# LulinZhang/BRDF-NeRF

Measured on AMD Instinct MI355X. Metric: train rays/sec (+ MFMA% of roofline), spsbrdf-nerf 64 samples/ray, 1/2/4/8 MI355X, higher is better.
Workload: dtype bf16; 1 GPU; BASELINE config 2: Djibouti-shaped synthetic rays, spsbrdf-nerf lambert train step (pass1 64 + guided 64 samples/ray, F=512, 8 Siren layers, PE10, ds_lambda=10), 4096 rays/GPU/step (4096 rays per global step, weak scaling); rays_per_gpu=4096, n_samples=64, guided_samples=64, parallelism=dp1, settle_steps=221

## Files before the change

brdf_nerf_amd/_lib.py:

```python
import ctypes as C
import os

HERE = os.path.dirname(os.path.abspath(__file__))
LIB_PATH = os.environ.get("BRDFNERF_HIP_LIB") or os.path.join(HERE, "libbrdfnerf_hip.so")

BN_MAX_LAYERS = 12
BN_MAX_HEADS = 6
BN_F32, BN_BF16, BN_F16 = 0, 1, 2
DTYPES = {"fp32": BN_F32, "bf16": BN_BF16, "fp16": BN_F16}
BN_ACT_SIN, BN_ACT_RELU = 0, 1
BN_HEAD_PLAIN, BN_HEAD_RPV_K, BN_HEAD_RPV_THETA, BN_HEAD_HAPKE_THETA, BN_HEAD_TILE3, BN_HEAD_BETA = 0, 1, 2, 3, 4, 5
BN_BRDF_AUX = 16

fptr = C.c_void_p


class FieldDesc(C.Structure):
    _fields_ = [("feat", C.c_int32), ("layers", C.c_int32), ("skip", C.c_int32), ("pe_freqs", C.c_int32),
                ("act", C.c_int32), ("dtype", C.c_int32), ("n_heads", C.c_int32),
                ("head_out", C.c_int32 * BN_MAX_HEADS), ("head_kind", C.c_int32 * BN_MAX_HEADS),
                ("normal_lr", C.c_int32), ("normal_an", C.c_int32), ("out_channels", C.c_int32), ("fold_feats", C.c_int32),
                ("dir_dim", C.c_int32), ("dir_freqs", C.c_int32), ("t_dim", C.c_int32)]


_PARAM_FIELDS = [("trunk_w", fptr * BN_MAX_LAYERS), ("trunk_b", fptr * BN_MAX_LAYERS),
                 ("sigma_w", fptr), ("sigma_b", fptr), ("feats_w", fptr), ("feats_b", fptr),
                 ("head_w1", fptr * BN_MAX_HEADS), ("head_b1", fptr * BN_MAX_HEADS),
                 ("head_w2", fptr * BN_MAX_HEADS), ("head_b2", fptr * BN_MAX_HEADS),
                 ("normal_w", fptr), ("normal_b", fptr), ("head0_wdir", fptr), ("head0_wdir_ld", C.c_int64),
                 ("head1_wt", fptr), ("head1_wt_ld", C.c_int64)]


class FieldParams(C.Structure):
    _fields_ = list(_PARAM_FIELDS)


class FieldGrads(C.Structure):
    _fields_ = list(_PARAM_FIELDS) + [("d_t_embed", fptr)]


class Points(C.Structure):
    _fields_ = [("xyz", fptr), ("rays", fptr), ("z", fptr), ("ray_stride", C.c_int32), ("n_samples", C.c_int32),
                ("n_points", C.c_int64), ("dirs", fptr), ("t_embed", fptr), ("point_offset", C.c_int64), ("total_points", C.c_int64),
                ("z2", fptr), ("n_samples2", C.c_int32), ("seg1_points", C.c_int64)]


class ShadeDesc(C.Structure):
    _fields_ = [(k, C.c_int32) for k in ("kind", "C", "ch_normal", "ch_p0", "ch_p1", "ch_p2", "rhoc_is_albedo", "shell",
                                         "cos_irradiance", "usealldepth")] + \
               [(k, C.c_float) for k in ("hpk_scl", "f0", "rgb_padding", "lambda_rgb", "lambda_ds", "lambda_hs")] + \
               [("irr", fptr), ("irr_stride", C.c_int64)]


BN_SHADE_LAMBERT, BN_SHADE_RPV, BN_SHADE_HAPKE, BN_SHADE_MICROFACET = 0, 1, 2, 3


class NormalReg(C.Structure):
    _fields_ = [("rays_d", fptr), ("rd_stride", C.c_int64), ("ch_an", C.c_int32), ("ch_lr", C.c_int32),
                ("lambda_an", C.c_float), ("lambda_lr", C.c_float), ("lambda_spv", C.c_float), ("spv_ch_an", C.c_int32),
                ("spv_ch_lr", C.c_int32), ("spv_ray", fptr), ("spv_tot", fptr)]


class Noise(C.Structure):
    _fields_ = [("rng", fptr), ("noise_std", C.c_float), ("rng_stream", C.c_uint32), ("ray_offset", C.c_int64)]


class FoldDesc(C.Structure):
    _fields_ = [("n_heads", C.c_int32), ("F", C.c_int32), ("rows", C.c_int32), ("wf", fptr), ("bf", fptr),
                ("w1", fptr * BN_MAX_HEADS), ("w1_ld", C.c_int64 * BN_MAX_HEADS), ("b1", fptr * BN_MAX_HEADS),
                ("w_fold", fptr * BN_MAX_HEADS), ("b_fold", fptr * BN_MAX_HEADS), ("m", fptr * BN_MAX_HEADS), ("s", fptr * BN_MAX_HEADS),
                ("d_w1", fptr * BN_MAX_HEADS), ("d_w1_ld", C.c_int64 * BN_MAX_HEADS), ("d_b1", fptr * BN_MAX_HEADS),
                ("d_wf", fptr), ("d_bf", fptr)]


BN_ABI_VERSION = 7
BN_STATE_BYTES, BN_STATE_LOSS_OFF, BN_STATE_LOSS_SLOTS, BN_STATE_POW_OFF, BN_STATE_PART_OFF = 1024, 64, 64, 320, 512
BN_STATE_NOISE_OFF = 40
BN_RNG_COARSE, BN_RNG_GUIDED, BN_RNG_GUIDED_TARGET, BN_RNG_NOISE_COARSE, BN_RNG_NOISE_MERGED, BN_RNG_SUN = 1, 2, 3, 4, 5, 6
BN_BWD_CHAIN, BN_BWD_WGRAD_TRUNK, BN_BWD_WGRAD_HEADS, BN_BWD_SKINNY, BN_BWD_ALL = 1, 2, 4, 8, 15


class LibraryMissing(RuntimeError):
    pass


_lib = None

_SIGS = {
    "bn_abi_version": (C.c_int, []),
    "bn_source_hash": (C.c_char_p, []),
    "bn_last_error": (C.c_char_p, []),
    "bn_build_flags": (C.c_char_p, []),
    "bn_set_deterministic": (C.c_int, [C.c_int]),
    "bn_get_deterministic": (C.c_int, []),
    "bn_field_packed_bytes": (C.c_size_t, [C.POINTER(FieldDesc)]),
    "bn_pack_field": (C.c_int, [C.POINTER(FieldDesc), C.POINTER(FieldParams), fptr, fptr]),
    "bn_field_stash_bytes": (C.c_size_t, [C.POINTER(FieldDesc), C.c_int64]),
    "bn_field_sigma": (C.c_int, [C.POINTER(FieldDesc), C.POINTER(FieldParams), fptr, C.POINTER(Points), fptr, fptr]),
    "bn_field_forward": (C.c_int, [C.POINTER(FieldDesc), C.POINTER(FieldParams), fptr, C.POINTER(Points), fptr, fptr,
                                   fptr]),
    "bn_field_backward": (C.c_int, [C.POINTER(FieldDesc), C.POINTER(FieldParams), fptr, C.POINTER(Points), fptr, fptr,
                                    fptr, C.POINTER(FieldGrads), fptr]),
    "bn_field_backward_parts": (C.c_int, [C.POINTER(FieldDesc), C.POINTER(FieldParams), fptr, C.POINTER(Points), fptr, fptr,
                                          fptr, C.POINTER(FieldGrads), C.c_int32, fptr]),
    "bn_field_normals": (C.c_int, [C.POINTER(FieldDesc), C.POINTER(FieldParams), fptr, C.POINTER(Points), fptr, fptr, fptr,
                                   C.c_int32, fptr]),
    "bn_composite_forward": (C.c_int, [fptr, fptr, C.c_int64, fptr, C.c_float, fptr, C.c_int64, C.c_int32, C.c_int64,
                                       C.c_int32, fptr, fptr, fptr, fptr, fptr, fptr]),
    "bn_composite_backward": (C.c_int, [fptr, fptr, C.c_int64, fptr, C.c_float, fptr, C.c_int64, C.c_int32, C.c_int64,
                                        C.c_int32, fptr, fptr, fptr, fptr, C.c_int64, fptr, C.c_int64, fptr]),
    "bn_lambert_loss": (C.c_int, [fptr, C.c_int32, fptr, fptr, C.c_int32, fptr, fptr, fptr, fptr, fptr, fptr, C.c_float, C.c_float,
                                  C.c_float, C.c_int32, C.c_int64, fptr, fptr, fptr, fptr, fptr, fptr]),
    "bn_stratified_z": (C.c_int, [fptr, fptr, C.c_int64, fptr, C.c_int64, C.c_int32, fptr, fptr]),
    "bn_guided_samples": (C.c_int, [fptr, fptr, fptr, fptr, C.c_int64, C.c_int32, C.c_int32, C.c_float, C.c_float,
                                    C.c_float, fptr, fptr, fptr, fptr, fptr, fptr, fptr, fptr, fptr]),
    "bn_guided_samples_nf": (C.c_int, [fptr, fptr, fptr, fptr, C.c_int64, C.c_int32, C.c_int32, fptr, C.c_float, fptr, fptr,
                                       fptr, fptr, fptr, fptr, fptr, fptr, fptr]),
    "bn_brdf_rpv_forward": (C.c_int, [fptr] * 7 + [C.c_int64, fptr, fptr, fptr]),
    "bn_brdf_rpv_backward": (C.c_int, [fptr] * 8 + [C.c_int64] + [fptr] * 6),
    "bn_brdf_hapke_forward": (C.c_int, [fptr] * 7 + [C.c_float, C.c_int32, C.c_int64, fptr, fptr, fptr]),
    "bn_brdf_hapke_backward": (C.c_int, [fptr] * 7 + [C.c_float, C.c_int32, fptr, C.c_int64] + [fptr] * 6),
    "bn_brdf_microfacet_forward": (C.c_int, [fptr] * 5 + [C.c_float, C.c_int64, fptr, fptr, fptr]),
    "bn_brdf_microfacet_backward": (C.c_int, [fptr] * 5 + [C.c_float, fptr, C.c_int64] + [fptr] * 4),
    "bn_adam_step": (C.c_int, [fptr, fptr, fptr, fptr, C.c_int64, C.c_float, C.c_float, C.c_float, C.c_float,
                               C.c_float, C.c_int32, C.c_float, fptr]),
    "bn_count_nonfinite": (C.c_int, [fptr, C.c_int64, fptr, fptr]),
    "bn_stratified_z_rng": (C.c_int, [fptr, fptr, C.c_int64, fptr, C.c_uint32, C.c_int64, C.c_int64, C.c_int32, fptr, fptr]),
    "bn_rng_uniform": (C.c_int, [fptr, C.c_uint32, C.c_int64, fptr, fptr]),
    "bn_rng_normal": (C.c_int, [fptr, C.c_uint32, C.c_int64, fptr, fptr]),
    "bn_normal_spv_reduce": (C.c_int, [fptr, C.c_int64, C.c_int32, C.c_float, fptr, fptr, fptr, fptr]),
    "bn_composite_guided": (C.c_int, [fptr, fptr, C.c_int64, C.c_int64, C.c_int32, C.c_int32, fptr, C.c_float, fptr, C.c_int64,
                                      fptr, C.c_int64, fptr, C.c_int64, fptr, fptr, fptr, C.c_uint32, C.c_uint32, C.c_int64, fptr, fptr,
                                      fptr, fptr, fptr, fptr, fptr]),
    "bn_merged_composite_forward": (C.c_int, [fptr, fptr, fptr, fptr, C.c_int32, C.c_int32, C.c_int32, C.c_int64, fptr, fptr, fptr,
                                              fptr, fptr, fptr, fptr, fptr, fptr, fptr, fptr]),
    "bn_merged_composite_backward": (C.c_int, [fptr, fptr, fptr, fptr, C.c_int32, C.c_int32, C.c_int32, C.c_int64, fptr, fptr, fptr,
                                               fptr, C.c_float, fptr, fptr, fptr, fptr, fptr, fptr, fptr]),
    "bn_ray_shade_loss": (C.c_int, [fptr, fptr, fptr, fptr, fptr, fptr, C.c_int64, fptr, C.c_int64, fptr, fptr, C.c_int64, fptr,
                                    C.c_int64, fptr, C.c_int64, fptr, C.c_int64, C.c_int64, fptr, fptr, fptr, C.c_int32, fptr, fptr,
                                    fptr, fptr, fptr, fptr]),
    "bn_ray_shade_dirs": (C.c_int, [fptr, fptr, fptr, fptr, C.c_int64, fptr, fptr, C.c_int64, C.c_int32, fptr, fptr, fptr]),
    "bn_lambert_tail": (C.c_int, [fptr, fptr, fptr, fptr, C.c_int32, C.c_int32, C.c_int32, C.c_int64, fptr, fptr, C.c_int64, fptr,
                                  C.c_int64, fptr, C.c_int64, fptr, C.c_int64, C.c_float, C.c_float, C.c_float, C.c_int32, fptr, fptr,
                                  C.c_int32, fptr, fptr, fptr, fptr, fptr, fptr, fptr, fptr]),
    "bn_sample_brdf_forward": (C.c_int, [fptr, fptr, fptr, C.c_int64, C.c_int64, C.c_int32, C.c_int64, C.c_int64, C.c_int32, C.c_int32,
                                         fptr, C.c_int32, fptr]),
    "bn_sample_brdf_backward": (C.c_int, [fptr, fptr, fptr, C.c_int64, C.c_int64, C.c_int32, C.c_int64, C.c_int64, C.c_int32, C.c_int32,
                                          fptr, C.c_int32, fptr, fptr]),
    "bn_fold_heads": (C.c_int, [fptr, fptr]),
    "bn_unfold_heads": (C.c_int, [fptr, fptr]),
    "bn_adam_multi": (C.c_int, [fptr, fptr, fptr, fptr, C.c_int32, fptr, fptr, fptr, C.c_float, C.c_float, C.c_float, C.c_float,
                                C.c_float, C.c_int32, fptr, fptr]),
    "bn_device_faults": (C.c_int, [C.POINTER(C.c_uint), fptr]),
    "bn_prof_enable": (C.c_int, [C.c_int]),
    "bn_prof_collect": (C.c_int, [C.POINTER(C.c_double), C.POINTER(C.c_int), C.c_int]),
}

PROF_NAMES = ["pack", "field_fwd_sigma", "field_fwd_full", "field_bwd_chain", "wgrad", "skinny_wgrad", "composite_fwd",
              "composite_bwd", "guided_samples", "stratified_z", "adam", "brdf", "field_adjoint", "field_adjoint_bwd", "wgrad_reduce"]


def prof_enable(on):
    lib().bn_prof_enable(int(bool(on)))


def prof_collect():
    n = len(PROF_NAMES)
    ms, cnt = (C.c_double * n)(), (C.c_int * n)()
    lib().bn_prof_collect(ms, cnt, n)
    return {PROF_NAMES[i]: (ms[i], cnt[i]) for i in range(n) if cnt[i]}


def exported_symbols():
    return sorted(_SIGS)


def load(path, baseline=False):
    if not os.path.exists(path):
        raise LibraryMissing(f"{path} not found: build the HIP extension first "
                             f"(python -m brdf_nerf_amd.build). There is no CPU fallback.")
    L = C.CDLL(path)
    for name, (res, args) in _SIGS.items():
        if baseline and not hasattr(L, name):
            continue
        fn = getattr(L, name)
        fn.restype, fn.argtypes = res, args
    if not baseline and L.bn_abi_version() != BN_ABI_VERSION:
        raise LibraryMissing(f"{path}: ABI version mismatch; rebuild")
    if not baseline and os.environ.get("BRDFNERF_ALLOW_STALE_LIB", "0") in ("", "0"):
        from .build import CSRC, source_hash
        if os.path.isdir(CSRC):
            have, want = L.bn_source_hash().decode(), source_hash()
            if have != want:
                raise LibraryMissing(f"{path} was built from other sources (library {have}, tree {want}): run "
                                     f"python -m brdf_nerf_amd.build (BRDFNERF_ALLOW_STALE_LIB=1 to load it anyway)")
    return L


def lib():
    global _lib
    if _lib is None:
        _lib = load(LIB_PATH)
        if os.environ.get("BRDFNERF_DETERMINISTIC", "0") not in ("", "0"):
            _lib.bn_set_deterministic(1)
    return _lib


def set_deterministic(on=True):
    return bool(lib().bn_set_deterministic(1 if on else 0))


def deterministic():
    L = lib()
    if not hasattr(L, "bn_get_deterministic"):
        prev = L.bn_set_deterministic(0)
        if prev:
            L.bn_set_deterministic(1)
        return bool(prev)
    return bool(L.bn_get_deterministic())


def use(handle):
    global _lib
    prev, _lib = _lib, handle
    return prev


def check(status, what=""):
    if status != 0:
        raise RuntimeError(f"{what} failed ({status}): {lib().bn_last_error().decode()}")
```

brdf_nerf_amd/csrc/field.h:

```cpp
#pragma once
#include "common.h"

#define BN_MAX_PASS 3
#define BN_DPH (3 * BN_MAX_HEADS)
#define BN_SINGLE_HEAD_NTW(NT) ((NT) > 1 ? (NT) / 2 : 1)

struct FieldGeom {
  int F, L, skip, pe_freqs, act;
  int P;
  int KP;
  int NT;
  int BM, waves;
  int dsz;
  int H2;
  int n_heads, n_pass;
  int pass_heads[BN_MAX_PASS];
  int pass_N[BN_MAX_PASS];
  int pass_NTW[BN_MAX_PASS];
  int head_col[BN_MAX_HEADS];
  int C;
  int ch_normal_an, ch_normal_lr;
  int fold;
  int DD, KD, dir_freqs, TD, KT0;
};

static inline void bn_tile_config(int dtype, int *BM, int *waves) {
  *BM = bn_half(dtype) ? 128 : 64;
  *waves = 8;
}

static inline int bn_make_geom(const bn_field_desc *d, FieldGeom *g) {
  BN_REQUIRE(d->feat >= 64 && d->feat <= 512 && d->feat % 64 == 0 && (d->feat == 512 || d->feat <= 256),
             "field: feat=%d unsupported (64,128,192,256,512)", d->feat);
  BN_REQUIRE(d->dtype == BN_F32 || d->dtype == BN_BF16 || d->dtype == BN_F16, "field: dtype=%d unknown", d->dtype);
  BN_REQUIRE(d->layers >= 2 && d->layers <= BN_MAX_LAYERS, "field: layers=%d unsupported", d->layers);
  BN_REQUIRE(d->skip < d->layers && d->skip != 0, "field: skip=%d invalid", d->skip);
  BN_REQUIRE(d->n_heads >= 1 && d->n_heads <= BN_MAX_HEADS, "field: n_heads=%d", d->n_heads);
  BN_REQUIRE(d->pe_freqs >= 0 && d->pe_freqs <= 10, "field: pe_freqs=%d", d->pe_freqs);
  g->F = d->feat; g->L = d->layers; g->skip = d->skip; g->pe_freqs = d->pe_freqs; g->act = d->act;
  g->P = d->pe_freqs > 0 ? 6 * d->pe_freqs : 3;
  g->KP = (g->P + 63) / 64 * 64;
  bn_tile_config(d->dtype, &g->BM, &g->waves);
  g->dsz = (int)bn_dsize(d->dtype, d->normal_an);
  {
    const int per = (d->feat + 32 * g->waves - 1) / (32 * g->waves);
    g->NT = per <= 1 ? 1 : (per <= 2 ? 2 : 4);
  }
  g->H2 = d->feat / 2;
  g->fold = d->fold_feats != 0;
  g->DD = d->dir_dim; g->dir_freqs = d->dir_freqs; g->TD = d->t_dim;
  g->KT0 = (d->dir_dim + 7) / 8 * 8;
  g->KD = (g->KT0 + d->t_dim + 15) / 16 * 16;
  BN_REQUIRE(d->dir_dim == 0 || (d->dir_dim == (d->dir_freqs > 0 ? 6 * d->dir_freqs : 3) && d->dir_dim <= 32 && g->fold),
             "field: dir_dim=%d dir_freqs=%d fold=%d unsupported (input_viewdir needs fold_feats and at most 5 octaves)", d->dir_dim,
             d->dir_freqs, g->fold);
  {
    const bool beta = d->n_heads >= 2 && d->head_kind[1] == BN_HEAD_BETA;
    BN_REQUIRE(beta == (d->t_dim > 0) && d->t_dim >= 0 && d->t_dim <= 16 && (!beta || (g->fold && d->head_out[1] == 1)),
               "field: t_dim=%d needs exactly a 1-wide head 1 of kind BN_HEAD_BETA (and fold_feats)", d->t_dim);
    for (int i = 0; i < d->n_heads; ++i)
      BN_REQUIRE(i == 1 || d->head_kind[i] != BN_HEAD_BETA, "field: BN_HEAD_BETA is head 1 only (head %d)", i);
    BN_REQUIRE(g->KD <= 32, "field: dir_dim=%d + t_dim=%d do not fit the 32-column extra-input tile", d->dir_dim, d->t_dim);
  }
  g->n_heads = d->n_heads;
  g->n_pass = (d->n_heads + 1) / 2;
  int c = d->t_dim > 0 ? 5 : 4;
  g->ch_normal_an = g->ch_normal_lr = -1;
  if (d->normal_an) { g->ch_normal_an = c; c += 3; }
  if (d->normal_lr) { g->ch_normal_lr = c; c += 3; }
  g->head_col[0] = 0;
  for (int i = 1; i < d->n_heads; ++i) {
    BN_REQUIRE(d->head_out[i] == 1 || d->head_out[i] == 3, "field: head_out[%d]=%d", i, d->head_out[i]);
    if (d->head_kind[i] == BN_HEAD_BETA) { g->head_col[i] = 4; continue; }
    g->head_col[i] = c;
    c += (d->head_kind[i] == BN_HEAD_PLAIN || d->head_kind[i] == BN_HEAD_HAPKE_THETA) ? d->head_out[i] : 3;
  }
  BN_REQUIRE(d->head_out[0] == 3, "field: head 0 must be rgb (3 outputs)");
  g->C = c;
  BN_REQUIRE(d->out_channels == c, "field: out_channels=%d but layout needs %d", d->out_channels, c);
  for (int p = 0; p < g->n_pass; ++p) {
    g->pass_heads[p] = (d->n_heads - 2 * p) >= 2 ? 2 : 1;
    g->pass_N[p] = g->pass_heads[p] * g->H2;
    g->pass_NTW[p] = g->pass_heads[p] == 2 ? g->NT : BN_SINGLE_HEAD_NTW(g->NT);
  }
  return 0;
}

struct PackedLayout {
  size_t fwd_trunk[BN_MAX_LAYERS][2];
  size_t fwd_feats, fwd_head[BN_MAX_PASS];
  size_t fwd_sigma, fwd_nlr;
  size_t fwd_dir;
  size_t bwd_trunk[BN_MAX_LAYERS];
  size_t bwd_feats, bwd_head[BN_MAX_PASS];
  size_t bwd_pe[2];
  size_t total;
};

static inline size_t bn_pad(size_t v, size_t a) { return (v + a - 1) / a * a; }

static inline void bn_make_packed_layout(const FieldGeom &g, PackedLayout *pl) {
  size_t off = 0;
  auto take = [&](size_t rows, size_t k) { size_t o = off; off += bn_pad(rows, 32) * bn_pad(k, 16); return o; };
  for (int l = 0; l < g.L; ++l) {
    pl->fwd_trunk[l][0] = pl->fwd_trunk[l][1] = 0;
    if (l == 0) pl->fwd_trunk[l][0] = take(g.F, g.KP);
    else if (l == g.skip) { pl->fwd_trunk[l][0] = take(g.F, g.KP); pl->fwd_trunk[l][1] = take(g.F, g.F); }
    else pl->fwd_trunk[l][0] = take(g.F, g.F);
  }
  pl->fwd_sigma = take(32, g.F);
  pl->fwd_feats = g.fold ? 0 : take(g.F, g.F);
  for (int p = 0; p < g.n_pass; ++p) pl->fwd_head[p] = take(g.pass_N[p], g.F);
  pl->fwd_nlr = g.ch_normal_lr >= 0 ? take(32, g.F) : 0;
  pl->fwd_dir = g.KD > 0 ? take(g.pass_N[0], g.KD) : 0;
  for (int l = 0; l < g.L; ++l) pl->bwd_trunk[l] = l >= 1 ? take(g.F, g.F) : 0;
  pl->bwd_feats = g.fold ? 0 : take(g.F, g.F);
  for (int p = 0; p < g.n_pass; ++p) pl->bwd_head[p] = take(g.F, g.pass_N[p]);
  pl->bwd_pe[0] = take(g.KP, g.F);
  pl->bwd_pe[1] = g.skip > 0 ? take(g.KP, g.F) : 0;
  pl->total = off;
}

struct StashLayout {
  size_t gscale;
  size_t sraw;
  size_t nraw;
  size_t dpre_trunk;
  size_t dpre_head;
  size_t pe;
  size_t dirpe;
  size_t Y[BN_MAX_LAYERS];
  size_t D[BN_MAX_LAYERS];
  size_t feats;
  size_t G[BN_MAX_PASS];
  size_t DG[BN_MAX_PASS];
  size_t dZ[BN_MAX_LAYERS];
  size_t dfeats;
  size_t dG[BN_MAX_PASS];
  size_t gradx;
  size_t sbar;
  size_t sprime;
  size_t gbar_pe;
  size_t adj_delta[BN_MAX_LAYERS];
  size_t adj_a[BN_MAX_LAYERS];
  size_t adj_abar[BN_MAX_LAYERS + 1];
  size_t adj_zbar[BN_MAX_LAYERS];
  size_t wgpart, wgpart_bytes;
  size_t total;
  int64_t Mpad;
};

static inline int64_t bn_wgrad_splits(bool half, int64_t tiles, int64_t Mpad, int64_t *m_per_block) {
  const int64_t stage = half ? 64 : 32;
  const int64_t min_mpb = half ? 512 : 256;
  int64_t n_split = (half ? (Mpad <= 327680 ? BN_W2_BLOCKS : 2 * BN_W2_BLOCKS) : 2048) / (tiles > 0 ? tiles : 1);
  if (n_split < 1) n_split = 1;
  int64_t mpb = ceil_div64(ceil_div64(Mpad, n_split), stage) * stage;
  if (mpb < min_mpb) mpb = min_mpb;
  if (m_per_block) *m_per_block = mpb;
  return ceil_div64(Mpad, mpb);
}
static inline size_t bn_wgpart_bytes(const FieldGeom &g, int64_t Mpad, size_t esz) {
  const bool half = esz != 4;
  const int64_t tl = half ? 256 : 128, ft = (g.F + tl - 1) / tl;
  const int64_t tiles_bound = (2 * g.L + 12) * ft * ft;
  const int64_t grid_bound = half ? 2 * BN_W2_BLOCKS : 2048;
  int64_t slabs = tiles_bound > grid_bound ? tiles_bound : grid_bound;
  const int64_t by_points = tiles_bound * bn_wgrad_splits(half, 1, Mpad, nullptr);
  if (by_points < slabs) slabs = by_points;
  const size_t wg = (size_t)slabs * (size_t)(tl * tl + tl) * 4;
  int64_t sk_splits = ceil_div64(Mpad, g.BM);
  if (sk_splits > 256) sk_splits = 256;
  const size_t sk = (size_t)10 * (size_t)sk_splits * (4 * 512 + 4) * 4;
  return wg > sk ? wg : sk;
}

static inline void bn_make_stash_layout(const FieldGeom &g, int64_t n_points, int BM, size_t esz, StashLayout *s) {
  const size_t dsz = (size_t)g.dsz;
  int64_t Mpad = ceil_div64(n_points, BM) * BM;
  s->Mpad = Mpad;
  size_t off = 0;
  auto take = [&](size_t bytes) { size_t o = off; off += bn_pad(bytes, 256); return o; };
  s->gscale = take(256);
  s->sraw = take((size_t)Mpad * 4);
  s->nraw = take((size_t)Mpad * 16);
  s->dpre_trunk = take((size_t)Mpad * 16);
  s->dpre_head = take((size_t)Mpad * BN_DPH * 4);
  s->pe = take((size_t)Mpad * g.KP * esz);
  s->dirpe = g.KD > 0 ? take((size_t)Mpad * g.KD * esz) : 0;
  for (int l = 0; l < g.L; ++l) s->Y[l] = take((size_t)Mpad * g.F * esz);
  for (int l = 0; l < g.L; ++l) s->D[l] = take((size_t)Mpad * g.F * dsz);
  s->feats = take((size_t)Mpad * g.F * esz);
  for (int p = 0; p < BN_MAX_PASS; ++p) {
    s->G[p] = s->DG[p] = s->dG[p] = 0;
    if (p < g.n_pass) {
      s->G[p] = take((size_t)Mpad * g.F * esz);
      s->DG[p] = take((size_t)Mpad * g.F * dsz);
    }
  }
  for (int l = 0; l < g.L; ++l) s->dZ[l] = take((size_t)Mpad * g.F * esz);
  s->dfeats = take((size_t)Mpad * g.F * esz);
  for (int p = 0; p < g.n_pass; ++p) s->dG[p] = take((size_t)Mpad * g.pass_N[p] * esz);
  s->gradx = s->sbar = s->sprime = s->gbar_pe = 0;
  for (int l = 0; l < BN_MAX_LAYERS; ++l) s->adj_delta[l] = s->adj_a[l] = s->adj_abar[l] = s->adj_zbar[l] = 0;
  s->adj_abar[BN_MAX_LAYERS] = 0;
  if (g.ch_normal_an >= 0) {
    s->gradx = take((size_t)Mpad * 16);
    s->sbar = take((size_t)Mpad * 4);
    s->sprime = take((size_t)Mpad * 4);
    s->gbar_pe = take((size_t)Mpad * g.KP * esz);
    for (int l = 0; l < g.L; ++l) {
      s->adj_delta[l] = take((size_t)Mpad * g.F * esz);
      s->adj_a[l] = take((size_t)Mpad * g.F * esz);
      s->adj_abar[l + 1] = take((size_t)Mpad * g.F * esz);
      s->adj_zbar[l] = take((size_t)Mpad * g.F * esz);
    }
  }
  s->wgpart_bytes = bn_wgpart_bytes(g, Mpad, esz);
  s->wgpart = take(s->wgpart_bytes);
  s->total = off;
}

static inline void bn_stash_layout_at(const FieldGeom &g, const bn_points *pts, int BM, size_t esz, StashLayout *s) {
  const int64_t total = pts->total_points > 0 ? pts->total_points : pts->n_points;
  bn_make_stash_layout(g, total, BM, esz, s);
  const size_t off = (size_t)pts->point_offset;
  if (off == 0) return;
  const size_t dsz = (size_t)g.dsz, F = (size_t)g.F;
  s->sraw += off * 4; s->nraw += off * 16; s->dpre_trunk += off * 16; s->dpre_head += off * BN_DPH * 4;
  s->pe += off * g.KP * esz;
  if (g.KD > 0) s->dirpe += off * g.KD * esz;
  for (int l = 0; l < g.L; ++l) { s->Y[l] += off * F * esz; s->D[l] += off * F * dsz; s->dZ[l] += off * F * esz; }
  s->feats += off * F * esz; s->dfeats += off * F * esz;
  for (int p = 0; p < g.n_pass; ++p) { s->G[p] += off * F * esz; s->DG[p] += off * F * dsz; s->dG[p] += off * g.pass_N[p] * esz; }
  if (g.ch_normal_an >= 0) {
    s->gradx += off * 16; s->sbar += off * 4; s->sprime += off * 4; s->gbar_pe += off * g.KP * esz;
    for (int l = 0; l < g.L; ++l) {
      s->adj_delta[l] += off * F * esz; s->adj_a[l] += off * F * esz; s->adj_abar[l + 1] += off * F * esz; s->adj_zbar[l] += off * F * esz;
    }
  }
  s->Mpad = ceil_div64(pts->n_points, BM) * BM;
}
```

brdf_nerf_amd/csrc/field_bwd.hip:

```cpp
#include "field_kernels.h"
#include "field_wgrad.h"

int bn_field_adjoint_backward(const bn_field_desc *desc, const bn_field_params *params, const void *packed, const bn_points *pts,
                              const float *d_out, void *stash, void *stream);

__device__ unsigned int g_bwd_fault;
unsigned int bn_bwd_fault_read(hipStream_t) {
  unsigned int v = 0u;
  if (hipMemcpyFromSymbol(&v, HIP_SYMBOL(g_bwd_fault), sizeof(unsigned int), 0, hipMemcpyDeviceToHost) != hipSuccess) return 0x80000000u;
  return v;
}
const unsigned int *bn_bwd_fault_ptr() {
  void *p = nullptr;
  return hipGetSymbolAddress(&p, HIP_SYMBOL(g_bwd_fault)) == hipSuccess ? (const unsigned int *)p : nullptr;
}

BN_PH_DEFINE_READER(bn_debug_phase_read_bwd)
BN_CLK_DEFINE(bn_debug_clock_read_bwd)

struct BwdArgs {
  FieldGeom g;
  bn_field_desc d;
  bn_field_params p;
  PackedLayout pl;
  StashLayout sl;
  const void *packed;
  int64_t M;
  const float *out, *d_out;
  char *stash;
  int an;
  const float *amax;
};

__device__ __forceinline__ void head_y_dy(int kind, int nout, const float *o, const float *dgo, int c, float &y, float &dy) {
  if (kind == BN_HEAD_PLAIN || kind == BN_HEAD_BETA) { y = o[c]; dy = dgo[c]; }
  else if (kind == BN_HEAD_HAPKE_THETA) { y = o[0] * (1.f / 0.52359877559829887f); dy = dgo[0] * 0.52359877559829887f; }
  else {
    const float ov = nout == 1 ? o[0] : o[c];
    const float dv = nout == 1 ? dgo[0] + dgo[1] + dgo[2] : dgo[c];
    if (kind == BN_HEAD_RPV_K) { y = (ov - 1.f) * 0.5f + 0.5f; dy = 2.f * dv; }
    else if (kind == BN_HEAD_RPV_THETA) { y = ov * 0.5f + 0.5f; dy = 2.f * dv; }
    else { y = ov; dy = dv; }
  }
}

__device__ __forceinline__ void bwd_dpre(const BwdArgs &A, int64_t gm, float (&dph)[BN_DPH], float (&dpt)[4]) {
  const FieldGeom &g = A.g;
#pragma unroll
  for (int i = 0; i < BN_DPH; ++i) dph[i] = 0.f;
#pragma unroll
  for (int i = 0; i < 4; ++i) dpt[i] = 0.f;
  if (gm >= A.M) return;
  const float *o = A.out + gm * g.C, *dgo = A.d_out + gm * g.C;
  for (int hd = 0; hd < g.n_heads; ++hd) {
    const int nout = A.d.head_out[hd], kind = A.d.head_kind[hd];
    for (int c = 0; c < nout; ++c) {
      float y, dy;
      head_y_dy(kind, nout, o + g.head_col[hd], dgo + g.head_col[hd], c, y, dy);
      dph[hd * 3 + c] = kind == BN_HEAD_BETA ? dy * -expm1f(-y) : dy * y * (1.f - y);
    }
  }
  const float sraw = ((const float *)(A.stash + A.sl.sraw))[gm];
  dpt[0] = dgo[3] * sigmoid_f(sraw);
  if (A.an) dpt[0] += ((const float *)(A.stash + A.sl.sbar))[gm];
  if (g.ch_normal_lr >= 0) {
    const float *v = (const float *)(A.stash + A.sl.nraw) + gm * 4;
    const float *dn = dgo + g.ch_normal_lr;
    const float n2 = v[0] * v[0] + v[1] * v[1] + v[2] * v[2];
    const float eps = 1.1920928955078125e-07f;
    const float inv = 1.f / sqrtf(fmaxf(n2, eps));
    const float vd = v[0] * dn[0] + v[1] * dn[1] + v[2] * dn[2];
    const float k = n2 > eps ? vd * inv * inv * inv : 0.f;
#pragma unroll
    for (int i = 0; i < 3; ++i) dpt[1 + i] = -(dn[i] * inv - v[i] * k);
  }
}

__global__ void clear_words_kernel(unsigned int *p, int n) {
  for (int i = blockIdx.x * blockDim.x + threadIdx.x; i < n; i += gridDim.x * blockDim.x) p[i] = 0u;
}

template <int WHICH> __global__ __launch_bounds__(256) void grad_amax_kernel(const BwdArgs A, float *amax) {
  const FieldGeom &g = A.g;
  float mx = 0.f;
  for (int64_t gm = (int64_t)blockIdx.x * 256 + threadIdx.x; gm < A.M; gm += (int64_t)gridDim.x * 256) {
    if (WHICH == 0) {
      float dph[BN_DPH], dpt[4];
      bwd_dpre(A, gm, dph, dpt);
#pragma unroll
      for (int i = 0; i < BN_DPH; ++i) { const float a = fabsf(dph[i]); mx = (a < 3.0e38f && a > mx) ? a : mx; }
#pragma unroll
      for (int i = 0; i < 4; ++i) { const float a = fabsf(dpt[i]); mx = (a < 3.0e38f && a > mx) ? a : mx; }
    } else {
      const float *gx = (const float *)(A.stash + A.sl.gradx) + gm * 4;
      const float *dn = A.d_out + gm * g.C + g.ch_normal_an;
      const float n2 = gx[0] * gx[0] + gx[1] * gx[1] + gx[2] * gx[2];
      const float eps = 1.1920928955078125e-07f;
      const float inv = 1.f / sqrtf(fmaxf(n2, eps));
      const float gd = gx[0] * dn[0] + gx[1] * dn[1] + gx[2] * dn[2];
      const float k = n2 > eps ? gd * inv * inv * inv : 0.f;
      const float fmx = g.pe_freqs > 0 ? (float)(1 << (g.pe_freqs - 1)) : 1.f;
      const float spm = ((const float *)(A.stash + A.sl.sprime))[gm];
#pragma unroll
      for (int c = 0; c < 3; ++c) { const float a = fabsf(dn[c] * inv - gx[c] * k) * spm * fmx; mx = (a < 3.0e38f && a > mx) ? a : mx; }
    }
  }
#pragma unroll
  for (int o = 32; o >= 1; o >>= 1) mx = fmaxf(mx, __shfl_xor(mx, o));
  if ((threadIdx.x & 63) == 0 && mx > 0.f) atomicMax((unsigned int *)amax + WHICH, __float_as_uint(mx));
}

template <typename T>
__global__ __launch_bounds__(256) void head_xin_grad_kernel(const T *__restrict__ dG, int ldg, int col0, int H2, const float *__restrict__ Wt,
                                                            int64_t ldw, int TD, int64_t M, const float *amax, float *__restrict__ d_t) {
  __shared__ float W[256 * 16];
  for (int i = threadIdx.x; i < H2 * 16; i += 256) W[i] = (i & 15) < TD ? Wt[(int64_t)(i >> 4) * ldw + (i & 15)] : 0.f;
  __syncthreads();
  const float osc = 1.f / chain_scale(amax);
  const int lane = threadIdx.x & 63, wave = threadIdx.x >> 6;
  for (int64_t gm = (int64_t)blockIdx.x * 4 + wave; gm < M; gm += (int64_t)gridDim.x * 4) {
    float acc[16];
#pragma unroll
    for (int c = 0; c < 16; ++c) acc[c] = 0.f;
    const T *row = dG + gm * ldg + col0;
    for (int j = lane; j < H2; j += 64) {
      const float d = (float)row[j];
#pragma unroll
      for (int c = 0; c < 16; ++c) acc[c] += d * W[j * 16 + c];
    }
#pragma unroll
    for (int c = 0; c < 16; ++c) {
#pragma unroll
      for (int o = 32; o >= 1; o >>= 1) acc[c] += __shfl_xor(acc[c], o);
    }
    if (lane < TD) {
      float v = 0.f;
#pragma unroll
      for (int c = 0; c < 16; ++c) v = lane == c ? acc[c] : v;
      d_t[gm * TD + lane] = v * osc;
    }
  }
}

template <typename T, int MT, int NTW, bool D16>
__device__ __forceinline__ void bwd_head_dG(const BwdArgs &A, int p, T *ACT, const float *DPH, int64_t , int64_t tile) {
  typedef typename DKind<T, D16>::type DK;
  typedef typename Elem<T>::vec4 vec4;
  constexpr int BM = MT * 32;
  const FieldGeom &g = A.g;
  const int F = g.F, LDA = F + Elem<T>::kPad;
  const int tid = threadIdx.x, lane = tid & 63, wave = tid >> 6, r = lane & 31, h = lane >> 5;
  const int N = g.pass_N[p];
  const int pc0 = wave * 32 * NTW;
  if (pc0 >= N) return;
// ... 167 lines not shown
          const int n0 = ncol0 + nt * 32 + 16 * gp + 4 * h;
          float dv[8], v[8];
          dpiece_get<DK>(dpre[nt][mt], gp, g.act, dscale, dv);
#pragma unroll
          for (int e = 0; e < 8; ++e) v[e] = acc[nt][mt][8 * gp + e];
          if constexpr (top) {
            const float ds = DPT[m * 4], a0 = DPT[m * 4 + 1], a1 = DPT[m * 4 + 2], a2 = DPT[m * 4 + 3];
#pragma unroll
            for (int half = 0; half < 2; ++half) {
              const int n = n0 + 8 * half;
              const f32x4 ws = *(const f32x4 *)(A.p.sigma_w + n);
#pragma unroll
              for (int e = 0; e < 4; ++e) v[4 * half + e] += ws[e] * ds;
              if (nlr) {
                const f32x4 wn0 = *(const f32x4 *)(A.p.normal_w + n), wn1 = *(const f32x4 *)(A.p.normal_w + F + n),
                            wn2 = *(const f32x4 *)(A.p.normal_w + 2 * F + n);
#pragma unroll
                for (int e = 0; e < 4; ++e) v[4 * half + e] += wn0[e] * a0 + wn1[e] * a1 + wn2[e] * a2;
              }
            }
          }
#pragma unroll
          for (int e = 0; e < 8; ++e) v[e] *= dv[e];
          if (A.an) {
            float zb[8];
            if constexpr (ZPRE) {
              const auto zq = __builtin_bit_cast(bf16x8, zraw[nt][mt][gp]);
#pragma unroll
              for (int e = 0; e < 8; ++e) zb[e] = (float)zq[e];
            } else {
              ld8((const WT *)(A.stash + A.sl.adj_zbar[lo]) + (size_t)tile * BM * F + native_off8<MT, NT>(wave, nt, mt, gp, lane), zb);
            }
#pragma unroll
            for (int e = 0; e < 8; ++e) v[e] += zb[e] * zr;
          }
          if constexpr (NATZ) {
            const typename Elem<T>::frag q = cvt8(T(), v);
            *(vec4 *)(ACT + (size_t)m * LDA + n0) = __builtin_shufflevector(q, q, 0, 1, 2, 3);
            *(vec4 *)(ACT + (size_t)m * LDA + n0 + 8) = __builtin_shufflevector(q, q, 4, 5, 6, 7);
            stash_store_buf(Zr, voff, ((((wave_u * NT + nt) * MT + mt) * 2 + gp) * 1024), q);
          } else {
            *(vec4 *)(ACT + (size_t)m * LDA + n0) = to_vec4(T(), v[0], v[1], v[2], v[3]);
            *(vec4 *)(ACT + (size_t)m * LDA + n0 + 8) = to_vec4(T(), v[4], v[5], v[6], v[7]);
          }
        }
      }
  };
  {
    if (!g.fold) {
      zero_acc<MT, NT>(acc);
      T *fdst = (T *)(A.stash + A.sl.dfeats) + (size_t)m0 * F;
      if (!ride) tile_to_global<T>(ACT, LDA, fdst, F, BM, F);
      if (wave_on) {
        load_D(g.L - 1, 0, NPRE);
        const size_t off = A.pl.bwd_feats + (size_t)(ncol0 / 32) * KSF * 512;
        if (ride) {
          TileCopyExact<T> zcopy(ACT, LDA, fdst, F, F, tid, WAVES * 64);
          gemm_seg<T, MT, NT, DP>(acc, packed + off, KSF, ACT, LDA, lane, zcopy);
        } else {
          gemm_seg<T, MT, NT, DP>(acc, packed + off, KSF, ACT, LDA, lane);
        }
        load_D(g.L - 1, NPRE, NT);
      }
    } else if (wave_on) {
      load_D(g.L - 1, 0, NT);
    }
    BN_PH(9)
    __syncthreads();
    BN_PH(10)
    if (wave_on) epilogue(g.L - 1, std::true_type());
    BN_PH(11)
    __syncthreads();
    BN_PH(12)
  }
  for (int l = g.L - 1; l >= 1; --l) {
    const int it = g.L - 1 - l;
    const int lo = l - 1;
    zero_acc<MT, NT>(acc);
    T *zdst = (T *)(A.stash + A.sl.dZ[l]) + (size_t)m0 * F;
    if (!NATZ && !ride) tile_to_global<T>(ACT, LDA, zdst, F, BM, F);
    if (wave_on) {
      if (!PING || BN_BWD_D_AT == 0) load_D(lo, 0, NPRE);
      const size_t off = A.pl.bwd_trunk[l] + (size_t)(ncol0 / 32) * KSF * 512;
      if constexpr (PING) {
        pp_wait(WR + 0, 4 * it, &g_bwd_fault);
        if (grp == 1) pp_wait(RD + 0, 4 * (it + 1), &g_bwd_fault);
        BN_PH(12)
        __builtin_amdgcn_s_setprio(1);
        if constexpr (sizeof(T) == 2) {
          gemm_fixed<T, MT, NT, (DP & (BN_GEMM_AFFINE - 1)), 32, 16>(acc, packed + off, KSF, 0, ACT, LDA, lane, [&]() {
            pp_signal(RD + 0 + grp, lane);
            pp_wait(WR + 1, 4 * it, &g_bwd_fault);
            if (BN_BWD_D_AT == 1) load_D(lo, 0, NPRE);
          });
        }
        __builtin_amdgcn_s_setprio(0);
        pp_signal(RD + 2 + grp, lane);
        if (BN_BWD_D_AT == 2) load_D(lo, 0, NPRE);
      } else if (!NATZ && ride) {
        TileCopyExact<T> zcopy(ACT, LDA, zdst, F, F, tid, WAVES * 64);
        gemm_seg<T, MT, NT, DP>(acc, packed + off, KSF, ACT, LDA, lane, zcopy);
      } else {
        gemm_seg<T, MT, NT, DP>(acc, packed + off, KSF, ACT, LDA, lane);
      }
      load_D(lo, NPRE, NT);
    }
    BN_PH(9)
    if constexpr (PING) {
      pp_wait(RD + 2 * grp + 0, 4 * (it + 1), &g_bwd_fault);
      pp_wait(RD + 2 * grp + 1, 4 * (it + 1), &g_bwd_fault);
    } else {
      __syncthreads();
    }
    BN_PH(10)
    if (wave_on) epilogue(lo, std::false_type());
    BN_PH(11)
    if constexpr (PING) pp_signal(WR + grp, lane);
    else __syncthreads();
    BN_PH(12)
  }
  if (PING) __syncthreads();
  if (!NATZ) tile_to_global<T>(ACT, LDA, (T *)(A.stash + A.sl.dZ[0]) + (size_t)m0 * F, F, BM, F);
  BN_PH(13)
#ifndef BN_PHASE_TIMING_WGRAD
  BN_PH_FLUSH
#endif
#ifndef BN_CLOCK_STAMP_WGRAD
  BN_CLK_END
#endif
}

template <typename T, int MT, int NT, int WAVES, bool D16> static int launch_bwd_k(const BwdArgs &a, int64_t tiles, hipStream_t st) {
  constexpr int BM = MT * 32;
  const size_t lds = (size_t)BM * (a.g.F + Elem<T>::kPad) * sizeof(T) + (size_t)BM * (BN_DPH + 4) * sizeof(float) + 64;
  if (int e = bn_configure_lds((const void *)field_bwd_kernel<T, MT, NT, WAVES, D16>, lds, "field_bwd")) return e;
  BnProfScope prof_(BN_K_BWD_CHAIN, st);
  field_bwd_kernel<T, MT, NT, WAVES, D16><<<dim3((unsigned)tiles), WAVES * 64, lds, st>>>(a);
  BN_LAUNCH_CHECK("field_bwd");
  return 0;
}
template <typename T, int MT, int NT, int WAVES> static int launch_bwd(const BwdArgs &a, int64_t tiles, hipStream_t st) {
  if constexpr (std::is_same<T, f16>::value) {
    if (a.g.dsz == 2) return launch_bwd_k<T, MT, NT, WAVES, true>(a, tiles, st);
  }
  return launch_bwd_k<T, MT, NT, WAVES, false>(a, tiles, st);
}

extern "C" int bn_field_backward(const bn_field_desc *desc, const bn_field_params *params, const void *packed,
                                 const bn_points *pts, const float *out, const float *d_out, void *stash,
                                 const bn_field_grads *G, void *stream) {
  return bn_field_backward_parts(desc, params, packed, pts, out, d_out, stash, G, BN_BWD_ALL, stream);
}

extern "C" int bn_field_backward_parts(const bn_field_desc *desc, const bn_field_params *params, const void *packed,
                                       const bn_points *pts, const float *out, const float *d_out, void *stash,
                                       const bn_field_grads *G, int32_t parts, void *stream) {
  BwdArgs a;
  if (int e = bn_make_geom(desc, &a.g)) return e;
  if (const int f = bn_field_fault_seen()) {
    bn_set_error("field_backward: an earlier %s launch lost an LDS hand-over (pp_wait timed out): its results are invalid",
                 (f & 1) ? "forward" : "backward");
    return BN_ELAUNCH;
  }
  a.an = desc->normal_an ? 1 : 0;
  BN_REQUIRE(pts && pts->n_points > 0 && packed && out && d_out && stash && G, "field_backward: null argument");
  BN_REQUIRE(parts > 0 && (parts & ~BN_BWD_ALL) == 0, "field_backward: parts=%d", parts);
  BN_REQUIRE(pts->point_offset == 0 && (pts->total_points == 0 || pts->total_points == pts->n_points),
             "field_backward: the backward runs over a whole point set (point_offset = 0)");
  BN_REQUIRE(pts->seg1_points == 0 || (pts->rays && pts->z && pts->z2 && pts->n_samples2 > 0 && pts->seg1_points < pts->n_points &&
                                       pts->seg1_points % pts->n_samples == 0 && (pts->n_points - pts->seg1_points) % pts->n_samples2 == 0),
             "field_backward: bad two-block point set");
  BN_REQUIRE(pts->seg1_points == 0 || !(desc->t_dim > 0 && G->d_t_embed), "field_backward: d_t_embed is not served for a two-block point set");
  const FieldGeom &g = a.g;
  a.d = *desc; a.p = *params; a.packed = packed; a.M = pts->n_points; a.out = out; a.d_out = d_out; a.stash = (char *)stash;
  bn_make_packed_layout(g, &a.pl);
  const bool bf = bn_half(desc->dtype);
  const bool f16m = desc->dtype == BN_F16;
  const int BM = g.BM;
  const size_t esz = bn_esize(desc->dtype);
  bn_make_stash_layout(g, pts->n_points, BM, esz, &a.sl);
  const int64_t tiles = ceil_div64(pts->n_points, BM);
  hipStream_t st = (hipStream_t)stream;
  int rc;
  float *amax = f16m ? (float *)((char *)stash + a.sl.gscale) : nullptr;
  a.amax = amax;
  const unsigned amax_grid = (unsigned)(ceil_div64(pts->n_points, 256) < 1024 ? ceil_div64(pts->n_points, 256) : 1024);
  if (parts & BN_BWD_CHAIN) {
  if (f16m) {
    clear_words_kernel<<<1, 64, 0, st>>>((unsigned int *)amax, 4);
    BN_LAUNCH_CHECK("clear amax");
    if (a.an) {
      grad_amax_kernel<1><<<amax_grid, 256, 0, st>>>(a, amax);
      BN_LAUNCH_CHECK("grad_amax<1>");
    }
  }
  if (a.an) {
    rc = bn_field_adjoint_backward(desc, params, packed, pts, d_out, stash, stream);
    if (rc) return rc;
  }
  if (f16m) {
    grad_amax_kernel<0><<<amax_grid, 256, 0, st>>>(a, amax);
    BN_LAUNCH_CHECK("grad_amax<0>");
  }
  rc = [&]() -> int { BN_DISPATCH_TILE(desc->dtype, g, launch_bwd, (a, tiles, st)); }();
  if (rc) return rc;
  }

  const StashLayout &sl = a.sl;
  char *S = (char *)stash;
  const int F = g.F, P0 = g.P;
  WgradArgs w;
  w.n_jobs = 0; w.Mpad = sl.Mpad; w.tile0[0] = 0; w.amax = amax; w.part = nullptr; w.n_split = 1;
  int scale_sel = 1;
  int b_native = 0;
  int a_native = 0;
  int part = BN_BWD_WGRAD_TRUNK;
  auto add = [&](const void *A_, int lda, int a0, const void *B_, int ldb, int b0, float *C, int ldc, float *bias, int N, int K) {
    if (!C || !(parts & part)) return;
    WgradJob &j = w.job[w.n_jobs];
    j.scale_sel = scale_sel;
    j.b_native = (b_native ? WG_B_NATIVE : 0) | (a_native ? WG_A_NATIVE : 0); j.b_bm = BM; j.b_F = F; j.b_bm_shift = BM == 128 ? 7 : 6;
    j.A = A_; j.B = B_; j.C = C; j.bias = bias; j.lda = lda; j.ldb = ldb; j.ldc = ldc; j.a_col0 = a0; j.b_col0 = b0; j.N = N; j.K = K;
    w.tile0[w.n_jobs + 1] = w.tile0[w.n_jobs] + ((N + 127) / 128) * ((K + 127) / 128);
    ++w.n_jobs;
  };
  const int naty = bf ? 1 : 0;
  a_native = naty;
  for (int l = 0; l < g.L; ++l) {
    const void *dZ = S + sl.dZ[l];
    b_native = 0;
    if (l == 0) add(dZ, F, 0, S + sl.pe, g.KP, 0, G->trunk_w[l], P0, G->trunk_b[l], F, P0);
    else if (l == g.skip) {
      add(dZ, F, 0, S + sl.pe, g.KP, 0, G->trunk_w[l], F + P0, G->trunk_b[l], F, P0);
      b_native = naty;
      add(dZ, F, 0, S + sl.Y[l - 1], F, 0, G->trunk_w[l] ? G->trunk_w[l] + P0 : nullptr, F + P0, nullptr, F, F);
    } else {
      b_native = naty;
      add(dZ, F, 0, S + sl.Y[l - 1], F, 0, G->trunk_w[l], F, G->trunk_b[l], F, F);
    }
  }
  a_native = 0;
  b_native = naty;
  part = BN_BWD_WGRAD_HEADS;
  if (!g.fold) add(S + sl.dfeats, F, 0, S + sl.Y[g.L - 1], F, 0, G->feats_w, F, G->feats_b, F, F);
  part = BN_BWD_WGRAD_TRUNK;
  b_native = 0;
  if (a.an) {
    scale_sel = 2;
    for (int l = 0; l < g.L; ++l) {
      const void *dl = S + sl.adj_delta[l];
      if (l == 0) add(dl, F, 0, S + sl.gbar_pe, g.KP, 0, G->trunk_w[l], P0, nullptr, F, P0);
      else if (l == g.skip) {
        add(dl, F, 0, S + sl.gbar_pe, g.KP, 0, G->trunk_w[l], F + P0, nullptr, F, P0);
        add(dl, F, 0, S + sl.adj_abar[l], F, 0, G->trunk_w[l] ? G->trunk_w[l] + P0 : nullptr, F + P0, nullptr, F, F);
      } else add(dl, F, 0, S + sl.adj_abar[l], F, 0, G->trunk_w[l], F, nullptr, F, F);
    }
  }
  scale_sel = 1;
  part = BN_BWD_WGRAD_HEADS;
  for (int hd = 0; hd < g.n_heads; ++hd) {
    const int p = hd / 2, hl = hd % 2;
    b_native = g.fold ? naty : 0;
    add(S + sl.dG[p], g.pass_N[p], hl * g.H2, S + (g.fold ? sl.Y[g.L - 1] : sl.feats), F, 0, G->head_w1[hd], F, G->head_b1[hd], g.H2, F);
  }
  if (g.DD > 0 && G->head0_wdir) {
    b_native = 0; scale_sel = 1;
    add(S + sl.dG[0], g.pass_N[0], 0, S + sl.dirpe, g.KD, 0, G->head0_wdir, (int)G->head0_wdir_ld, nullptr, g.H2, g.DD);
  }
  if (g.TD > 0 && G->head1_wt) {
    b_native = 0; scale_sel = 1;
    add(S + sl.dG[0], g.pass_N[0], g.H2, S + sl.dirpe, g.KD, g.KT0, G->head1_wt, (int)G->head1_wt_ld, nullptr, g.H2, g.TD);
  }
  BN_REQUIRE(w.n_jobs <= BN_MAX_WGRAD_JOBS, "field_backward: too many wgrad jobs");
  float *wgpart = (float *)(S + sl.wgpart);
  if (w.n_jobs > 0)
    if (int e = bn_launch_wgrad(w, bf, f16m, sl.Mpad, wgpart, sl.wgpart_bytes, st)) return e;
  if (!(parts & BN_BWD_SKINNY)) return 0;
  SkinnyArgs s;
  s.n_jobs = 0; s.Mpad = sl.Mpad; s.amax = amax; s.part = nullptr;
  for (int i = 0; i < BN_MAX_SKINNY_JOBS; ++i) { s.job[i].scale_sel = 0; s.job[i].unit_dpre = 0; }
  {
    SkinnyJob &j = s.job[s.n_jobs];
    j.X = S + sl.Y[g.L - 1]; j.ldx = F; j.x_col0 = 0; j.K = F; j.dpre = (const float *)(S + sl.dpre_trunk); j.ldp = 4; j.p_col0 = 0;
    j.nc = g.ch_normal_lr >= 0 ? 4 : 1; j.native = 0;
    if (naty) { j.native = 1; j.bm = BM; j.ntw = g.NT; j.tstride = BM * F; }
    for (int c = 0; c < 4; ++c) { j.out[c] = nullptr; j.bias[c] = nullptr; }
    j.out[0] = G->sigma_w; j.bias[0] = G->sigma_b;
    if (g.ch_normal_lr >= 0) {
      BN_REQUIRE(G->normal_w && G->normal_b, "field_backward: normal grads missing");
      for (int c = 0; c < 3; ++c) { j.out[1 + c] = G->normal_w + (size_t)c * F; j.bias[1 + c] = G->normal_b + c; }
    }
    if (j.out[0]) ++s.n_jobs;
  }
  if (a.an && G->sigma_w) {
    SkinnyJob &j = s.job[s.n_jobs++];
    j.unit_dpre = 1;
    j.scale_sel = 2;
    j.X = S + sl.adj_abar[g.L]; j.ldx = F; j.x_col0 = 0; j.K = F; j.dpre = (const float *)(S + sl.sprime); j.ldp = 1; j.p_col0 = 0; j.nc = 1; j.native = 0;
    for (int c = 0; c < 4; ++c) { j.out[c] = nullptr; j.bias[c] = nullptr; }
    j.out[0] = G->sigma_w;
  }
  for (int hd = 0; hd < g.n_heads; ++hd) {
    if (!G->head_w2[hd]) continue;
    const int p = hd / 2, hl = hd % 2;
    SkinnyJob &j = s.job[s.n_jobs++];
    j.X = S + sl.G[p]; j.ldx = 0; j.x_col0 = hl * g.H2; j.K = g.H2;
    j.native = 1; j.bm = BM; j.ntw = g.pass_NTW[p]; j.tstride = BM * F;
    j.dpre = (const float *)(S + sl.dpre_head); j.ldp = BN_DPH; j.p_col0 = hd * 3; j.nc = desc->head_out[hd];
    for (int c = 0; c < 4; ++c) { j.out[c] = nullptr; j.bias[c] = nullptr; }
    for (int c = 0; c < j.nc; ++c) { j.out[c] = G->head_w2[hd] + (size_t)c * g.H2; j.bias[c] = G->head_b2[hd] ? G->head_b2[hd] + c : nullptr; }
  }
  if (s.n_jobs > 0) {
    int skinny_splits = SKINNY_SPLITS;
    {
      int64_t most = sl.Mpad / (2 * (int64_t)BM) > 1 ? sl.Mpad / (2 * (int64_t)BM) : 1;
      if (sl.Mpad <= 131072 && most > 128) most = 128;
      if (skinny_splits > most) skinny_splits = (int)most;
    }
    int64_t smpb = ceil_div64(ceil_div64(sl.Mpad, skinny_splits), BM) * BM;
    s.m_per_block = (int)smpb;
    if (int e = bn_launch_skinny(s, bf, f16m, sl.Mpad, smpb, wgpart, sl.wgpart_bytes, st)) return e;
  }
  if (g.TD > 0 && G->d_t_embed) {
    BN_REQUIRE(params->head1_wt && params->head1_wt_ld >= g.TD && g.H2 <= 256, "field_backward: head1_wt missing (beta)");
    const int64_t M = pts->n_points;
    const unsigned blocks = (unsigned)(ceil_div64(M, 4) < 4096 ? ceil_div64(M, 4) : 4096);
    const int ldg = g.pass_N[0];
    if (f16m) head_xin_grad_kernel<f16><<<dim3(blocks), 256, 0, st>>>((const f16 *)(S + sl.dG[0]), ldg, g.H2, g.H2, params->head1_wt, params->head1_wt_ld, g.TD, M, amax, G->d_t_embed);
    else if (bf) head_xin_grad_kernel<bf16><<<dim3(blocks), 256, 0, st>>>((const bf16 *)(S + sl.dG[0]), ldg, g.H2, g.H2, params->head1_wt, params->head1_wt_ld, g.TD, M, amax, G->d_t_embed);
    else head_xin_grad_kernel<float><<<dim3(blocks), 256, 0, st>>>((const float *)(S + sl.dG[0]), ldg, g.H2, g.H2, params->head1_wt, params->head1_wt_ld, g.TD, M, amax, G->d_t_embed);
    BN_LAUNCH_CHECK("head_xin_grad");
  }
  return 0;
}
```

brdf_nerf_amd/csrc/field_wgrad.h:

```cpp
#pragma once
#include <hip/hip_runtime.h>
#include <stdint.h>

struct WgradJob {
  const void *A;
  const void *B;
  float *C;
  float *bias;
  int lda, ldb, ldc;
  int a_col0, b_col0;
  int N, K;
  int scale_sel;
  int b_native;
  int b_bm, b_F;
  int b_bm_shift;
};
#define WG_B_NATIVE 1
#define WG_A_NATIVE 2
#define BN_MAX_WGRAD_JOBS 44
struct WgradArgs {
  WgradJob job[BN_MAX_WGRAD_JOBS];
  int tile0[BN_MAX_WGRAD_JOBS + 1];
  int n_jobs;
  int64_t Mpad;
  int m_per_block;
  const float *amax;
  float *part;
  int n_split;
  int chain_next[BN_MAX_WGRAD_JOBS];
  unsigned char head[BN_MAX_WGRAD_JOBS];
};
#define WG_SLAB256 (256 * 256 + 256)
#define WG_SLAB128 (128 * 128 + 128)
#define SK_SLAB (4 * 512 + 4)

struct SkinnyJob {
  const void *X;
  const float *dpre;
  int ldx, x_col0, K, ldp, p_col0, nc;
  int native;
  int bm, ntw, tstride;
  float *out[4];
  float *bias[4];
  int scale_sel;
  int unit_dpre;
};
#define BN_MAX_SKINNY_JOBS 10
struct SkinnyArgs {
  SkinnyJob job[BN_MAX_SKINNY_JOBS];
  int n_jobs;
  int64_t Mpad;
  int m_per_block;
  const float *amax;
  float *part;
};

int bn_launch_wgrad(WgradArgs &wv, bool bf, bool f16m, int64_t Mpad, float *part, size_t part_bytes, hipStream_t st);
int bn_launch_skinny(SkinnyArgs &sv, bool bf, bool f16m, int64_t Mpad, int64_t m_per_block, float *part, size_t part_bytes, hipStream_t st);
unsigned int bn_bwd_fault_read(hipStream_t st);
```

brdf_nerf_amd/csrc/field_wgrad.hip:

```cpp
#include "field_kernels.h"
#include "field_wgrad.h"


__device__ __forceinline__ float wg_unscale(const float *amax, int sel) {
  if (amax == nullptr || sel == 0) return 1.f;
  return 1.f / (sel == 1 ? chain_scale(amax) : grad_scale_from(amax + 1, BN_GS_TARGET_ADJ));
}

#define WG_BK 32
template <typename T> struct WgTile;
template <> struct WgTile<float> { static constexpr int LD = 128 + 4; };

template <typename T> __device__ __forceinline__ typename Elem<T>::frag wg_frag(const T *tile, int mm, int col0, int lane);
template <> __device__ __forceinline__ f32x8 wg_frag<float>(const float *tile, int mm, int col0, int lane) {
  constexpr int LD = WgTile<float>::LD;
  const int h = lane >> 5, r = lane & 31;
  f32x8 f;
#pragma unroll
  for (int j = 0; j < 8; ++j) f[j] = tile[(size_t)(mm + 2 * j + h) * LD + col0 + r];
  return f;
}

template <typename T> __global__ __launch_bounds__(256) void wgrad_kernel(const WgradArgs A) {
  constexpr int LD = WgTile<T>::LD;
  constexpr int EPC = 16 / sizeof(T);
  constexpr int CPR = 128 / EPC;
  constexpr int NCH = WG_BK * CPR / 256;
  __shared__ __attribute__((aligned(16))) T sA[WG_BK * LD];
  __shared__ __attribute__((aligned(16))) T sB[WG_BK * LD];
  int jb = 0;
  while (jb + 1 < A.n_jobs && (int)blockIdx.x >= A.tile0[jb + 1]) ++jb;
  const WgradJob &J = A.job[jb];
  const int t = blockIdx.x - A.tile0[jb];
  const int tiles_k = (J.K + 127) / 128;
  const int n0 = (t / tiles_k) * 128, k0 = (t % tiles_k) * 128;
  const int tid = threadIdx.x, lane = tid & 63, wave = tid >> 6, wr = wave >> 1, wc = wave & 1;
  const int64_t mb = (int64_t)blockIdx.y * A.m_per_block;
  const int64_t me = mb + A.m_per_block < A.Mpad ? mb + A.m_per_block : A.Mpad;
  const T *gA = (const T *)J.A + J.a_col0 + n0;
  const T *gB = (const T *)J.B + J.b_col0 + k0;
  uint4 ra[NCH], rb[NCH];
  auto gload = [&](int64_t m) {
#pragma unroll
    for (int c = 0; c < NCH; ++c) {
      const int ch = tid + c * 256, row = ch / CPR, cc = (ch % CPR) * EPC;
      ra[c] = (n0 + cc < J.N) ? *(const uint4 *)(gA + (m + row) * J.lda + cc) : uint4{0, 0, 0, 0};
      rb[c] = (k0 + cc < J.K) ? *(const uint4 *)(gB + (m + row) * J.ldb + cc) : uint4{0, 0, 0, 0};
    }
  };
  auto sstore = [&]() {
#pragma unroll
    for (int c = 0; c < NCH; ++c) {
      const int ch = tid + c * 256, row = ch / CPR, cc = (ch % CPR) * EPC;
      *(uint4 *)(sA + row * LD + cc) = ra[c];
      *(uint4 *)(sB + row * LD + cc) = rb[c];
    }
  };
  f32x16 acc[2][2];
#pragma unroll
  for (int a = 0; a < 2; ++a)
#pragma unroll
    for (int b = 0; b < 2; ++b)
#pragma unroll
      for (int i = 0; i < 16; ++i) acc[a][b][i] = 0.f;
  float bsum = 0.f;
  const bool do_bias = J.bias != nullptr && k0 == 0 && tid < 128;
  gload(mb);
  for (int64_t m = mb; m < me; m += WG_BK) {
    __syncthreads();
    sstore();
    __syncthreads();
    if (m + WG_BK < me) gload(m + WG_BK);
#pragma unroll
    for (int mm = 0; mm < WG_BK; mm += 16) {
      typename Elem<T>::frag fa[2], fb[2];
#pragma unroll
      for (int a = 0; a < 2; ++a) fa[a] = wg_frag<T>(sA, mm, wr * 64 + a * 32, lane);
#pragma unroll
      for (int b = 0; b < 2; ++b) fb[b] = wg_frag<T>(sB, mm, wc * 64 + b * 32, lane);
#pragma unroll
      for (int a = 0; a < 2; ++a)
#pragma unroll
        for (int b = 0; b < 2; ++b) mma32(acc[a][b], fa[a], fb[b]);
    }
    if (do_bias) {
#pragma unroll 8
      for (int row = 0; row < WG_BK; ++row) bsum += (float)sA[row * LD + tid];
    }
  }
  float *P = A.part + ((size_t)blockIdx.x * gridDim.y + blockIdx.y) * WG_SLAB128;
#pragma unroll
  for (int a = 0; a < 2; ++a)
#pragma unroll
    for (int b = 0; b < 2; ++b)
#pragma unroll
      for (int q = 0; q < 4; ++q)
        *(f32x4 *)(P + (size_t)(((((wave * 2 + a) * 2 + b) * 4 + q) * 64 + lane) * 4)) =
            f32x4{acc[a][b][4 * q], acc[a][b][4 * q + 1], acc[a][b][4 * q + 2], acc[a][b][4 * q + 3]};
  if (do_bias) P[128 * 128 + tid] = bsum;
}

__device__ __attribute__((aligned(16))) unsigned short w2_zeros[8];
#define W2_LD (256 + 32)
#define W2_BK 64
#define W2_STAGE (W2_BK * W2_LD)
__device__ __forceinline__ int w2_swz(int row) { return ((row >> 1) & 3) << 1; }
template <typename T> __device__ __forceinline__ typename Elem<T>::frag w2_frag(const T *tile, int mm, int col0, int lane) {
  const int h = lane >> 5, grp = (lane >> 4) & 1, i = lane & 15, q = i >> 2, p = i & 3;
  const int s_lo = (4 * grp + p) ^ w2_swz(8 * h + q);
  const int d_hi = 4 * W2_LD + ((((s_lo ^ 4) - s_lo)) << 2);
  const T *a = tile + (size_t)(mm + 8 * h + q) * W2_LD + (((col0 >> 2) + s_lo) << 2);
  typedef __attribute__((address_space(3))) s16x4 lds_v4;
  const s16x4 lo = __builtin_amdgcn_ds_read_tr16_b64_v4i16((lds_v4 *)a);
  const s16x4 hi = __builtin_amdgcn_ds_read_tr16_b64_v4i16((lds_v4 *)(a + d_hi));
  union { s16x4 s[2]; typename Elem<T>::frag b; } u;
  u.s[0] = lo; u.s[1] = hi;
  return u.b;
}

__device__ __forceinline__ float frag_sum8(float s, const bf16x8 &f) {
  typedef __attribute__((ext_vector_type(2))) __bf16 bf16x2;
  const bf16x2 one = {(__bf16)1.f, (__bf16)1.f};
  s = __builtin_amdgcn_fdot2_f32_bf16(__builtin_shufflevector(f, f, 0, 1), one, s, false);
  s = __builtin_amdgcn_fdot2_f32_bf16(__builtin_shufflevector(f, f, 2, 3), one, s, false);
  s = __builtin_amdgcn_fdot2_f32_bf16(__builtin_shufflevector(f, f, 4, 5), one, s, false);
  s = __builtin_amdgcn_fdot2_f32_bf16(__builtin_shufflevector(f, f, 6, 7), one, s, false);
  return s;
}
__device__ __forceinline__ float frag_sum8(float s, const f16x8 &f) {
  typedef __attribute__((ext_vector_type(2))) _Float16 f16x2;
  const f16x2 one = {(_Float16)1.f, (_Float16)1.f};
  s = __builtin_amdgcn_fdot2(__builtin_shufflevector(f, f, 0, 1), one, s, false);
  s = __builtin_amdgcn_fdot2(__builtin_shufflevector(f, f, 2, 3), one, s, false);
  s = __builtin_amdgcn_fdot2(__builtin_shufflevector(f, f, 4, 5), one, s, false);
  s = __builtin_amdgcn_fdot2(__builtin_shufflevector(f, f, 6, 7), one, s, false);
  return s;
}
__device__ __forceinline__ float frag_sum8(float s, const f32x8 &f) {
#pragma unroll
  for (int j = 0; j < 8; ++j) s += f[j];
  return s;
}

#if defined(BN_PHASE_TIMING) && defined(BN_PHASE_TIMING_WGRAD)
BN_PH_DEFINE_READER(bn_debug_phase_read_wgrad)
#define WG_PH_DECL BN_PH_DECL
#define WG_PH(i) BN_PH(i)
#define WG_PH_FLUSH BN_PH_FLUSH
#else
#define WG_PH_DECL
#define WG_PH(i)
#define WG_PH_FLUSH
#endif
#ifndef W2_WAVES
// ... 48 lines not shown
      *(u32x4 *)(rowp + ((sl0 ^ nswz) << 2)) = u32x4{s02[0], s13[0], s02[1], s13[1]};
    } else {
      *(u32x4 *)(sA + buf * W2_STAGE + (row0 + RPP * c) * W2_LD + scol) = ra[c];
    }
    if (BNAT) {
      T *rowp = sB + buf * W2_STAGE + (32 * (c & 1) + nr) * W2_LD;
      const int sl0 = lslot0 + 4 * ((c >> 1) & 1);
      const auto s02 = __builtin_amdgcn_permlane32_swap(rb[c][0], rb[c][2], false, false);
      const auto s13 = __builtin_amdgcn_permlane32_swap(rb[c][1], rb[c][3], false, false);
      *(u32x4 *)(rowp + ((sl0 ^ nswz) << 2)) = u32x4{s02[0], s13[0], s02[1], s13[1]};
    } else {
      *(u32x4 *)(sB + buf * W2_STAGE + (row0 + RPP * c) * W2_LD + scol) = rb[c];
    }
  };
  auto sstore = [&](int buf) {
#pragma unroll
    for (int c = 0; c < NC; ++c) sstore1(buf, c);
  };
  f32x16 acc[W2_RA][4];
#pragma unroll
  for (int a = 0; a < W2_RA; ++a)
#pragma unroll
    for (int b = 0; b < 4; ++b)
#pragma unroll
      for (int i = 0; i < 16; ++i) acc[a][b][i] = 0.f;
  constexpr int BA = W2_RA / 2;
  const bool do_bias = J.bias != nullptr && k0 == 0;
  float bsum[BA];
#pragma unroll
  for (int a = 0; a < BA; ++a) bsum[a] = 0.f;
  WG_PH_DECL
  auto compute = [&](int buf, int64_t m_next2) {
    const T *cA = sA + buf * W2_STAGE, *cB = sB + buf * W2_STAGE;
    frag_t fa[2][W2_RA], fb[2][NBV > 0 ? NBV : 1];
    auto frags = [&](int set, int mm) {
#pragma unroll
      for (int a = 0; a < W2_RA; ++a) fa[set][a] = w2_frag<T>(cA, mm, wr * (W2_RA * 32) + a * 32, lane);
#pragma unroll
      for (int b = 0; b < NBV; ++b) fb[set][b] = w2_frag<T>(cB, mm, wc * 128 + b * 32, lane);
    };
    frags(0, 0);
#pragma unroll
    for (int i = 0; i < W2_BK / 16; ++i) {
      const int cur = i & 1;
      if (i + 1 < W2_BK / 16) frags(cur ^ 1, (i + 1) * 16);
      __builtin_amdgcn_sched_barrier(0);
#pragma unroll
      for (int a = 0; a < W2_RA; ++a)
#pragma unroll
        for (int b = 0; b < NBV; ++b) mma32(acc[a][b], fa[cur][a], fb[cur][b]);
      {
#pragma unroll
        for (int a = 0; a < BA; ++a) {
          const u32x4 f0 = __builtin_bit_cast(u32x4, fa[cur][a]), f1 = __builtin_bit_cast(u32x4, fa[cur][BA + a]);
          bsum[a] = frag_sum8(bsum[a], __builtin_bit_cast(frag_t, wc ? f1 : f0));
        }
      }
      {
        constexpr int CPS = NC / (W2_BK / 16) > 0 ? NC / (W2_BK / 16) : 1;
#pragma unroll
        for (int q = 0; q < CPS; ++q) {
          const int c = i * CPS + q;
          if (c < NC) { sstore1(buf ^ 1, c); gload1(m_next2, c); }
        }
      }
      __builtin_amdgcn_sched_barrier(0);
    }
  };
  gload(mb);
  sstore(0);
#pragma unroll
  for (int c = 0; c < NC; ++c) {
    __builtin_amdgcn_sched_barrier(0);
    gload1(mb + W2_BK, c);
  }
  __builtin_amdgcn_sched_barrier(0);
  WG_PH(14)
  int buf = 0;
  for (int64_t m = mb; m < me; m += W2_BK) {
    __syncthreads();
    WG_PH(3)
    compute(buf, m + 2 * W2_BK);
    WG_PH(0)
    buf ^= 1;
  }
  const int r = lane & 31, h = lane >> 5;
#pragma unroll
  for (int a = 0; a < W2_RA; ++a)
#pragma unroll
    for (int b = 0; b < 4; ++b)
#pragma unroll
      for (int q = 0; q < 4; ++q)
        *(f32x4 *)(P + (size_t)(((((wave * W2_RA + a) * 4 + b) * 4 + q) * 64 + lane) * 4)) =
            f32x4{acc[a][b][4 * q], acc[a][b][4 * q + 1], acc[a][b][4 * q + 2], acc[a][b][4 * q + 3]};
  if (do_bias) {
#pragma unroll
    for (int a = 0; a < BA; ++a) {
      const float v = bsum[a] + __shfl_xor(bsum[a], 32);
      if (h == 0) P[256 * 256 + wr * (W2_RA * 32) + (wc * BA + a) * 32 + r] = v;
    }
  }
  WG_PH(4)
  WG_PH_FLUSH
}

template <typename T>
__global__ __launch_bounds__(W2_WAVES * 64, W2_WAVES == 8 ? 2 : 1) void wgrad256_kernel(const WgradArgs A, int n_split, int n_blocks) {
  extern __shared__ __attribute__((aligned(16))) char smem_w[];
  T *sA = (T *)smem_w;
  T *sB = sA + 2 * W2_STAGE;
  const int per = n_blocks / 8;
  const int lid = (int)((blockIdx.x % 8) * per + blockIdx.x / 8);
  const int total_tiles = A.tile0[A.n_jobs];
  if (lid >= total_tiles * n_split) return;
  const int split = lid / total_tiles, tt = lid % total_tiles;
  int jb = 0;
  while (jb + 1 < A.n_jobs && tt >= A.tile0[jb + 1]) ++jb;
  const WgradJob &J = A.job[jb];
  const int t = tt - A.tile0[jb];
  const int tiles_k = (J.K + 255) / 256;
  const int n0 = (t / tiles_k) * 256, k0 = (t % tiles_k) * 256;
  const int64_t mb = (int64_t)split * A.m_per_block;
  const int64_t me = mb + A.m_per_block < A.Mpad ? mb + A.m_per_block : A.Mpad;
  if (mb >= me) return;
  const int wc = (threadIdx.x >> 6) & 1;
  const int cols = J.K - k0 - wc * 128;
  float *P = A.part + ((size_t)tt * n_split + split) * WG_SLAB256;
#ifdef BN_CLOCK_STAMP_WGRAD
  BN_CLK_BEGIN
#endif
  if (J.b_native & WG_A_NATIVE) {
    if (J.b_native & WG_B_NATIVE) {
      if (cols >= 65) w2_body<T, 4, true, true>(J, n0, k0, mb, me, sA, sB, P);
      else if (cols >= 33) w2_body<T, 2, true, true>(J, n0, k0, mb, me, sA, sB, P);
      else w2_body<T, 0, true, true>(J, n0, k0, mb, me, sA, sB, P);
    } else if (cols >= 65) w2_body<T, 4, false, true>(J, n0, k0, mb, me, sA, sB, P);
    else if (cols >= 33) w2_body<T, 2, false, true>(J, n0, k0, mb, me, sA, sB, P);
    else if (cols >= 1) w2_body<T, 1, false, true>(J, n0, k0, mb, me, sA, sB, P);
    else w2_body<T, 0, false, true>(J, n0, k0, mb, me, sA, sB, P);
  } else if (J.b_native & WG_B_NATIVE) {
    if (cols >= 65) w2_body<T, 4, true, false>(J, n0, k0, mb, me, sA, sB, P);
    else if (cols >= 33) w2_body<T, 2, true, false>(J, n0, k0, mb, me, sA, sB, P);
    else w2_body<T, 0, true, false>(J, n0, k0, mb, me, sA, sB, P);
  } else if (cols >= 65) w2_body<T, 4, false, false>(J, n0, k0, mb, me, sA, sB, P);
  else if (cols >= 33) w2_body<T, 2, false, false>(J, n0, k0, mb, me, sA, sB, P);
  else if (cols >= 1) w2_body<T, 1, false, false>(J, n0, k0, mb, me, sA, sB, P);
  else w2_body<T, 0, false, false>(J, n0, k0, mb, me, sA, sB, P);
#ifdef BN_CLOCK_STAMP_WGRAD
  BN_CLK_END
#endif
}


template <typename T> __global__ __launch_bounds__(256) void skinny_wgrad_kernel(const SkinnyArgs A) {
  const SkinnyJob &J = A.job[blockIdx.y];
  const float osc = wg_unscale(A.amax, J.scale_sel);
  const int64_t mb = (int64_t)blockIdx.x * A.m_per_block;
  const int64_t me = mb + A.m_per_block < A.Mpad ? mb + A.m_per_block : A.Mpad;
  const int tid = threadIdx.x;
  __shared__ float red[4 * 512 + 4];
  for (int i = tid; i < 4 * 512 + 4; i += 256) red[i] = 0.f;
  __syncthreads();
  if (J.native) {
    const int lane = tid & 63, wv = tid >> 6, r = lane & 31, h = lane >> 5;
    const int mt_n = J.bm / 32, ncb = J.K / 32;
    const T *X = (const T *)J.X;
    float bs[4] = {0, 0, 0, 0}, bs0[4] = {0, 0, 0, 0};
    for (int cb = wv; cb < ncb; cb += 4) {
      const int cbp = J.x_col0 / 32 + cb, wave_n = cbp / J.ntw, nt = cbp % J.ntw;
      float s[2][4][8];
#pragma unroll
      for (int gp = 0; gp < 2; ++gp)
#pragma unroll
        for (int c = 0; c < 4; ++c)
#pragma unroll
          for (int e = 0; e < 8; ++e) s[gp][c][e] = 0.f;
#pragma unroll 2
      for (int64_t m0 = mb; m0 < me; m0 += 32) {
        const int64_t tile = m0 / J.bm;
        const int mt = (int)(m0 % J.bm) / 32;
        const float *dp = J.dpre + (m0 + r) * J.ldp + J.p_col0;
        float d[4];
#pragma unroll
        for (int c = 0; c < 4; ++c) d[c] = dp[c];
#pragma unroll
        for (int c = 0; c < 4; ++c) bs[c] += d[c];
#pragma unroll
        for (int gp = 0; gp < 2; ++gp) {
          float x[8];
          ld8(X + (size_t)tile * J.tstride + ((((size_t)(wave_n * J.ntw + nt) * mt_n + mt) * 2 + gp) * 64 + lane) * 8, x);
#pragma unroll
          for (int c = 0; c < 4; ++c)
#pragma unroll
            for (int e = 0; e < 8; ++e) s[gp][c][e] += d[c] * x[e];
        }
      }
#pragma unroll
      for (int c = 0; c < 4; ++c)
        if (c < J.nc) {
#pragma unroll
          for (int gp = 0; gp < 2; ++gp)
#pragma unroll
            for (int e = 0; e < 8; ++e) {
              float *dst = &red[c * 512 + cb * 32 + 16 * gp + 4 * h + (e & 3) + 8 * (e >> 2)];
              float v = s[gp][c][e];
#pragma unroll
              for (int o = 16; o >= 1; o >>= 1) v += __shfl_xor(v, o);
              if (r == 0) *dst = v;
            }
        }
      if (cb == 0) {
#pragma unroll
        for (int c = 0; c < 4; ++c) bs0[c] = bs[c];
      }
#pragma unroll
      for (int c = 0; c < 4; ++c) bs[c] = 0.f;
    }
    if (wv == 0 && h == 0) {
#pragma unroll
      for (int c = 0; c < 4; ++c)
        if (c < J.nc) {
          float v = bs0[c];
#pragma unroll
          for (int o = 16; o >= 1; o >>= 1) v += __shfl_xor(v, o);
          if (r == 0) red[4 * 512 + c] = v;
        }
    }
  } else {
  const T *X = (const T *)J.X + J.x_col0;
  const int ncg = J.K / 8, nrg = 256 / ncg;
  const int cg = tid % ncg, rg = tid / ncg;
  float s[4][8], bs[4] = {0, 0, 0, 0};
#pragma unroll
  for (int c = 0; c < 4; ++c)
#pragma unroll
    for (int e = 0; e < 8; ++e) s[c][e] = 0.f;
  if (rg < nrg) {
#pragma unroll 2
    for (int64_t m = mb + rg; m < me; m += nrg) {
      float x[8];
      ld8(X + m * J.ldx + cg * 8, x);
      const float *dp = J.dpre + m * J.ldp + J.p_col0;
#pragma unroll
      for (int c = 0; c < 4; ++c) {
        const float d = J.unit_dpre ? 1.f : dp[c];
#pragma unroll
        for (int e = 0; e < 8; ++e) s[c][e] += d * x[e];
        bs[c] += d;
      }
    }
  }
  for (int turn = 0; turn < nrg; ++turn) {
    if (rg == turn) {
#pragma unroll
      for (int c = 0; c < 4; ++c)
        if (c < J.nc) {
#pragma unroll
          for (int e = 0; e < 8; ++e) red[c * 512 + cg * 8 + e] += s[c][e];
          if (cg == 0) red[4 * 512 + c] += bs[c];
        }
    }
    __syncthreads();
  }
  }
  __syncthreads();
  float *SP = A.part + ((size_t)blockIdx.y * gridDim.x + blockIdx.x) * SK_SLAB;
  for (int i = tid; i < J.nc * J.K; i += 256) {
    const int c = i / J.K, k = i % J.K;
    SP[c * 512 + k] = red[c * 512 + k];
  }
  if (tid < 4) SP[4 * 512 + tid] = tid < J.nc ? red[4 * 512 + tid] : 0.f;
}

template <int TILE> __global__ __launch_bounds__(256) void wgrad_reduce_kernel(const WgradArgs A) {
  constexpr int NB = TILE / 64;
  constexpr int SLAB = TILE * TILE + TILE;
  constexpr int SUBS = TILE * TILE / 4 / 256;
  const int tt = blockIdx.x / SUBS, sub = blockIdx.x % SUBS, tid = threadIdx.x;
  int jb = 0;
  while (jb + 1 < A.n_jobs && tt >= A.tile0[jb + 1]) ++jb;
  if (!A.head[jb]) return;
  const WgradJob &J = A.job[jb];
  const int t = tt - A.tile0[jb];
  const int tiles_k = (J.K + TILE - 1) / TILE;
  const int n0 = (t / tiles_k) * TILE, k0 = (t % tiles_k) * TILE;
  const int ns = A.n_split;
  {
    const int idx4 = sub * 256 + tid;
    const int lane = idx4 & 63, q = (idx4 >> 6) & 3, b = (idx4 >> 8) % NB, a = ((idx4 >> 8) / NB) & 1, wave = (idx4 >> 8) / (NB * 2);
    f32x4 v = {0.f, 0.f, 0.f, 0.f};
    for (int jj = jb; jj >= 0; jj = A.chain_next[jj]) {
      const float osc = wg_unscale(A.amax, A.job[jj].scale_sel);
      const float *P = A.part + (size_t)(A.tile0[jj] + t) * ns * SLAB + (size_t)idx4 * 4;
      f32x4 sum = {0.f, 0.f, 0.f, 0.f};
      int sp = 0;
      for (; sp + 8 <= ns; sp += 8) {
        f32x4 x[8];
#pragma unroll
        for (int u = 0; u < 8; ++u) x[u] = *(const f32x4 *)(P + (size_t)(sp + u) * SLAB);
#pragma unroll
        for (int u = 0; u < 8; ++u) sum += x[u];
      }
      for (; sp < ns; ++sp) sum += *(const f32x4 *)(P + (size_t)sp * SLAB);
      v += sum * osc;
    }
    const int r = lane & 31, h = lane >> 5, wr = wave >> 1, wc = wave & 1;
    const int k = k0 + wc * (TILE / 2) + b * 32 + r, nb = n0 + wr * 64 + a * 32 + 8 * q + 4 * h;
#pragma unroll
    for (int e = 0; e < 4; ++e)
      if (nb + e < J.N && k < J.K) J.C[(size_t)(nb + e) * J.ldc + k] += v[e];
  }
  if (sub == 0 && k0 == 0 && tid < TILE && n0 + tid < J.N) {
    float v = 0.f;
    float *dst = nullptr;
    for (int jj = jb; jj >= 0; jj = A.chain_next[jj]) {
      if (!A.job[jj].bias) continue;
      dst = A.job[jj].bias;
      const float osc = wg_unscale(A.amax, A.job[jj].scale_sel);
      const float *P = A.part + (size_t)(A.tile0[jj] + t) * ns * SLAB + TILE * TILE + tid;
      float sum = 0.f;
      for (int sp = 0; sp < ns; ++sp) sum += P[(size_t)sp * SLAB];
      v += sum * osc;
    }
    if (dst) dst[n0 + tid] += v;
  }
}

__global__ __launch_bounds__(256) void skinny_reduce_kernel(const SkinnyArgs A, int n_split) {
  __shared__ float part[8][32], bpart[256];
  const int jb = blockIdx.x, c = blockIdx.y, k0 = blockIdx.z * 32, tid = threadIdx.x, kk = tid & 31, g = tid >> 5;
  const SkinnyJob &J = A.job[jb];
  if (c >= J.nc || !J.out[c] || k0 >= J.K) return;
  for (int j2 = 0; j2 < jb; ++j2)
    for (int c2 = 0; c2 < A.job[j2].nc; ++c2)
      if (A.job[j2].out[c2] == J.out[c]) return;
  float v = 0.f, vb = 0.f;
  for (int j2 = jb; j2 < A.n_jobs; ++j2)
    for (int c2 = 0; c2 < A.job[j2].nc; ++c2) {
      if (A.job[j2].out[c2] != J.out[c]) continue;
      const float osc = wg_unscale(A.amax, A.job[j2].scale_sel);
      const float *P = A.part + (size_t)j2 * n_split * SK_SLAB;
      const bool col = k0 + kk < A.job[j2].K;
      float sum = 0.f;
      int sp = g;
      for (; sp + 56 < n_split; sp += 64) {
        float x[8];
#pragma unroll
        for (int u = 0; u < 8; ++u) x[u] = col ? P[(size_t)(sp + 8 * u) * SK_SLAB + c2 * 512 + k0 + kk] : 0.f;
#pragma unroll
        for (int u = 0; u < 8; ++u) sum += x[u];
      }
      for (; sp < n_split; sp += 8) sum += col ? P[(size_t)sp * SK_SLAB + c2 * 512 + k0 + kk] : 0.f;
      __syncthreads();
      part[g][kk] = sum;
      __syncthreads();
      if (g == 0) {
        float t = 0.f;
#pragma unroll
        for (int q = 0; q < 8; ++q) t += part[q][kk];
        v += t * osc;
      }
      if (k0 == 0 && A.job[j2].bias[c2] && J.bias[c]) {
        __syncthreads();
        bpart[tid] = tid < n_split ? P[(size_t)tid * SK_SLAB + 4 * 512 + c2] : 0.f;
        __syncthreads();
        if (tid == 0) {
          float t = 0.f;
          for (int q = 0; q < n_split; ++q) t += bpart[q];
          vb += t;
        }
      }
    }
  if (g == 0 && k0 + kk < J.K) J.out[c][k0 + kk] += v;
  if (k0 == 0 && tid == 0 && J.bias[c]) *J.bias[c] += vb;
}

static void wg_chain(WgradArgs &wv) {
  for (int j = 0; j < wv.n_jobs; ++j) { wv.chain_next[j] = -1; wv.head[j] = 1; }
  for (int j = 0; j < wv.n_jobs; ++j) {
    if (!wv.head[j]) continue;
    int last = j;
    for (int q = j + 1; q < wv.n_jobs; ++q) {
      const WgradJob &a = wv.job[j], &b = wv.job[q];
      if (b.C == a.C && b.N == a.N && b.K == a.K && b.ldc == a.ldc) { wv.chain_next[last] = q; wv.head[q] = 0; last = q; }
    }
  }
}

int bn_launch_wgrad(WgradArgs &wv, bool bf, bool f16m, int64_t Mpad, float *part, size_t part_bytes, hipStream_t st) {
  if (wv.n_jobs == 0) { wv.tile0[0] = 0; return 0; }
  BN_REQUIRE(part, "wgrad: no slab workspace");
  wv.part = part;
  wv.tile0[0] = 0;
  wg_chain(wv);
  if (bf) {
    for (int j = 0; j < wv.n_jobs; ++j)
      wv.tile0[j + 1] = wv.tile0[j] + ((wv.job[j].N + 255) / 256) * ((wv.job[j].K + 255) / 256);
    const int tiles = wv.tile0[wv.n_jobs];
    static_assert(W2_BK == 64, "bn_wgrad_splits (field.h) rounds the points per workgroup to W2_BK");
    int64_t mpb2 = 0;
    const int64_t n_split = bn_wgrad_splits(true, tiles, Mpad, &mpb2);
    wv.m_per_block = (int)mpb2;
    wv.n_split = (int)n_split;
    BN_REQUIRE((size_t)tiles * n_split * WG_SLAB256 * sizeof(float) <= part_bytes, "wgrad: %d tiles x %d splits do not fit the slab workspace (%zu bytes)",
               tiles, (int)n_split, part_bytes);
    const int n_blocks = (int)ceil_div64((int64_t)tiles * n_split, 8) * 8;
    const size_t lds = (size_t)4 * W2_STAGE * 2;
    const void *kfn = f16m ? (const void *)wgrad256_kernel<f16> : (const void *)wgrad256_kernel<bf16>;
    if (int e = bn_configure_lds(kfn, lds, "wgrad256")) return e;
    {
      BnProfScope prof_(BN_K_WGRAD, st);
      const dim3 grd((unsigned)n_blocks), blk(W2_WAVES * 64);
      if (f16m) wgrad256_kernel<f16><<<grd, blk, lds, st>>>(wv, (int)n_split, n_blocks);
      else wgrad256_kernel<bf16><<<grd, blk, lds, st>>>(wv, (int)n_split, n_blocks);
      BN_LAUNCH_CHECK("wgrad256");
    }
    BnProfScope prof_(BN_K_WGRAD_REDUCE, st);
    wgrad_reduce_kernel<256><<<dim3((unsigned)tiles * 64), 256, 0, st>>>(wv);
    BN_LAUNCH_CHECK("wgrad_reduce");
    return 0;
  }
  for (int j = 0; j < wv.n_jobs; ++j)
    wv.tile0[j + 1] = wv.tile0[j] + ((wv.job[j].N + 127) / 128) * ((wv.job[j].K + 127) / 128);
  const int tiles = wv.tile0[wv.n_jobs];
  static_assert(WG_BK == 32, "bn_wgrad_splits (field.h) rounds the points per workgroup to WG_BK");
  int64_t mpb = 0;
  wv.n_split = (int)bn_wgrad_splits(false, tiles, Mpad, &mpb);
  wv.m_per_block = (int)mpb;
  BN_REQUIRE((size_t)tiles * wv.n_split * WG_SLAB128 * sizeof(float) <= part_bytes, "wgrad: %d tiles x %d splits do not fit the slab workspace (%zu bytes)",
             tiles, wv.n_split, part_bytes);
  dim3 grid((unsigned)tiles, (unsigned)wv.n_split);
  {
    BnProfScope prof_(BN_K_WGRAD, st);
    wgrad_kernel<float><<<grid, 256, 0, st>>>(wv);
    BN_LAUNCH_CHECK("wgrad");
  }
  BnProfScope prof_(BN_K_WGRAD_REDUCE, st);
  wgrad_reduce_kernel<128><<<dim3((unsigned)tiles * 16), 256, 0, st>>>(wv);
  BN_LAUNCH_CHECK("wgrad_reduce");
  return 0;
}

int bn_launch_skinny(SkinnyArgs &sv, bool bf, bool f16m, int64_t Mpad, int64_t m_per_block, float *part, size_t part_bytes, hipStream_t st) {
  if (sv.n_jobs == 0) return 0;
  sv.part = part;
  sv.m_per_block = (int)m_per_block;
  const int n_split = (int)ceil_div64(Mpad, m_per_block);
  BN_REQUIRE(n_split <= 256, "skinny_wgrad: %d splits (at most 256)", n_split);
  BN_REQUIRE(part && (size_t)sv.n_jobs * n_split * SK_SLAB * sizeof(float) <= part_bytes, "skinny_wgrad: %d jobs x %d splits do not fit the slab workspace",
             sv.n_jobs, n_split);
  dim3 grid((unsigned)n_split, (unsigned)sv.n_jobs);
  {
    BnProfScope prof_(BN_K_SKINNY, st);
    if (f16m) skinny_wgrad_kernel<f16><<<grid, 256, 0, st>>>(sv);
    else if (bf) skinny_wgrad_kernel<bf16><<<grid, 256, 0, st>>>(sv);
    else skinny_wgrad_kernel<float><<<grid, 256, 0, st>>>(sv);
    BN_LAUNCH_CHECK("skinny_wgrad");
  }
  BnProfScope prof_(BN_K_WGRAD_REDUCE, st);
  skinny_reduce_kernel<<<dim3((unsigned)sv.n_jobs, 4, 16), 256, 0, st>>>(sv, n_split);
  BN_LAUNCH_CHECK("skinny_reduce");
  return 0;
}
```

brdf_nerf_amd/csrc/head_fold.hip:

```cpp
#include "common.h"

struct FoldArgs {
  bn_fold_desc d;
  int tiles_per_head;
  int tiles_dw1, tiles_dwf;
};

__device__ __forceinline__ f32x4 k4_load(const float *p, int64_t sk, bool vec) {
  if (vec) return *(const f32x4 *)p;
  return f32x4{p[0], p[sk], p[2 * sk], p[3 * sk]};
}
__device__ __forceinline__ void tile_mac(f32x16 &acc, const float *A, int64_t sam, int64_t sak, const float *B, int64_t sbk, int64_t sbn,
                                         int k0, int k1, int lane) {
  const int r = lane & 31, h = lane >> 5;
  const bool a4 = sak == 1 && (sam & 3) == 0 && ((uintptr_t)A & 15) == 0;
  const bool b4 = sbk == 1 && (sbn & 3) == 0 && ((uintptr_t)B & 15) == 0;
  const float *a = A + r * sam + 4 * h * sak, *b = B + r * sbn + 4 * h * sbk;
  int k = k0;
  for (; k + 32 <= k1; k += 32) {
    f32x4 av[4], bv[4];
#pragma unroll
    for (int u = 0; u < 4; ++u) {
      av[u] = k4_load(a + (int64_t)(k + 8 * u) * sak, sak, a4);
      bv[u] = k4_load(b + (int64_t)(k + 8 * u) * sbk, sbk, b4);
    }
#pragma unroll
    for (int u = 0; u < 4; ++u)
#pragma unroll
      for (int q = 0; q < 4; ++q) acc = __builtin_amdgcn_mfma_f32_32x32x2f32(av[u][q], bv[u][q], acc, 0, 0, 0);
  }
  for (; k + 8 <= k1; k += 8) {
    const f32x4 av = k4_load(a + (int64_t)k * sak, sak, a4), bv = k4_load(b + (int64_t)k * sbk, sbk, b4);
#pragma unroll
    for (int q = 0; q < 4; ++q) acc = __builtin_amdgcn_mfma_f32_32x32x2f32(av[q], bv[q], acc, 0, 0, 0);
  }
}
__device__ __forceinline__ void tile_reduce(f32x16 &acc, float *red, int wave, int lane) {
  if (wave > 0) {
#pragma unroll
    for (int i = 0; i < 16; ++i) red[((wave - 1) * 16 + i) * 64 + lane] = acc[i];
  }
  __syncthreads();
  if (wave == 0) {
#pragma unroll
    for (int w = 0; w < 3; ++w)
#pragma unroll
      for (int i = 0; i < 16; ++i) acc[i] += red[(w * 16 + i) * 64 + lane];
  }
}

__global__ __launch_bounds__(256) void fold_kernel(const FoldArgs A) {
  __shared__ float red[3 * 16 * 64];
  const bn_fold_desc &d = A.d;
  const int tid = threadIdx.x, lane = tid & 63, wave = tid >> 6, r = lane & 31, h = lane >> 5;
  const int F = d.F, rows = d.rows;
  const int head = blockIdx.x / A.tiles_per_head, t = blockIdx.x % A.tiles_per_head;
  const float *w1 = d.w1[head];
  const int64_t ld1 = d.w1_ld[head];
  const int nt = F / 32, m0 = (t / nt) * 32, n0 = (t % nt) * 32;
  f32x16 acc;
#pragma unroll
  for (int i = 0; i < 16; ++i) acc[i] = 0.f;
  const int kq = F / 4;
  tile_mac(acc, w1 + (int64_t)m0 * ld1, ld1, 1, d.wf + n0, F, 1, wave * kq, (wave + 1) * kq, lane);
  tile_reduce(acc, red, wave, lane);
  if (wave == 0) {
#pragma unroll
    for (int i = 0; i < 16; ++i) d.w_fold[head][(int64_t)(m0 + (i & 3) + 8 * (i >> 2) + 4 * h) * F + n0 + r] = acc[i];
  }
  if (d.m[head]) {
    const int rr = tid >> 3, cc = (tid & 7) * 4;
    *(f32x4 *)(d.m[head] + (int64_t)(m0 + rr) * F + n0 + cc) = f32x4{0.f, 0.f, 0.f, 0.f};
  }
  if (n0 == 0) {
    float sum[8];
#pragma unroll
    for (int i = 0; i < 8; ++i) sum[i] = 0.f;
    const float *wr = w1 + (int64_t)(m0 + 8 * wave) * ld1;
    for (int k = lane; k < F; k += 64) {
      const float bk = d.bf[k];
#pragma unroll
      for (int i = 0; i < 8; ++i) sum[i] = fmaf(wr[(int64_t)i * ld1 + k], bk, sum[i]);
    }
#pragma unroll
    for (int i = 0; i < 8; ++i) {
#pragma unroll
      for (int o = 32; o > 0; o >>= 1) sum[i] += __shfl_xor(sum[i], o);
    }
    if (lane < 8) {
      float v = 0.f;
#pragma unroll
      for (int i = 0; i < 8; ++i) v = lane == i ? sum[i] : v;
      const int n = m0 + 8 * wave + lane;
      d.b_fold[head][n] = v + d.b1[head][n];
      if (d.s[head]) d.s[head][n] = 0.f;
    }
  }
}

__global__ __launch_bounds__(256) void unfold_kernel(const FoldArgs A) {
  __shared__ float red[3 * 16 * 64];
  const bn_fold_desc &d = A.d;
  const int tid = threadIdx.x, lane = tid & 63, wave = tid >> 6, r = lane & 31, h = lane >> 5;
  const int F = d.F, rows = d.rows, nt = F / 32;
  int b = blockIdx.x;
  f32x16 acc;
#pragma unroll
  for (int i = 0; i < 16; ++i) acc[i] = 0.f;
  if (b < A.tiles_dw1) {
    const int head = b / A.tiles_per_head, t = b % A.tiles_per_head;
    if (!d.m[head] || !d.d_w1[head]) return;
    const int m0 = (t / nt) * 32, n0 = (t % nt) * 32, kq = F / 4;
    tile_mac(acc, d.m[head] + (int64_t)m0 * F, F, 1, d.wf + (int64_t)n0 * F, 1, F, wave * kq, (wave + 1) * kq, lane);
    tile_reduce(acc, red, wave, lane);
    if (wave == 0) {
      const float bfn = d.bf[n0 + r];
#pragma unroll
      for (int i = 0; i < 16; ++i) {
        const int m = m0 + (i & 3) + 8 * (i >> 2) + 4 * h;
        float *p = d.d_w1[head] + (int64_t)m * d.d_w1_ld[head] + n0 + r;
        *p += acc[i] + d.s[head][m] * bfn;
      }
    }
    if (n0 == 0 && tid < 32 && d.d_b1[head]) d.d_b1[head][m0 + tid] += d.s[head][m0 + tid];
    return;
  }
  b -= A.tiles_dw1;
  if (b < A.tiles_dwf) {
    if (!d.d_wf) return;
    const int m0 = (b / nt) * 32, n0 = (b % nt) * 32, kq = rows / 4;
    for (int head = 0; head < d.n_heads; ++head)
      if (d.m[head])
        tile_mac(acc, d.w1[head] + m0, 1, d.w1_ld[head], d.m[head] + n0, F, 1, wave * kq, (wave + 1) * kq, lane);
    tile_reduce(acc, red, wave, lane);
    if (wave == 0) {
#pragma unroll
      for (int i = 0; i < 16; ++i) d.d_wf[(int64_t)(m0 + (i & 3) + 8 * (i >> 2) + 4 * h) * F + n0 + r] += acc[i];
    }
    if (n0 == 0 && d.d_bf) {
      const int kk = tid & 31, grp = tid >> 5;
      float sum = 0.f;
      for (int head = 0; head < d.n_heads; ++head)
        if (d.s[head])
          for (int n = grp; n < rows; n += 8) sum = fmaf(d.w1[head][(int64_t)n * d.w1_ld[head] + m0 + kk], d.s[head][n], sum);
      __syncthreads();
      red[grp * 32 + kk] = sum;
      __syncthreads();
      if (tid < 32) {
        float v = 0.f;
#pragma unroll
        for (int q = 0; q < 8; ++q) v += red[q * 32 + tid];
        d.d_bf[m0 + tid] += v;
      }
    }
    return;
  }
}

static int fold_check(const bn_fold_desc *d, const char *what) {
  BN_REQUIRE(d && d->n_heads >= 1 && d->n_heads <= BN_MAX_HEADS && d->F >= 64 && d->F % 64 == 0 && d->rows >= 32 && d->rows % 32 == 0 &&
                 d->wf && d->bf,
             "%s: bad descriptor (F=%d rows=%d heads=%d)", what, d ? d->F : 0, d ? d->rows : 0, d ? d->n_heads : 0);
  for (int i = 0; i < d->n_heads; ++i) BN_REQUIRE(d->w1[i] && d->w1_ld[i] >= d->F, "%s: head %d first-layer weight missing", what, i);
  return 0;
}

extern "C" int bn_fold_heads(const bn_fold_desc *d, void *stream) {
  if (int e = fold_check(d, "fold_heads")) return e;
  for (int i = 0; i < d->n_heads; ++i) BN_REQUIRE(d->b1[i] && d->w_fold[i] && d->b_fold[i], "fold_heads: head %d buffers missing", i);
  FoldArgs a;
  a.d = *d; a.tiles_per_head = (d->rows / 32) * (d->F / 32); a.tiles_dw1 = a.tiles_dwf = 0;
  BnProfScope prof_(BN_K_PACK, (hipStream_t)stream);
  fold_kernel<<<dim3((unsigned)(d->n_heads * a.tiles_per_head)), 256, 0, (hipStream_t)stream>>>(a);
  BN_LAUNCH_CHECK("fold_heads");
  return 0;
}

extern "C" int bn_unfold_heads(const bn_fold_desc *d, void *stream) {
  if (int e = fold_check(d, "unfold_heads")) return e;
  FoldArgs a;
  a.d = *d; a.tiles_per_head = (d->rows / 32) * (d->F / 32);
  a.tiles_dw1 = d->n_heads * a.tiles_per_head; a.tiles_dwf = (d->F / 32) * (d->F / 32);
  BnProfScope prof_(BN_K_PACK, (hipStream_t)stream);
  unfold_kernel<<<dim3((unsigned)(a.tiles_dw1 + a.tiles_dwf)), 256, 0, (hipStream_t)stream>>>(a);
  BN_LAUNCH_CHECK("unfold_heads");
  return 0;
}
```

brdf_nerf_amd/csrc/prof.h:

```cpp
#pragma once
#include <hip/hip_runtime.h>
enum { BN_K_PACK = 0, BN_K_FWD_SIGMA, BN_K_FWD_FULL, BN_K_BWD_CHAIN, BN_K_WGRAD, BN_K_SKINNY, BN_K_COMPOSITE_FWD,
       BN_K_COMPOSITE_BWD, BN_K_GUIDED, BN_K_STRATIFIED, BN_K_ADAM, BN_K_BRDF, BN_K_ADJOINT, BN_K_ADJBWD, BN_K_WGRAD_REDUCE, BN_K_COUNT };
extern bool g_bn_prof_on;
void bn_prof_start(int id, hipStream_t st);
void bn_prof_stop(hipStream_t st);
struct BnProfScope {
  hipStream_t st; bool on;
  BnProfScope(int id, hipStream_t s) : st(s), on(g_bn_prof_on) { if (on) bn_prof_start(id, st); }
  ~BnProfScope() { if (on) bn_prof_stop(st); }
};
```

brdf_nerf_amd/functions.py:

```python
import ctypes as C
import os

import torch

from . import _lib as L


def _stream():
    return C.c_void_p(torch.cuda.current_stream().cuda_stream)


def _p(t):
    if t is None:
        return None
    assert t.is_cuda and t.is_contiguous(), "C ABI needs contiguous device tensors"
    return C.c_void_p(t.data_ptr())


def _f32(t):
    return t.contiguous() if t.dtype == torch.float32 else t.float().contiguous()


class FieldSpec:

# ... 191 lines not shown
        names, grad_enabled, dirs = names_grad
        named = dict(zip(names, params))
        if t_embed is not None:
            t_embed = t_embed.detach().float().contiguous()
        pts = make_points(xyz, rays, z, dirs, t_embed)
        ref = xyz if xyz is not None else z
        out = torch.empty(pts.n_points, spec.out_channels, dtype=torch.float32, device=ref.device)
        ctx.t_grad = bool(grad_enabled and t_embed is not None and ctx.needs_input_grad[5])
        need_grad = grad_enabled and (any(p.requires_grad for p in params) or ctx.t_grad)
        stash = None
        if need_grad or spec.normal_an:
            nbytes = L.lib().bn_field_stash_bytes(C.byref(spec.desc), pts.n_points)
            stash = torch.empty(nbytes, dtype=torch.uint8, device=ref.device)
        ps = spec.params_struct(named)
        L.check(L.lib().bn_field_forward(C.byref(spec.desc), C.byref(ps), _p(packed), C.byref(pts), _p(out), _p(stash),
                                         _stream()), "bn_field_forward")
        if spec.normal_an:
            L.check(L.lib().bn_field_normals(C.byref(spec.desc), C.byref(ps), _p(packed), C.byref(pts), _p(stash), _p(out), None,
                                             1 if need_grad else 0, _stream()), "bn_field_normals")
            if not need_grad:
                stash = None
        ctx.spec, ctx.packed, ctx.names, ctx.stash = spec, packed, names, stash
        ctx.pts_t = (xyz, rays, z, dirs, t_embed)
        ctx.save_for_backward(out, *params)
        return out

    @staticmethod
    def backward(ctx, d_out):
        out, *params = ctx.saved_tensors
        spec, names = ctx.spec, ctx.names
        if ctx.stash is None:
            raise RuntimeError("FieldFunction.backward without a stash (forward ran under no_grad)")
        named = dict(zip(names, params))
        sizes = [p.numel() for p in params]
        offs, tot = [], 0
        for n in sizes:
            offs.append(tot)
            tot += (n + 3) // 4 * 4
        flat = torch.zeros(tot, dtype=torch.float32, device=out.device)
        grads = [flat[o:o + n].view(p.shape) for o, n, p in zip(offs, sizes, params)]
        named_grads = dict(zip(names, grads))
        gs = spec.params_struct(named_grads, grads=True)
        ps = spec.params_struct(named)
        xyz, rays, z, dirs, t_embed = ctx.pts_t
        pts = make_points(xyz, rays, z, dirs, t_embed)
        d_t = None
        if ctx.t_grad:
            d_t = torch.empty(pts.n_points, spec.t_dim, dtype=torch.float32, device=out.device)
            gs.d_t_embed = d_t.data_ptr()
            if rays is not None:
                d_t = d_t.view(rays.shape[0], -1, spec.t_dim)
        d_out = _f32(d_out)
        L.check(L.lib().bn_field_backward(C.byref(spec.desc), C.byref(ps), _p(ctx.packed), C.byref(pts), _p(out),
                                          _p(d_out), _p(ctx.stash), C.byref(gs), _stream()), "bn_field_backward")
        if spec.fold_feats:
            spec.unfold_grads(named, named_grads)
        ctx.stash = None
        if d_t is not None and d_t.dim() == 3:
            d_t = d_t.sum(1)
        return (None, None, None, None, None, d_t, None) + tuple(g if p.requires_grad else None
                                                                 for g, p in zip(grads, params))


class CompositeFunction(torch.autograd.Function):

    @staticmethod
    def forward(ctx, z, out, noise, noise_std):
        R, S = z.shape
        Cc = out.shape[-1] if out.dim() == 3 else 1
        dev = z.device
        alphas = torch.empty(R, S, dtype=torch.float32, device=dev)
        trans = torch.empty_like(alphas)
        weights = torch.empty_like(alphas)
        depth = torch.empty(R, dtype=torch.float32, device=dev)
        sigma_only = out.dim() == 2
        acc = None if sigma_only else torch.empty(R, Cc, dtype=torch.float32, device=dev)
        base = out.data_ptr()
        sig_ptr = C.c_void_p(base if sigma_only else base + 3 * 4)
        L.check(L.lib().bn_composite_forward(_p(z), sig_ptr, 1 if sigma_only else Cc, _p(noise), float(noise_std),
                                             None if sigma_only else _p(out), Cc, 0 if sigma_only else Cc, R, S,
                                             _p(alphas), _p(trans), _p(weights), _p(depth), _p(acc), _stream()),
                "bn_composite_forward")
        ctx.save_for_backward(z, out, noise)
        ctx.noise_std, ctx.sigma_only = float(noise_std), sigma_only
        ctx.mark_non_differentiable(alphas, trans)
        if sigma_only:
            return alphas, trans, weights, depth
        return alphas, trans, weights, depth, acc

    @staticmethod
    def backward(ctx, d_alphas, d_trans, d_weights, d_depth, d_acc=None):
        z, out, noise = ctx.saved_tensors
        R, S = z.shape
        sigma_only = ctx.sigma_only
        Cc = 1 if sigma_only else out.shape[-1]
        d_out = torch.zeros_like(out)
        base = out.data_ptr()
        dbase = d_out.data_ptr()
        sig_ptr = C.c_void_p(base if sigma_only else base + 12)
        dsig_ptr = C.c_void_p(dbase if sigma_only else dbase + 12)
        dw = None if d_weights is None else _f32(d_weights)
        dd = None if d_depth is None else _f32(d_depth)
        da = None if (d_acc is None or sigma_only) else _f32(d_acc)
        L.check(L.lib().bn_composite_backward(_p(z), sig_ptr, 1 if sigma_only else Cc, _p(noise), ctx.noise_std,
                                              None if sigma_only else _p(out), Cc, 0 if sigma_only else Cc, R, S,
                                              _p(dw), _p(dd), _p(da), dsig_ptr, 1 if sigma_only else Cc,
                                              None if sigma_only else _p(d_out), Cc, _stream()),
                "bn_composite_backward")
        return None, d_out, None, None


def composite(z, out, noise=None, noise_std=0.0):
    return CompositeFunction.apply(z.contiguous(), out.contiguous(), noise, noise_std)


def composite_forward_raw(z, out, noise=None, noise_std=0.0, bufs=None):
    R, S = z.shape
    Cc = out.shape[-1]
    dev = z.device
    b = bufs if bufs is not None else {}
    mk = lambda k, shape: b.get(k) if k in b else torch.empty(shape, dtype=torch.float32, device=dev)
    alphas, trans, weights = mk("alphas", (R, S)), mk("trans", (R, S)), mk("weights", (R, S))
    depth, acc = mk("depth", (R,)), mk("acc", (R, Cc))
    L.check(L.lib().bn_composite_forward(_p(z), C.c_void_p(out.data_ptr() + 12), Cc, _p(noise), float(noise_std), _p(out), Cc,
                                         Cc, R, S, _p(alphas), _p(trans), _p(weights), _p(depth), _p(acc), _stream()),
            "bn_composite_forward")
    return alphas, trans, weights, depth, acc


def composite_backward_raw(z, out, d_weights, d_depth, d_acc, noise=None, noise_std=0.0, d_out=None):
    R, S = z.shape
    Cc = out.shape[-1]
    if d_out is None:
        d_out = torch.empty_like(out)
    L.check(L.lib().bn_composite_backward(_p(z), C.c_void_p(out.data_ptr() + 12), Cc, _p(noise), float(noise_std), _p(out), Cc,
                                          Cc, R, S, _p(d_weights), _p(d_depth), _p(d_acc),
                                          C.c_void_p(d_out.data_ptr() + 12), Cc, _p(d_out), Cc, _stream()),
            "bn_composite_backward")
    return d_out


def field_forward_raw(spec, named_params, packed, out, stash, xyz=None, rays=None, z=None, point_offset=0, total_points=0):
    pts = make_points(xyz, rays, z, point_offset=point_offset, total_points=total_points)
    ps = spec.params_struct(named_params)
    L.check(L.lib().bn_field_forward(C.byref(spec.desc), C.byref(ps), _p(packed), C.byref(pts), _p(out), _p(stash), _stream()),
            "bn_field_forward")
    if spec.normal_an:
        L.check(L.lib().bn_field_normals(C.byref(spec.desc), C.byref(ps), _p(packed), C.byref(pts), _p(stash), _p(out), None, 1,
                                         _stream()), "bn_field_normals")
    return out


def field_backward_raw(spec, named_params, named_grads, packed, out, d_out, stash, xyz=None, rays=None, z=None, unfold=True,
                       zero_folded=True, parts=L.BN_BWD_ALL, z2=None):
    pts = make_points(xyz, rays, z, z2=z2)
    ps, gs = spec.params_struct(named_params), spec.params_struct(named_grads, grads=True)
    L.check(L.lib().bn_field_backward_parts(C.byref(spec.desc), C.byref(ps), _p(packed), C.byref(pts), _p(out), _p(d_out), _p(stash),
                                            C.byref(gs), int(parts), _stream()), "bn_field_backward")
    if spec.fold_feats and unfold:
        spec.unfold_grads(named_params, named_grads, zero=zero_folded)


def field_stash_bytes(spec, n_points):
    return L.lib().bn_field_stash_bytes(C.byref(spec.desc), int(n_points))


def lambert_loss(acc, weights, z, depth, rgbs, rgb_padding, lambda_rgb, valid_depth=None, target_depth=None,
                 target_weight=None, target_std=None, lambda_ds=0.0, usealldepth=False):
    R, S = weights.shape
    Cc = acc.shape[1]
    dev = acc.device
    ray_loss = torch.empty(R, dtype=torch.float32, device=dev)
    rgb = torch.empty(R, 3, dtype=torch.float32, device=dev)
    d_acc = torch.empty(R, Cc, dtype=torch.float32, device=dev)
    d_depth = torch.empty(R, dtype=torch.float32, device=dev)
    d_weights = torch.empty(R, S, dtype=torch.float32, device=dev)
    use = target_depth is not None and lambda_ds > 0
    f = lambda t: _f32(t).contiguous() if (use and t is not None) else None
    acc, weights, z, depth, rgbs = _f32(acc), _f32(weights), _f32(z), _f32(depth), _f32(rgbs)
    vd, td, tw, ts = f(valid_depth), f(target_depth), f(target_weight), f(target_std)
    L.check(L.lib().bn_lambert_loss(_p(acc), Cc, _p(weights), _p(z), S, _p(depth), _p(rgbs), _p(vd), _p(td), _p(tw), _p(ts),
                                    float(rgb_padding), float(lambda_rgb), float(lambda_ds), int(bool(usealldepth)), R,
                                    _p(ray_loss), _p(rgb), _p(d_acc), _p(d_depth), _p(d_weights), _stream()), "bn_lambert_loss")
    return ray_loss.sum(), rgb, d_acc, d_depth, d_weights


def stratified_z(near, far, u):
    R, S = u.shape
    near, far, u = _f32(near).reshape(R), _f32(far).reshape(R), _f32(u)
    z = torch.empty(R, S, dtype=torch.float32, device=u.device)
    L.check(L.lib().bn_stratified_z(_p(near), _p(far), 1, _p(u), R, S, _p(z), _stream()), "bn_stratified_z")
    return z


def guided_samples(z, weights, depth, u, near0, far0, d_range, use_target=None, target_depth=None, target_std=None,
                   u_target=None, target_row=None, merge=True):
    R, S = z.shape
    G = u.shape[1]
    dev = z.device
    z2 = torch.empty(R, G, dtype=torch.float32, device=dev)
    z_all = torch.empty(R, S + G, dtype=torch.float32, device=dev) if merge else None
    idx = torch.empty(R, S + G, dtype=torch.int64, device=dev) if merge else None
    if torch.is_tensor(near0):
        assert far0 is None and near0.is_cuda and near0.dtype == torch.float32 and near0.numel() == 2 and near0.is_contiguous()
        L.check(L.lib().bn_guided_samples_nf(_p(z), _p(weights), _p(depth), _p(u), R, S, G, C.c_void_p(near0.data_ptr()),
                                             float(d_range), _p(use_target), _p(target_depth), _p(target_std), _p(u_target),
                                             _p(target_row), _p(z2), _p(z_all), _p(idx), _stream()), "bn_guided_samples_nf")
        return z2, z_all, idx
    L.check(L.lib().bn_guided_samples(_p(z), _p(weights), _p(depth), _p(u), R, S, G, float(near0), float(far0),
                                      float(d_range), _p(use_target), _p(target_depth), _p(target_std), _p(u_target),
                                      _p(target_row), _p(z2), _p(z_all), _p(idx), _stream()), "bn_guided_samples")
    return z2, z_all, idx


def new_step_state(device, seed, lr):
    st = torch.zeros(L.BN_STATE_BYTES // 8, dtype=torch.int64, device=device)
    st[0] = int(seed) & 0x7FFFFFFFFFFFFFFF
    st.view(torch.float32)[4] = float(lr)
    st.view(torch.float64)[L.BN_STATE_POW_OFF // 8:L.BN_STATE_POW_OFF // 8 + 8] = 1.0
    return st


def set_adam_steps(state, steps, betas=(0.9, 0.999)):
    steps = list(steps) + [0] * (4 - len(steps))
    state.view(torch.int32)[6:10] = torch.tensor(steps, dtype=torch.int32)
    pw = [float(betas[0]) ** s for s in steps] + [float(betas[1]) ** s for s in steps]
    state.view(torch.float64)[L.BN_STATE_POW_OFF // 8:L.BN_STATE_POW_OFF // 8 + 8] = torch.tensor(pw, dtype=torch.float64)


def state_views(state):
    f, i = state.view(torch.float32), state.view(torch.int32)
    return state[1], f[4], i[6:10], f[L.BN_STATE_LOSS_OFF // 4:L.BN_STATE_LOSS_OFF // 4 + L.BN_STATE_LOSS_SLOTS]


def set_state_noise(state, noise_std):
    state.view(torch.float32)[L.BN_STATE_NOISE_OFF // 4].fill_(float(noise_std))


def state_loss_partials(state):
    return state.view(torch.float32)[L.BN_STATE_PART_OFF // 4:L.BN_STATE_PART_OFF // 4 + L.BN_STATE_LOSS_SLOTS]


def stratified_z_rng(rays, S, state, z=None, ray_offset=0, near_far=None, stream_id=None):
    src, col = (rays, 6) if near_far is None else (near_far, 0)
    R = src.shape[0]
    assert src.is_contiguous() and src.dtype == torch.float32 and src.shape[1] >= col + 2
    if z is None:
        z = torch.empty(R, S, dtype=torch.float32, device=src.device)
    base = src.data_ptr() + 4 * col
    L.check(L.lib().bn_stratified_z_rng(C.c_void_p(base), C.c_void_p(base + 4), src.shape[1], _p(state),
                                        L.BN_RNG_COARSE if stream_id is None else int(stream_id),
                                        int(ray_offset), R, S, _p(z), _stream()), "bn_stratified_z_rng")
    return z


def rng_uniform(state, stream_id, n):
    u = torch.empty(n, dtype=torch.float32, device=state.device)
    L.check(L.lib().bn_rng_uniform(_p(state), int(stream_id), n, _p(u), _stream()), "bn_rng_uniform")
    return u


def rng_normal(state, stream_id, n):
    x = torch.empty(n, dtype=torch.float32, device=state.device)
    L.check(L.lib().bn_rng_normal(_p(state), int(stream_id), n, _p(x), _stream()), "bn_rng_normal")
    return x


def noise_arg(state, noise_std, stream_id, ray_offset=0, from_state=False):
    if not noise_std:
        return None
    n = L.Noise()
    n.rng, n.noise_std, n.rng_stream, n.ray_offset = state.data_ptr(), -1.0 if from_state else float(noise_std), int(stream_id), int(ray_offset)
    n._keep = state
    return n


def _nz(noise):
    return None if noise is None else C.byref(noise)


def _strided(t):
    if t is None:
        return None, 1
    assert t.dtype == torch.float32 and t.dim() == 1 and t.is_cuda
    return C.c_void_p(t.data_ptr()), t.stride(0) if t.shape[0] > 1 else 1


def _depth_targets(use, valid_depth, target_depth, target_weight, target_std):
    return tuple(a for t in (valid_depth, target_depth, target_weight, target_std) for a in _strided(t if use else None))


def composite_guided(z, out1, G, near_far, d_range, use_target=None, target_depth=None, target_std=None, u=None, u_target=None,
                     state=None, bufs=None, want_pass1=False, ray_offset=0, sigma=None, noise=None):
    R, S = z.shape
    Cc = out1.shape[-1] if sigma is None else 1
    sig_ptr = C.c_void_p(out1.data_ptr() + 12) if sigma is None else _p(sigma)
    dev = z.device
    b = bufs if bufs is not None else {}
    mk = lambda k, shape, dt=torch.float32: b[k] if k in b else torch.empty(shape, dtype=dt, device=dev)
    z2, z_all, idx = mk("z2", (R, G)), mk("z_all", (R, S + G)), mk("idx", (R, S + G), torch.int64)
    w1 = mk("w1", (R, S)) if want_pass1 else None
    d1 = mk("d1", (R,)) if want_pass1 else None
    ut_p, ut_s = _strided(use_target)
    td_p, td_s = _strided(target_depth)
    ts_p, ts_s = _strided(target_std)
    L.check(L.lib().bn_composite_guided(_p(z), sig_ptr, Cc, R, S, G, C.c_void_p(near_far.data_ptr()),
                                        float(d_range), ut_p, ut_s, td_p, td_s, ts_p, ts_s, _p(u), _p(u_target), _p(state),
                                        L.BN_RNG_GUIDED, L.BN_RNG_GUIDED_TARGET, int(ray_offset), _p(z2), _p(z_all), _p(idx), _p(w1), _p(d1),
                                        _nz(noise), _stream()), "bn_composite_guided")
# ... 249 lines not shown
```

brdf_nerf_amd/trainer.py:

```python
import functools
import warnings
from collections import OrderedDict, namedtuple

import torch

from . import functions as Fn
from . import _lib as L
from . import losses
from .distributed import allreduce_sum_
from .rendering import shade, shade_desc, identity_desc, get_z_vals, inference, sun_far

_Block = namedtuple("_Block", "out stash z z2 s1 s2 row0")


class _Rows:

    def __init__(self, blocks, z_all, idx, src, d_all):
        self.blocks, self.z_all, self.idx, self.src, self.d_all = blocks, z_all, idx, src, d_all
        self.R, self.S1 = src[0].shape[:2]
        self.S2 = 0 if src[1] is None else src[1].shape[1]
        self.n = self.R * (self.S1 + self.S2)
        self.d_src = self.split(d_all)

    def split(self, a):
        n1 = self.R * self.S1
        return a[:n1].view(self.R, self.S1, -1), (a[n1:].view(self.R, self.S2, -1) if self.S2 else None)

    @staticmethod
    def of(a, block):
        return a[block.row0:block.row0 + block.out.shape[0]]


def _reg_lambdas(spec, reg):
    spv = float(reg.get("nr_spv", 0)) if (spec.normal_an and spec.normal_lr and abs(reg.get("nr_spv", 0)) > 1e-5) else 0.0
    return float(reg.get("hs", 0)), float(reg.get("nr_an", 0)), float(reg.get("nr_lr", 0)), spv


class FusedTrainer:
    def __init__(self, model, args, lr=5e-4, betas=(0.9, 0.999), eps=1e-8, weight_decay=0.0, lambda_rgb=1.0, ds_lambda=0.0,
                 usealldepth=False, process_group=None, strict_rng=True, reuse_coarse=True, nr_reg_an_lambda=0.0,
                 nr_reg_lr_lambda=0.0, hs_lambda=0.0, nr_spv_lambda=0.0, data_parallel=True):
        self.model, self.args = model, args
        self.reg = dict(nr_an=nr_reg_an_lambda, nr_lr=nr_reg_lr_lambda, hs=hs_lambda, nr_spv=nr_spv_lambda)
        self.fused_glue = True
        self.sanitize_grads = True
        self.lr, self.betas, self.eps, self.wd = lr, betas, eps, weight_decay
        self.lambda_rgb, self.ds_lambda, self.usealldepth = lambda_rgb, ds_lambda, usealldepth
        self.pg, self.strict_rng, self.reuse_coarse = process_group, strict_rng, reuse_coarse
        self.world = 1
        if data_parallel and (process_group is not None or (torch.distributed.is_available() and torch.distributed.is_initialized())):
            self.world = torch.distributed.get_world_size(process_group)
        self.nr_lr = model.normal in ("analystic_learned", "learned")
        self.nr_an = model.normal in ("analystic_learned", "analystic")
        self._flatten()
        self._bufs = OrderedDict()
        self._touched = None
        self.max_buf_variants = 3
        self.lean = True
        self.merge_passes = True
        self.overlap_allreduce = True
        self.ray_offset = 0
        self.keep_grads = False
        self.seed_hook = None
        self.repeatable_loss = True
        self.use_graph = True
        self.graph_after = 3
        self.max_graphs = 16
        self._graphs, self._sig_seen, self._nf_dev, self._no_graph = OrderedDict(), OrderedDict(), {}, set()
        self._graph_cap_warned = False
        self.state = Fn.new_step_state(self.flat_param.device, torch.initial_seed(), lr)
        self._rng_step, self._state_lr, self._grads_clean, self._state_noise = 0, float(lr), True, 0.0
        self._state_adam = [0, 0, 0, 0]
        self._nonfinite = torch.zeros(2, dtype=torch.int64, device=self.flat_param.device)

    def seed_draws(self, seed):
        self.state[0] = int(seed) & 0x7FFFFFFFFFFFFFFF

    def _flatten(self):
        model = self.model
        named = dict(model.named_parameters())
        base = set(model.spec(False, False, self.nr_lr, beta=False).used_param_names())
        theta = {n for n in named if n.startswith("theta_from_xyz.")}
        groups = [("base", [n for n in named if n in base]),
                  ("brdf", [n for n in named if n not in base and n not in theta]),
                  ("theta", [n for n in named if n in theta])]
        offs, tot = {}, 0
        self.groups = []
        for gname, names in groups:
            lo = tot
            for n in names:
                offs[n] = tot
                tot += (named[n].numel() + 3) // 4 * 4
            if tot > lo:
                self.groups.append((gname, lo, tot))
        self.n_base = self.groups[0][2]
        trunk = [n for n in named if n.startswith("fc_net.")]
        ends = [offs[n] + (named[n].numel() + 3) // 4 * 4 for n in trunk]
        self.n_trunk = max(ends) if trunk and max(ends) <= min([offs[n] for n in named if n not in trunk] + [tot]) else 0
        self.adam_steps = {gname: 0 for gname, _, _ in self.groups}
        dev = next(model.parameters()).device
        self.flat_param = torch.zeros(tot, dtype=torch.float32, device=dev)
        self.flat_grad = torch.zeros_like(self.flat_param)
        self.exp_avg = torch.zeros_like(self.flat_param)
        self.exp_avg_sq = torch.zeros_like(self.flat_param)
        self.grad_views = {}
        with torch.no_grad():
            for _, names in groups:
                for n in names:
                    p, o = named[n], offs[n]
                    view = self.flat_param[o:o + p.numel()].view(p.shape)
                    view.copy_(p.data)
                    p.data = view
                    self.grad_views[n] = self.flat_grad[o:o + p.numel()].view(p.shape)

    @property
    def steps_a(self):
        return self.adam_steps["base"]

    @property
    def steps_b(self):
        return self.adam_steps.get("brdf", self.adam_steps.get("theta", 0))

    def dropped_grad_elems(self):
        return tuple(int(v) for v in self._nonfinite.tolist())

    @property
    def dropped_samples(self):
        return sum(self.dropped_grad_elems())

    def _buf(self, key, shape, dtype=torch.float32):
        k = (key, tuple(shape), dtype)
        b = self._bufs.get(k)
        if b is None:
            b = torch.empty(shape, dtype=dtype, device=self.flat_param.device)
            same = [q for q in self._bufs if q[0] == key]
            for q in same[:max(0, len(same) + 1 - self.max_buf_variants)]:
                del self._bufs[q]
            self._bufs[k] = b
        else:
            self._bufs.move_to_end(k)
        if self._touched is not None:
            self._touched.append(b)
        return b

    def step(self, rays, rgbs, valid_depth=None, depths=None, depth_std=None, apply_brdf=False, apply_theta=False,
             cos_irra_on=False, depth_loss_on=True, near_far=None, regularisers=True, gsam_only=False):
        model, args = self.model, self.args
        S, G = args.n_samples, args.guided_samples
        R = rays.shape[0]
        dev = rays.device
        spec = model.spec(apply_brdf, apply_theta, self.nr_lr, self.nr_an, beta=False)
        reg0 = self.reg if regularisers else {}
        sun_on = getattr(model, "sun_v", "none") == "analystic" and apply_brdf
        sun_lean = sun_on and gsam_only and args.noise_std == 0 and args.data == "sat"
        if (self.lean and not self.strict_rng and self.reuse_coarse
                and (not sun_on or sun_lean)
                and rays.dtype == torch.float32 and rays.is_contiguous() and rays.shape[1] >= 8 and S + G <= 512):
            return self._step_lean(spec, rays, rgbs, valid_depth, depths, depth_std, apply_brdf, apply_theta, cos_irra_on,
                                   depth_loss_on, near_far, regularisers, gsam_only)
        self._grads_clean = False
        named = model.named()
        packed = model.repack(spec)
        near, far = rays[:, 6:7], rays[:, 7:8]
        rays_d = rays[:, 3:6]
        sun_d = rays[:, 8:11] if args.data == "sat" else torch.ones_like(rays[:, 0:3])
        need_noise = self.strict_rng or args.noise_std != 0
        C = spec.out_channels
        S2 = G if gsam_only else S + G
        reuse = self.reuse_coarse and not gsam_only
        with torch.no_grad():
            z = Fn.stratified_z(near, far, torch.rand(R, S, device=dev))
            noise1 = torch.randn(R, S, device=dev) if need_noise else None
            noise1 = noise1 if args.noise_std != 0 else None
            if reuse:
                out1 = self._buf("out1", (R * S, C))
                stash1 = self._buf("stash1", (Fn.field_stash_bytes(spec, R * S),), torch.uint8)
                Fn.field_forward_raw(spec, named, packed, out1, stash1, rays=rays, z=z)
                _, _, w1, d1, _ = Fn.composite_forward_raw(z, out1.view(R, S, C), noise1, args.noise_std)
            else:
                sig = Fn.field_sigma(spec, named, packed, rays=rays, z=z).view(R, S)
                _, _, w1, d1 = Fn.composite(z, sig, noise1, args.noise_std)
            sun_res = None
            if sun_on:
                if not gsam_only:
                    raise NotImplementedError("--sun_v analystic needs gsam_only=True (SURVEY quirk 2: the reference raises a "
                                              "shape error with the merged S+G sample set)")
                far_sun = sun_far(d1, rays_d, sun_d)
                z_sun = get_z_vals(G, dev, far_sun * 0.01, far_sun)
                sun_rays = torch.cat([rays[:, 0:3] + rays_d * d1.unsqueeze(-1), sun_d], -1).contiguous()
                rs, _ = inference(model, args, None, z_sun, rays_d=sun_d, mode="train", sigma_only=True, _rays=sun_rays,
                                  _packed=packed)
                sun_res = {"sun": rs["transparency"].unsqueeze(-1), "weights_sc": rs["weights"]}
            u = torch.rand(R, G, device=dev)
            use_t = tdep = tstd = u_t = trow = None
            if valid_depth is not None:
                valid = (valid_depth > 0) if self.strict_rng else None
                u_t = torch.rand(R, G, device=dev)
                tdep = depths[:, 0].float().contiguous()
                tstd = depth_std.float().reshape(-1).contiguous()
                if self.strict_rng:
                    use_t = valid.float().contiguous()
                    trow = (torch.cumsum(valid.int(), 0) - 1).clamp_min(0).int().contiguous()
                else:
                    use_t = valid_depth if (valid_depth.dtype == torch.float32 and valid_depth.is_contiguous()) \
                        else (valid_depth > 0).float().contiguous()
            near0, far0 = near_far if near_far is not None else (rays[0, 6:8], None)
            z2, z_all, idx = Fn.guided_samples(z, w1, d1, u, near0, far0, args.std_range, use_t, tdep, tstd, u_t, trow,
                                               merge=not gsam_only)
            if gsam_only:
                z_all = z2
            noise2 = torch.randn(R, S2, device=dev) if need_noise else None
            noise2 = noise2 if args.noise_std != 0 else None
# ... 164 lines not shown
                None if depths is None else depths.data_ptr(), None if depth_std is None else depth_std.data_ptr(),
                nf.data_ptr(), use_ds, tuple(active), float(self.ds_lambda), float(self.lambda_rgb), bool(self.usealldepth),
                L.deterministic(), int(self.ray_offset), bool(self.keep_grads), bool(self.merge_passes), bool(apply_brdf),
                bool(cos_irra_on), float(reg.get("hs", 0)), bool(self.sanitize_grads), float(reg.get("nr_an", 0)),
                float(reg.get("nr_lr", 0)), bool(gsam_only), self._noise_f32() != 0.0, float(reg.get("nr_spv", 0)),
                bool(self.repeatable_loss),
                str(getattr(model, "sun_v", "none")), bool(model.MultiBRDF), str(args.data),
                int(args.n_samples), int(args.guided_samples), float(args.std_range), float(model.rgb_padding),
                int(getattr(args, "funcH", 1)), float(getattr(args, "hpk_scl", 1.0)), float(getattr(args, "fresnel_f0", 0.04)),
                int(getattr(args, "shell_hapke", 0)), tuple(float(b) for b in self.betas), float(self.eps), float(self.wd))

    def _replay_or_capture(self, sig, body, keep):
        ent = self._graphs.get(sig)
        if ent is not None:
            self._graphs.move_to_end(sig)
            ent[0].replay()
            return ent[1]
        n = self._sig_seen.pop(sig, 0) + 1
        self._sig_seen[sig] = n
        while len(self._sig_seen) > 256:
            self._sig_seen.popitem(last=False)
        if n <= self.graph_after or sig in self._no_graph:
            return body()
        if len(self._graphs) >= self.max_graphs:
            self._graphs.popitem(last=False)
            if not self._graph_cap_warned:
                warnings.warn(f"brdf_nerf_amd: more than {self.max_graphs} distinct training-step signatures were captured; the "
                              f"least recently used graph is dropped (inputs whose addresses change every step defeat the replay: "
                              f"keep batches in fixed buffers, e.g. RayTable.next_batch(out=...))")
                self._graph_cap_warned = True
        g = torch.cuda.CUDAGraph()
        torch.cuda.synchronize()
        self._touched = []
        try:
            with torch.cuda.graph(g):
                out = body()
        except Exception as e:
            warnings.warn(f"brdf_nerf_amd: HIP graph capture of the training step failed ({type(e).__name__}: {e}); "
                          f"this step signature runs eagerly")
            self._no_graph.add(sig)
            self._touched = None
            torch.cuda.synchronize()
            return body()
        self._graphs[sig] = (g, out, tuple(keep + self._touched))
        self._touched = None
        g.replay()
        return out

    def _lean_body(self, spec, rays, rgbs, valid_depth, depths, depth_std, apply_brdf, cos_irra_on, use_ds, nf, reg, active,
                   gsam_only=False):
        model, args = self.model, self.args
        S, G = args.n_samples, args.guided_samples
        R, C = rays.shape[0], spec.out_channels
        st = self.state
        named = model.named()
        sun_on = gsam_only and getattr(model, "sun_v", "none") == "analystic" and apply_brdf
        with torch.no_grad():
            packed = model.repack(spec)
            z = Fn.stratified_z_rng(rays, S, st, self._buf("z", (R, S)), ray_offset=self.ray_offset)
            tile = 64 if spec.dtype == L.BN_F32 else 128
            merged = self.merge_passes and (R * S) % tile == 0 and not gsam_only
            n_all = R * (S + G)
            has_t = valid_depth is not None
            guide = (valid_depth, depths[:, 0], depth_std) if has_t else (None, None, None)
            nz1 = Fn.noise_arg(st, self._noise_f32(), L.BN_RNG_NOISE_COARSE, self.ray_offset, from_state=True)
            nz2 = Fn.noise_arg(st, self._noise_f32(), L.BN_RNG_NOISE_MERGED, self.ray_offset, from_state=True)
            bufs = {"z2": self._buf("z2", (R, G)), "z_all": self._buf("z_all", (R, S + G)),
                    "idx": self._buf("idx", (R, S + G), torch.int64)}
            if gsam_only:
                sig1 = Fn.field_sigma(spec, named, packed, rays=rays, z=z, out=self._buf("sig1", (R * S,)))
                if sun_on:
                    bufs = dict(bufs, w1=self._buf("w1", (R, S)), d1=self._buf("d1", (R,)))
                cg = Fn.composite_guided(z, None, G, nf, args.std_range, *guide, state=st, bufs=bufs,
                                         ray_offset=self.ray_offset, sigma=sig1.view(R, S), noise=nz1, want_pass1=sun_on)
                z2 = cg[0]
                if sun_on:
                    d1 = cg[4]
                    rays_d, sun_d = rays[:, 3:6], rays[:, 8:11]
                    far_sun = sun_far(d1, rays_d, sun_d)
                    z_sun = Fn.stratified_z_rng(None, G, st, self._buf("z_sun", (R, G)), ray_offset=self.ray_offset,
                                                near_far=torch.cat([far_sun * 0.01, far_sun], -1).contiguous(), stream_id=L.BN_RNG_SUN)
                    sun_rays = torch.cat([rays[:, 0:3] + rays_d * d1.unsqueeze(-1), sun_d], -1).contiguous()
                    sig_sun = Fn.field_sigma(spec, named, packed, rays=sun_rays, z=z_sun)
                    sun_T = Fn.composite(z_sun, sig_sun.view(R, G), None, 0.0)[1]
                if self.seed_hook is not None:
                    self.seed_hook("z2", z2)
                out2 = self._buf("out2", (R * G, C))
                stash2 = self._buf("stash2", (Fn.field_stash_bytes(spec, R * G),), torch.uint8)
                Fn.field_forward_raw(spec, named, packed, out2, stash2, rays=rays, z=z2)
                rows = _Rows([_Block(out2, stash2, z2, None, G, 0, 0)], z2, None, (out2.view(R, G, C), None), self._buf("d_all", (R * G, C)))
            else:
                if merged:
                    out_all = self._buf("out_all", (n_all, C))
                    stash_all = self._buf("stash_all", (Fn.field_stash_bytes(spec, n_all),), torch.uint8)
                    out1 = out_all[:R * S]
                    Fn.field_forward_raw(spec, named, packed, out_all, stash_all, rays=rays, z=z, point_offset=0, total_points=n_all)
                else:
                    out1 = self._buf("out1", (R * S, C))
                    stash1 = self._buf("stash1", (Fn.field_stash_bytes(spec, R * S),), torch.uint8)
                    Fn.field_forward_raw(spec, named, packed, out1, stash1, rays=rays, z=z)
                z2, z_all, idx = Fn.composite_guided(z, out1.view(R, S, C), G, nf, args.std_range, *guide, state=st, bufs=bufs,
                                                     ray_offset=self.ray_offset, noise=nz1)
                if self.seed_hook is not None:
                    self.seed_hook("z2", z2)
                if merged:
                    Fn.field_forward_raw(spec, named, packed, out_all, stash_all, rays=rays, z=z2, point_offset=R * S, total_points=n_all)
                    if self.seed_hook is not None:
                        self.seed_hook("out_all", out_all)
                    out2 = out_all[R * S:]
                    blocks = [_Block(out_all, stash_all, z, z2, S, G, 0)]
                else:
                    out2 = self._buf("out2", (R * G, C))
                    stash2 = self._buf("stash2", (Fn.field_stash_bytes(spec, R * G),), torch.uint8)
                    Fn.field_forward_raw(spec, named, packed, out2, stash2, rays=rays, z=z2)
                    blocks = [_Block(out1, stash1, z, None, S, 0, 0), _Block(out2, stash2, z2, None, G, 0, R * S)]
                rows = _Rows(blocks, z_all, idx, (out1.view(R, S, C), out2.view(R, G, C)), self._buf("d_all", (n_all, C)))
            hs, nr_an, nr_lr, spv = regs = _reg_lambdas(spec, reg)
            lambda_ds = self.ds_lambda if use_ds else 0.0
            targets = (valid_depth, depths[:, 0], depths[:, 1], depth_std) if use_ds else (None, None, None, None)
            tail = functools.partial(self._ray_tail, spec, rows, rays, rgbs, targets, lambda_ds, nz2)
            kdesc = shade_desc(model, args, spec, apply_brdf, cos_irra_on)
            multi = bool(model.MultiBRDF) and apply_brdf
            sun_rows = sun_on and (multi or kdesc.kind == L.BN_SHADE_LAMBERT)
            if (multi and kdesc.kind != L.BN_SHADE_LAMBERT) or sun_rows:
                bdesc = shade_desc(model, args, spec, apply_brdf, cos_irra_on, irr=sun_T.reshape(-1)) if sun_rows else kdesc
                sun_col = 8 if args.data == "sat" else -1
                with_reg = hs > 0 or spv != 0.0 or nr_an > 0 or nr_lr > 0
                Bd = self._buf("B_full" if with_reg else "B_4", (rows.n, C if with_reg else 4))
                d_B = self._buf("d_Bfull" if with_reg else "d_B", Bd.shape)
                for b in rows.blocks:
                    Fn.sample_brdf(bdesc, b.out, rays, R * b.s1, b.s1, b.s2, rows.of(Bd, b), sun_col=sun_col)
                if with_reg:
                    loss, rgb = tail(rows.split(Bd), rows.split(d_B), regs=regs,
                                     desc=identity_desc(C, self.lambda_rgb, lambda_ds, hs, self.usealldepth))
                else:
                    loss, rgb = tail(rows.split(Bd), rows.split(d_B), pad=0.0)
                for b in rows.blocks:
                    Fn.sample_brdf(bdesc, b.out, rays, R * b.s1, b.s1, b.s2, rows.of(rows.d_all, b), backward_of=rows.of(d_B, b), sun_col=sun_col)
                if self.sanitize_grads:
                    Fn.count_nonfinite(rows.d_all, self._nonfinite)
                    torch.nan_to_num_(rows.d_all, nan=0.0, posinf=0.0, neginf=0.0)
            elif len(spec.heads) == 1 and not spec.normal_an and not spec.normal_lr and hs <= 0:
                loss, rgb = tail(rows.src, rows.d_src, pad=model.rgb_padding)
            else:
                desc = shade_desc(model, args, spec, apply_brdf, cos_irra_on, self.lambda_rgb, lambda_ds, hs, self.usealldepth,
                                  irr=sun_T[:, -1] if sun_on else None)
                loss, rgb = tail(rows.src, rows.d_src, desc=desc, regs=regs, sun_d=rays[:, 8:11] if args.data == "sat" else None)
        if self.seed_hook is not None:
            self.seed_hook("d_all", rows.d_all)
        with torch.no_grad():
            def backward(parts, last):
                for b in rows.blocks:
                    Fn.field_backward_raw(spec, named, self.grad_views, packed, b.out, rows.of(rows.d_all, b), b.stash, rays=rays, z=b.z,
                                          z2=b.z2, unfold=last and b is rows.blocks[-1], zero_folded=False, parts=parts)
            if self.world > 1 and self.overlap_allreduce and 0 < self.n_trunk < self.flat_grad.numel():
                import torch.distributed as dist
                backward(L.BN_BWD_CHAIN | L.BN_BWD_WGRAD_TRUNK, False)
                wa = dist.all_reduce(self.flat_grad[:self.n_trunk], op=dist.ReduceOp.SUM, group=self.pg, async_op=True)
                backward(L.BN_BWD_WGRAD_HEADS | L.BN_BWD_SKINNY, True)
                wb = dist.all_reduce(self.flat_grad[self.n_trunk:], op=dist.ReduceOp.SUM, group=self.pg, async_op=True)
                wa.wait()
                wb.wait()
            else:
                backward(L.BN_BWD_ALL, True)
                if self.world > 1:
                    allreduce_sum_(self.flat_grad, self.pg)
            keep = self.keep_grads
            Fn.adam_multi(self.flat_param, self.flat_grad, self.exp_avg, self.exp_avg_sq, [(lo, hi) for _, lo, hi in self.groups],
                          active, st, self.betas, self.eps, self.wd, 1.0 / self.world, zero_grad=not keep)
        return loss, rgb

    def _ray_tail(self, spec, rows, rays, rgbs, targets, lambda_ds, noise, src, grads, pad=None, desc=None, regs=None, sun_d=None):
        R, C = rays.shape[0], spec.out_channels
        z_all, idx = rows.z_all, rows.idx
        ray_loss = self._buf("ray_loss", (R,)) if self.repeatable_loss else None
        loss_acc = None if self.repeatable_loss else Fn.state_loss_partials(self.state)
        nonfinite = self._nonfinite if self.sanitize_grads else None
        if desc is None:
            rgb = self._buf("rgb", (R, 3))
            Fn.lambert_tail(z_all, idx, *src, rgbs, pad, self.lambda_rgb, *grads, *targets, lambda_ds, self.usealldepth,
                            ray_loss=ray_loss, loss_acc=loss_acc, rgb=rgb, nonfinite=nonfinite, noise=noise)
        else:
            hs, nr_an, nr_lr, spv = regs
            nreg = Fn.normal_reg(rays[:, 3:6], spec.ch_normal_an if spec.normal_an else -1, spec.ch_normal_lr if spec.normal_lr else -1,
                                 nr_an, nr_lr, lambda_spv=spv,
                                 spv_ray=self._buf("spv_ray", (R, 2)) if spv else None, spv_tot=self._buf("spv_tot", (4,)) if spv else None)
            o = Fn.merged_composite_forward(z_all, idx, *src,
                                            {k: self._buf("m_" + k, sh) for k, sh in (("depth", (R,)), ("acc", (R, C)),
                                                                                      ("wsum", (R,)), ("var", (R,)), ("reg", (R,)))},
                                            want=("depth", "acc", "wsum", "var"), nreg=nreg, noise=noise)
            sb = {k: self._buf("s_" + k, sh) for k, sh in (("rgb", (R, 3)), ("d_acc", (R, C)), ("d_wsum", (R,)), ("d_depth", (R,)))}
            g = Fn.ray_shade_loss(desc, o["acc"], o["wsum"], o["depth"], o["var"], rays[:, 3:6], sun_d, rgbs, sb, *targets,
                                  ray_loss=ray_loss, loss_acc=loss_acc, nonfinite=nonfinite, extra_loss=o.get("reg"))
            rgb = g["rgb"]
            if spv:
                Fn.normal_spv_reduce(nreg, R, z_all.shape[1], ray_loss=ray_loss, loss_acc=loss_acc)
            Fn.merged_composite_backward(z_all, idx, *src, None, g["d_depth"], g["d_acc"], *grads, d_wsum=g["d_wsum"],
                                         nonfinite=nonfinite, hs_scale=hs / R if hs > 0 else 0.0, depth=o["depth"], nreg=nreg, noise=noise)
        return (ray_loss.sum() if self.repeatable_loss else None), rgb

    def _adam(self, apply_brdf, apply_theta=False):
        scale = 1.0 / self.world
        for (gname, lo, hi), on in zip(self.groups, self._active_groups(apply_brdf, apply_theta)):
            if not on:
                continue
            self.adam_steps[gname] += 1
            Fn.adam_step(self.flat_param[lo:hi], self.flat_grad[lo:hi], self.exp_avg[lo:hi], self.exp_avg_sq[lo:hi],
                         self.adam_steps[gname], self.lr, self.betas, self.eps, self.wd, scale)
```

include/brdfnerf_hip.h:

```cpp
#ifndef BRDFNERF_HIP_H
#define BRDFNERF_HIP_H

#include <stddef.h>
#include <stdint.h>

#ifdef __cplusplus
extern "C" {
#endif

#define BN_ABI_VERSION 7
#define BN_MAX_LAYERS 12
#define BN_MAX_HEADS 6

typedef enum { BN_OK = 0, BN_EINVAL = -1, BN_EUNSUPPORTED = -2, BN_ELAUNCH = -3 } bn_status;
typedef enum { BN_F32 = 0, BN_BF16 = 1, BN_F16 = 2 } bn_dtype;
typedef enum { BN_ACT_SIN = 0, BN_ACT_RELU = 1 } bn_act;
typedef enum {
  BN_HEAD_PLAIN = 0,
  BN_HEAD_RPV_K = 1,
  BN_HEAD_RPV_THETA = 2,
  BN_HEAD_HAPKE_THETA = 3,
  BN_HEAD_TILE3 = 4,
  BN_HEAD_BETA = 5
} bn_head_kind;
// ... 75 lines not shown
                      const bn_points *pts, const float *out, const float *d_out, void *stash,
                      const bn_field_grads *grads, void *stream);

enum { BN_BWD_CHAIN = 1, BN_BWD_WGRAD_TRUNK = 2, BN_BWD_WGRAD_HEADS = 4, BN_BWD_SKINNY = 8, BN_BWD_ALL = 15 };
int bn_field_backward_parts(const bn_field_desc *desc, const bn_field_params *params, const void *packed,
                            const bn_points *pts, const float *out, const float *d_out, void *stash,
                            const bn_field_grads *grads, int32_t parts, void *stream);

int bn_composite_forward(const float *z, const float *sigma, int64_t sigma_stride, const float *noise,
                         float noise_std, const float *chan, int64_t chan_stride, int32_t C, int64_t R, int32_t S,
                         float *alphas, float *trans, float *weights, float *depth, float *acc, void *stream);
int bn_composite_backward(const float *z, const float *sigma, int64_t sigma_stride, const float *noise,
                          float noise_std, const float *chan, int64_t chan_stride, int32_t C, int64_t R, int32_t S,
                          const float *d_weights, const float *d_depth, const float *d_acc, float *d_sigma,
                          int64_t d_sigma_stride, float *d_chan, int64_t d_chan_stride, void *stream);

int bn_lambert_loss(const float *acc, int32_t C, const float *weights, const float *z, int32_t S, const float *depth,
                    const float *rgbs, const float *valid_depth, const float *target_depth, const float *target_weight,
                    const float *target_std, float rgb_padding, float lambda_rgb, float lambda_ds, int32_t usealldepth,
                    int64_t R, float *ray_loss, float *rgb, float *d_acc, float *d_depth, float *d_weights, void *stream);

int bn_stratified_z(const float *near, const float *far, int64_t nf_stride, const float *u, int64_t R, int32_t S,
                    float *z, void *stream);

int bn_guided_samples(const float *z, const float *weights, const float *depth, const float *u, int64_t R,
                      int32_t S, int32_t G, float near0, float far0, float d_range, const float *use_target,
                      const float *target_depth, const float *target_std, const float *u_target,
                      const int32_t *target_row, float *z2_sorted, float *z_all, int64_t *sort_idx, void *stream);

int bn_guided_samples_nf(const float *z, const float *weights, const float *depth, const float *u, int64_t R,
                         int32_t S, int32_t G, const float *near_far, float d_range, const float *use_target,
                         const float *target_depth, const float *target_std, const float *u_target,
                         const int32_t *target_row, float *z2_sorted, float *z_all, int64_t *sort_idx, void *stream);

#define BN_BRDF_AUX 16
int bn_brdf_rpv_forward(const float *l, const float *v, const float *n, const float *w, const float *k,
                        const float *theta, const float *rhoc, int64_t N, float *brdf, float *aux, void *stream);
int bn_brdf_rpv_backward(const float *l, const float *v, const float *n, const float *w, const float *k,
                         const float *theta, const float *rhoc, const float *d_brdf, int64_t N, float *d_n,
                         float *d_w, float *d_k, float *d_theta, float *d_rhoc, void *stream);
int bn_brdf_hapke_forward(const float *l, const float *v, const float *n, const float *w, const float *b,
                          const float *c, const float *theta , float hpk_scl, int32_t shell, int64_t N,
                          float *brdf, float *aux, void *stream);
int bn_brdf_hapke_backward(const float *l, const float *v, const float *n, const float *w, const float *b,
                           const float *c, const float *theta, float hpk_scl, int32_t shell, const float *d_brdf,
                           int64_t N, float *d_n, float *d_w, float *d_b, float *d_c, float *d_theta, void *stream);
int bn_brdf_microfacet_forward(const float *l, const float *v, const float *n, const float *albedo,
                               const float *rough , float f0, int64_t N, float *brdf, float *aux,
                               void *stream);
int bn_brdf_microfacet_backward(const float *l, const float *v, const float *n, const float *albedo,
                                const float *rough, float f0, const float *d_brdf, int64_t N, float *d_n,
                                float *d_albedo, float *d_rough, void *stream);

int bn_adam_step(float *param, const float *grad, float *exp_avg, float *exp_avg_sq, int64_t n, float lr,
                 float beta1, float beta2, float eps, float weight_decay, int32_t step, float grad_scale,
                 void *stream);


#define BN_STATE_BYTES 1024
#define BN_STATE_NOISE_OFF 40
#define BN_STATE_LOSS_OFF 64
#define BN_STATE_LOSS_SLOTS 64
#define BN_STATE_POW_OFF 320
#define BN_STATE_PART_OFF 512
#define BN_ADAM_MAX_GROUPS 4
enum { BN_RNG_COARSE = 1, BN_RNG_GUIDED = 2, BN_RNG_GUIDED_TARGET = 3, BN_RNG_NOISE_COARSE = 4, BN_RNG_NOISE_MERGED = 5, BN_RNG_SUN = 6 };

typedef struct {
  const unsigned long long *rng;
  float noise_std;
  uint32_t rng_stream;
  int64_t ray_offset;
} bn_noise;
int bn_rng_normal(const unsigned long long *rng, uint32_t rng_stream, int64_t n, float *x, void *stream);

int bn_stratified_z_rng(const float *near, const float *far, int64_t nf_stride, const unsigned long long *rng,
                        uint32_t rng_stream, int64_t ray_offset, int64_t R, int32_t S, float *z, void *stream);
int bn_rng_uniform(const unsigned long long *rng, uint32_t rng_stream, int64_t n, float *u, void *stream);

int bn_composite_guided(const float *z, const float *sigma, int64_t sigma_stride, int64_t R, int32_t S, int32_t G,
                        const float *near_far, float d_range, const float *use_target, int64_t ut_stride,
                        const float *target_depth, int64_t td_stride, const float *target_std, int64_t ts_stride,
                        const float *u, const float *u_target, const unsigned long long *rng, uint32_t rng_u,
                        uint32_t rng_ut, int64_t ray_offset, float *z2_sorted, float *z_all, int64_t *sort_idx, float *weights,
                        float *depth, const bn_noise *noise, void *stream);

typedef struct {
  const float *rays_d;
  int64_t rd_stride;
  int32_t ch_an, ch_lr;
  float lambda_an, lambda_lr;
  float lambda_spv;
  int32_t spv_ch_an, spv_ch_lr;
  float *spv_ray;
  float *spv_tot;
} bn_normal_reg;
int bn_normal_spv_reduce(const float *spv_ray, int64_t R, int32_t S, float lambda_spv, float *spv_tot, float *ray_loss,
                         float *loss_acc, void *stream);
int bn_merged_composite_forward(const float *z, const int64_t *sort_idx, const float *out1, const float *out2, int32_t S1,
                                int32_t S2, int32_t C, int64_t R, float *alphas, float *trans, float *weights, float *depth,
                                float *acc, float *wsum, float *var, const bn_normal_reg *nreg, float *reg_out,
                                const bn_noise *noise, void *stream);
int bn_merged_composite_backward(const float *z, const int64_t *sort_idx, const float *out1, const float *out2, int32_t S1,
                                 int32_t S2, int32_t C, int64_t R, const float *d_weights, const float *d_depth,
                                 const float *d_acc, const float *d_wsum, float hs_scale, const float *depth,
                                 const bn_normal_reg *nreg, float *d_out1, float *d_out2, unsigned long long *nonfinite,
                                 const bn_noise *noise, void *stream);

enum { BN_SHADE_LAMBERT = 0, BN_SHADE_RPV = 1, BN_SHADE_HAPKE = 2, BN_SHADE_MICROFACET = 3 };
typedef struct {
  int32_t kind, C, ch_normal, ch_p0, ch_p1, ch_p2;
  int32_t rhoc_is_albedo, shell, cos_irradiance, usealldepth;
  float hpk_scl, f0, rgb_padding, lambda_rgb, lambda_ds, lambda_hs;
  const float *irr;
  int64_t irr_stride;
} bn_shade_desc;
int bn_ray_shade_loss(const bn_shade_desc *desc, const float *acc, const float *wsum, const float *depth, const float *var,
                      const float *rays_d, int64_t rd_stride, const float *sun_d, int64_t sd_stride, const float *rgbs,
                      const float *valid_depth, int64_t v_stride, const float *target_depth, int64_t td_stride,
                      const float *target_weight, int64_t tw_stride, const float *target_std, int64_t ts_stride, int64_t R,
                      float *rgb, float *ray_loss, float *loss_acc, int32_t loss_slots, float *d_acc, float *d_wsum,
                      float *d_depth, unsigned long long *nonfinite, const float *extra_loss, void *stream);
int bn_ray_shade_dirs(const bn_shade_desc *desc, const float *acc, const float *wsum, const float *rays_d, int64_t rd_stride,
                      const float *sun, const float *view, int64_t R, int32_t K, float *rgb, float *brdf, void *stream);
int bn_lambert_tail(const float *z, const int64_t *sort_idx, const float *out1, const float *out2, int32_t S1, int32_t S2,
                    int32_t C, int64_t R, const float *rgbs, const float *valid_depth, int64_t v_stride,
                    const float *target_depth, int64_t td_stride, const float *target_weight, int64_t tw_stride,
                    const float *target_std, int64_t ts_stride, float rgb_padding, float lambda_rgb, float lambda_ds,
                    int32_t usealldepth, float *ray_loss, float *loss_acc, int32_t loss_slots, float *rgb,
                    float *weights, float *depth, float *d_out1, float *d_out2, unsigned long long *nonfinite,
                    const bn_noise *noise, void *stream);

int bn_sample_brdf_forward(const bn_shade_desc *desc, const float *X, const float *rays, int64_t R, int64_t ray_stride,
                           int32_t sun_col, int64_t N, int64_t n1, int32_t S1, int32_t S2, float *B, int32_t b_stride, void *stream);
int bn_sample_brdf_backward(const bn_shade_desc *desc, const float *X, const float *rays, int64_t R, int64_t ray_stride,
                            int32_t sun_col, int64_t N, int64_t n1, int32_t S1, int32_t S2, const float *dB, int32_t b_stride,
                            float *dX, void *stream);

typedef struct {
  int32_t n_heads, F, rows;
  const float *wf, *bf;
  const float *w1[BN_MAX_HEADS];
  int64_t w1_ld[BN_MAX_HEADS];
  const float *b1[BN_MAX_HEADS];
  float *w_fold[BN_MAX_HEADS], *b_fold[BN_MAX_HEADS];
  float *m[BN_MAX_HEADS], *s[BN_MAX_HEADS];
  float *d_w1[BN_MAX_HEADS];
  int64_t d_w1_ld[BN_MAX_HEADS];
  float *d_b1[BN_MAX_HEADS];
  float *d_wf, *d_bf;
} bn_fold_desc;
int bn_fold_heads(const bn_fold_desc *d, void *stream);
int bn_unfold_heads(const bn_fold_desc *d, void *stream);

int bn_adam_multi(float *param, float *grad, float *exp_avg, float *exp_avg_sq, int32_t n_groups, const int64_t *lo,
                  const int64_t *hi, const int32_t *active, float beta1, float beta2, float eps, float weight_decay,
                  float grad_scale, int32_t zero_grad, void *state, void *stream);

int bn_count_nonfinite(const float *x, int64_t n, unsigned long long *counts, void *stream);

int bn_device_faults(unsigned int *faults, void *stream);

#define BN_PROF_IDS 14
int bn_prof_enable(int on);
int bn_prof_collect(double *ms_sum, int *count, int n_ids);

#ifdef __cplusplus
}
#endif
#endif
```

profiles/ab_kernels.py:

```python
import os
import statistics
import sys

sys.path.insert(0, os.path.dirname(os.path.dirname(os.path.abspath(__file__))))
import torch
import bench
from brdf_nerf_amd import _lib as L
from brdf_nerf_amd import functions as Fn
from brdf_nerf_amd import load_model
from brdf_nerf_amd.trainer import FusedTrainer


def main():
    tags = [a for a in sys.argv[1:] if not a.startswith("--")]
    opt = dict(a[2:].split("=", 1) for a in sys.argv[1:] if a.startswith("--") and "=" in a)
    config, dtype, rounds = opt.get("config", "lambert"), opt.get("dtype", "bf16"), int(opt.get("rounds", 5))
    n_rays = int(opt.get("rays", 4096))
    dev = torch.device("cuda", 0)
    here = os.path.dirname(os.path.dirname(os.path.abspath(__file__)))
    variants = {}
    for tag in tags:
        build, _, attrs = tag.partition(":")
        path = os.path.join(here, "brdf_nerf_amd", "libbrdfnerf_hip.so") if build == "default" else \
            os.path.join(here, "brdf_nerf_amd", "build", build, "libbrdfnerf_hip.so")
        h = L.load(path, baseline=build.startswith("r0"))
        L.use(h)
        args = bench.make_args(n_rays, 64, 64, dtype, **bench.CONFIG_FLAGS[config][0])
        torch.manual_seed(0)
        model = load_model(args).to(dev)
        tr = FusedTrainer(model, args, lr=5e-4, ds_lambda=10.0, strict_rng=False)
        tr.use_graph = False
        for kv in filter(None, attrs.split(",")):
            k, v = kv.split("=")
            if k == "zero_stash":
                spec0 = model.spec(*[bool(x) for x in (bench.CONFIG_FLAGS[config][1]["apply_brdf"], bench.CONFIG_FLAGS[config][1]["apply_theta"])],
                                   tr.nr_lr, tr.nr_an, beta=False)
                tr._buf("stash_all", (Fn.field_stash_bytes(spec0, n_rays * 128),), torch.uint8).zero_()
                continue
            setattr(tr, k, {"True": True, "False": False}.get(v, int(v) if v.lstrip("-").isdigit() else v))
        variants[tag] = (h, args, model, tr)
    b = bench.synthetic_batch(n_rays, 1, dev)
    flags = bench.CONFIG_FLAGS[config][1]
    z = torch.sort(torch.rand(n_rays, 128, device=dev) * 2, -1)[0]
    times = {tag: {} for tag in tags}
    counts = {tag: {} for tag in tags}
    for rnd in range(rounds + 1):
        for tag in tags:
            h, args, model, tr = variants[tag]
            L.use(h)
            L.prof_enable(True)
            for _ in range(3):
                tr.step(b["rays"], b["rgbs"], valid_depth=b["valid_depth"], depths=b["depths"], depth_std=b["depth_std"],
                        near_far=(0.0, 2.0), **flags)
            spec = model.spec(False, False, False)
            packed = model.repack(spec)
            for _ in range(4):
                Fn.field_sigma(spec, model.named(), packed, rays=b["rays"], z=z)
            torch.cuda.synchronize()
            prof = L.prof_collect()
            L.prof_enable(False)
            if rnd == 0:
                continue
            for k, (ms, n) in prof.items():
                times[tag].setdefault(k, []).append(ms / n)
                counts[tag][k] = n / (4 if k == "field_fwd_sigma" else 3)
    import time
    step_ms = {tag: [] for tag in tags}
    for rnd in range(rounds + 1):
        for tag in tags:
            h, args, model, tr = variants[tag]
            L.use(h)
            tr.use_graph = True
            for _ in range(6):
                tr.step(b["rays"], b["rgbs"], valid_depth=b["valid_depth"], depths=b["depths"], depth_std=b["depth_std"],
                        near_far=(0.0, 2.0), **flags)
            torch.cuda.synchronize()
            t0 = time.perf_counter()
            for _ in range(30):
                tr.step(b["rays"], b["rgbs"], valid_depth=b["valid_depth"], depths=b["depths"], depth_std=b["depth_std"],
                        near_far=(0.0, 2.0), **flags)
            torch.cuda.synchronize()
            if rnd:
                step_ms[tag].append((time.perf_counter() - t0) / 30 * 1e3)
    keys = ["pack", "field_fwd_sigma", "field_fwd_full", "field_bwd_chain", "wgrad", "skinny_wgrad", "wgrad_reduce", "field_adjoint", "field_adjoint_bwd",
            "composite_fwd", "composite_bwd", "brdf", "guided_samples", "stratified_z", "adam"]
    print(f"config {config} dtype {dtype} rays {n_rays}: launches per step x ms per launch, median (min) over {rounds} alternating rounds")
    print(f"{'kernel':>18} " + " ".join(f"{t[:26]:>26}" for t in tags))
    for k in keys:
        if not any(k in times[t] for t in tags):
            continue
        row = []
        for t in tags:
            v = times[t].get(k)
            row.append(f"{counts[t][k]:g} x {statistics.median(v):.4f} ({min(v):.4f})" if v else "-")
        print(f"{k:>18} " + " ".join(f"{c:>26}" for c in row))
    print(f"{'step (wall, ms)':>18} " + " ".join(f"{statistics.median(step_ms[t]):.4f} ({min(step_ms[t]):.4f})".rjust(26) for t in tags))


if __name__ == "__main__":
    main()
```

Measured before the change: 613,900 rays/s.

## Merge wgrad reduce into skinny wgrad launch and skinny reduce into unfold

New measurement: 614,200 rays/s (median of 6 runs). Within noise of the previous version (+0.0%).

```diff
diff --git a/brdf_nerf_amd/_lib.py b/brdf_nerf_amd/_lib.py
--- a/brdf_nerf_amd/_lib.py
+++ b/brdf_nerf_amd/_lib.py
@@ -103,6 +103,8 @@
                                     fptr, C.POINTER(FieldGrads), fptr]),
     "bn_field_backward_parts": (C.c_int, [C.POINTER(FieldDesc), C.POINTER(FieldParams), fptr, C.POINTER(Points), fptr, fptr,
                                           fptr, C.POINTER(FieldGrads), C.c_int32, fptr]),
+    "bn_field_backward_merged": (C.c_int, [C.POINTER(FieldDesc), C.POINTER(FieldParams), fptr, C.POINTER(Points), fptr, fptr,
+                                           fptr, C.POINTER(FieldGrads), C.c_int32, fptr, fptr]),
     "bn_field_normals": (C.c_int, [C.POINTER(FieldDesc), C.POINTER(FieldParams), fptr, C.POINTER(Points), fptr, fptr, fptr,
                                    C.c_int32, fptr]),
     "bn_composite_forward": (C.c_int, [fptr, fptr, C.c_int64, fptr, C.c_float, fptr, C.c_int64, C.c_int32, C.c_int64,
@@ -157,7 +159,8 @@
 }
 
 PROF_NAMES = ["pack", "field_fwd_sigma", "field_fwd_full", "field_bwd_chain", "wgrad", "skinny_wgrad", "composite_fwd",
-              "composite_bwd", "guided_samples", "stratified_z", "adam", "brdf", "field_adjoint", "field_adjoint_bwd", "wgrad_reduce"]
+              "composite_bwd", "guided_samples", "stratified_z", "adam", "brdf", "field_adjoint", "field_adjoint_bwd", "wgrad_reduce",
+              "reduce_unfold"]
 
 
 def prof_enable(on):
diff --git a/brdf_nerf_amd/csrc/field.h b/brdf_nerf_amd/csrc/field.h
--- a/brdf_nerf_amd/csrc/field.h
+++ b/brdf_nerf_amd/csrc/field.h
@@ -160,6 +160,11 @@
   if (m_per_block) *m_per_block = mpb;
   return ceil_div64(Mpad, mpb);
 }
+static inline size_t bn_skpart_bytes(const FieldGeom &g, int64_t Mpad) {
+  int64_t sk_splits = ceil_div64(Mpad, g.BM);
+  if (sk_splits > 256) sk_splits = 256;
+  return (size_t)10 * (size_t)sk_splits * (4 * 512 + 4) * 4;
+}
 static inline size_t bn_wgpart_bytes(const FieldGeom &g, int64_t Mpad, size_t esz) {
   const bool half = esz != 4;
   const int64_t tl = half ? 256 : 128, ft = (g.F + tl - 1) / tl;
@@ -169,10 +174,7 @@
   const int64_t by_points = tiles_bound * bn_wgrad_splits(half, 1, Mpad, nullptr);
   if (by_points < slabs) slabs = by_points;
   const size_t wg = (size_t)slabs * (size_t)(tl * tl + tl) * 4;
-  int64_t sk_splits = ceil_div64(Mpad, g.BM);
-  if (sk_splits > 256) sk_splits = 256;
-  const size_t sk = (size_t)10 * (size_t)sk_splits * (4 * 512 + 4) * 4;
-  return wg > sk ? wg : sk;
+  return bn_pad(wg, 256) + bn_skpart_bytes(g, Mpad);
 }
 
 static inline void bn_make_stash_layout(const FieldGeom &g, int64_t n_points, int BM, size_t esz, StashLayout *s) {
diff --git a/brdf_nerf_amd/csrc/field_bwd.hip b/brdf_nerf_amd/csrc/field_bwd.hip
--- a/brdf_nerf_amd/csrc/field_bwd.hip
+++ b/brdf_nerf_amd/csrc/field_bwd.hip
@@ -1,5 +1,6 @@
 #include "field_kernels.h"
 #include "field_wgrad.h"
+#include "head_fold.h"
 
 int bn_field_adjoint_backward(const bn_field_desc *desc, const bn_field_params *params, const void *packed, const bn_points *pts,
                               const float *d_out, void *stash, void *stream);
@@ -473,9 +474,25 @@
   return bn_field_backward_parts(desc, params, packed, pts, out, d_out, stash, G, BN_BWD_ALL, stream);
 }
 
+static int field_backward_impl(const bn_field_desc *desc, const bn_field_params *params, const void *packed, const bn_points *pts,
+                               const float *out, const float *d_out, void *stash, const bn_field_grads *G, int32_t parts,
+                               bool merged, const bn_fold_desc *unfold, void *stream);
+
 extern "C" int bn_field_backward_parts(const bn_field_desc *desc, const bn_field_params *params, const void *packed,
                                        const bn_points *pts, const float *out, const float *d_out, void *stash,
                                        const bn_field_grads *G, int32_t parts, void *stream) {
+  return field_backward_impl(desc, params, packed, pts, out, d_out, stash, G, parts, false, nullptr, stream);
+}
+
+extern "C" int bn_field_backward_merged(const bn_field_desc *desc, const bn_field_params *params, const void *packed,
+                                        const bn_points *pts, const float *out, const float *d_out, void *stash,
+                                        const bn_field_grads *G, int32_t parts, const bn_fold_desc *unfold, void *stream) {
+  return field_backward_impl(desc, params, packed, pts, out, d_out, stash, G, parts, true, unfold, stream);
+}
+
+static int field_backward_impl(const bn_field_desc *desc, const bn_field_params *params, const void *packed, const bn_points *pts,
+                               const float *out, const float *d_out, void *stash, const bn_field_grads *G, int32_t parts,
+                               bool merged, const bn_fold_desc *unfold, void *stream) {
   BwdArgs a;
   if (int e = bn_make_geom(desc, &a.g)) return e;
   if (const int f = bn_field_fault_seen()) {
@@ -593,10 +610,16 @@
     add(S + sl.dG[0], g.pass_N[0], g.H2, S + sl.dirpe, g.KD, g.KT0, G->head1_wt, (int)G->head1_wt_ld, nullptr, g.H2, g.TD);
   }
   BN_REQUIRE(w.n_jobs <= BN_MAX_WGRAD_JOBS, "field_backward: too many wgrad jobs");
-  float *wgpart = (float *)(S + sl.wgpart);
-  if (w.n_jobs > 0)
-    if (int e = bn_launch_wgrad(w, bf, f16m, sl.Mpad, wgpart, sl.wgpart_bytes, st)) return e;
-  if (!(parts & BN_BWD_SKINNY)) return 0;
+  const size_t skpart_bytes = bn_skpart_bytes(g, sl.Mpad), wgslab_bytes = sl.wgpart_bytes - skpart_bytes;
+  float *wgpart = (float *)(S + sl.wgpart), *skpart = (float *)(S + sl.wgpart + wgslab_bytes);
+  FoldArgs ufa;
+  if (unfold)
+    if (int e = bn_unfold_args(unfold, &ufa)) return e;
+  if (!(parts & BN_BWD_SKINNY)) {
+    if (w.n_jobs > 0)
+      if (int e = bn_launch_wgrad(w, bf, f16m, sl.Mpad, wgpart, wgslab_bytes, st)) return e;
+    return unfold ? bn_unfold_heads(unfold, stream) : 0;
+  }
   SkinnyArgs s;
   s.n_jobs = 0; s.Mpad = sl.Mpad; s.amax = amax; s.part = nullptr;
   for (int i = 0; i < BN_MAX_SKINNY_JOBS; ++i) { s.job[i].scale_sel = 0; s.job[i].unit_dpre = 0; }
@@ -631,6 +654,9 @@
     for (int c = 0; c < 4; ++c) { j.out[c] = nullptr; j.bias[c] = nullptr; }
     for (int c = 0; c < j.nc; ++c) { j.out[c] = G->head_w2[hd] + (size_t)c * g.H2; j.bias[c] = G->head_b2[hd] ? G->head_b2[hd] + c : nullptr; }
   }
+  const bool ride = merged && s.n_jobs > 0;
+  if (w.n_jobs > 0)
+    if (int e = bn_launch_wgrad(w, bf, f16m, sl.Mpad, wgpart, wgslab_bytes, st, !ride)) return e;
   if (s.n_jobs > 0) {
     int skinny_splits = SKINNY_SPLITS;
     {
@@ -640,8 +666,13 @@
     }
     int64_t smpb = ceil_div64(ceil_div64(sl.Mpad, skinny_splits), BM) * BM;
     s.m_per_block = (int)smpb;
-    if (int e = bn_launch_skinny(s, bf, f16m, sl.Mpad, smpb, wgpart, sl.wgpart_bytes, st)) return e;
-  }
+    if (ride) {
+      if (int e = bn_launch_skinny_merged(s, w.n_jobs > 0 ? &w : nullptr, unfold ? &ufa : nullptr, bf, f16m, sl.Mpad, smpb, skpart,
+                                          skpart_bytes, st)) return e;
+    } else if (int e = bn_launch_skinny(s, bf, f16m, sl.Mpad, smpb, skpart, skpart_bytes, st)) return e;
+  }
+  if (unfold && !ride)
+    if (int e = bn_unfold_heads(unfold, stream)) return e;
   if (g.TD > 0 && G->d_t_embed) {
     BN_REQUIRE(params->head1_wt && params->head1_wt_ld >= g.TD && g.H2 <= 256, "field_backward: head1_wt missing (beta)");
     const int64_t M = pts->n_points;
diff --git a/brdf_nerf_amd/csrc/field_wgrad.h b/brdf_nerf_amd/csrc/field_wgrad.h
--- a/brdf_nerf_amd/csrc/field_wgrad.h
+++ b/brdf_nerf_amd/csrc/field_wgrad.h
@@ -33,6 +33,16 @@
 #define WG_SLAB256 (256 * 256 + 256)
 #define WG_SLAB128 (128 * 128 + 128)
 #define SK_SLAB (4 * 512 + 4)
+struct WgradReduceJob { float *C, *bias; int ldc, N, K, scale_sel; };
+struct WgradReduceArgs {
+  WgradReduceJob job[BN_MAX_WGRAD_JOBS];
+  int tile0[BN_MAX_WGRAD_JOBS + 1];
+  int n_jobs, n_split;
+  const float *amax;
+  const float *part;
+  int chain_next[BN_MAX_WGRAD_JOBS];
+  unsigned char head[BN_MAX_WGRAD_JOBS];
+};
 
 struct SkinnyJob {
   const void *X;
@@ -55,6 +65,9 @@
   float *part;
 };
 
-int bn_launch_wgrad(WgradArgs &wv, bool bf, bool f16m, int64_t Mpad, float *part, size_t part_bytes, hipStream_t st);
+int bn_launch_wgrad(WgradArgs &wv, bool bf, bool f16m, int64_t Mpad, float *part, size_t part_bytes, hipStream_t st, bool reduce = true);
 int bn_launch_skinny(SkinnyArgs &sv, bool bf, bool f16m, int64_t Mpad, int64_t m_per_block, float *part, size_t part_bytes, hipStream_t st);
+struct FoldArgs;
+int bn_launch_skinny_merged(SkinnyArgs &sv, const WgradArgs *wv, const FoldArgs *unfold, bool bf, bool f16m, int64_t Mpad,
+                            int64_t m_per_block, float *part, size_t part_bytes, hipStream_t st);
 unsigned int bn_bwd_fault_read(hipStream_t st);
diff --git a/brdf_nerf_amd/csrc/field_wgrad.hip b/brdf_nerf_amd/csrc/field_wgrad.hip
--- a/brdf_nerf_amd/csrc/field_wgrad.hip
+++ b/brdf_nerf_amd/csrc/field_wgrad.hip
@@ -1,5 +1,6 @@
 #include "field_kernels.h"
 #include "field_wgrad.h"
+#include "head_fold.h"
 
 
 __device__ __forceinline__ float wg_unscale(const float *amax, int sel) {
@@ -354,13 +355,11 @@
 }
 
 
-template <typename T> __global__ __launch_bounds__(256) void skinny_wgrad_kernel(const SkinnyArgs A) {
-  const SkinnyJob &J = A.job[blockIdx.y];
-  const float osc = wg_unscale(A.amax, J.scale_sel);
-  const int64_t mb = (int64_t)blockIdx.x * A.m_per_block;
+template <typename T> __device__ __forceinline__ void skinny_wgrad_body(const SkinnyArgs &A, int split, int jb, int n_split, float *red) {
+  const SkinnyJob &J = A.job[jb];
+  const int64_t mb = (int64_t)split * A.m_per_block;
   const int64_t me = mb + A.m_per_block < A.Mpad ? mb + A.m_per_block : A.Mpad;
   const int tid = threadIdx.x;
-  __shared__ float red[4 * 512 + 4];
   for (int i = tid; i < 4 * 512 + 4; i += 256) red[i] = 0.f;
   __syncthreads();
   if (J.native) {
@@ -466,23 +465,27 @@
   }
   }
   __syncthreads();
-  float *SP = A.part + ((size_t)blockIdx.y * gridDim.x + blockIdx.x) * SK_SLAB;
+  float *SP = A.part + ((size_t)jb * n_split + split) * SK_SLAB;
   for (int i = tid; i < J.nc * J.K; i += 256) {
     const int c = i / J.K, k = i % J.K;
     SP[c * 512 + k] = red[c * 512 + k];
   }
   if (tid < 4) SP[4 * 512 + tid] = tid < J.nc ? red[4 * 512 + tid] : 0.f;
 }
-
-template <int TILE> __global__ __launch_bounds__(256) void wgrad_reduce_kernel(const WgradArgs A) {
+template <typename T> __global__ __launch_bounds__(256) void skinny_wgrad_kernel(const SkinnyArgs A) {
+  __shared__ float red[4 * 512 + 4];
+  skinny_wgrad_body<T>(A, (int)blockIdx.x, (int)blockIdx.y, (int)gridDim.x, red);
+}
+
+template <int TILE, typename ARGS> __device__ __forceinline__ void wgrad_reduce_body(const ARGS &A, int bid) {
   constexpr int NB = TILE / 64;
   constexpr int SLAB = TILE * TILE + TILE;
   constexpr int SUBS = TILE * TILE / 4 / 256;
-  const int tt = blockIdx.x / SUBS, sub = blockIdx.x % SUBS, tid = threadIdx.x;
+  const int tt = bid / SUBS, sub = bid % SUBS, tid = threadIdx.x;
   int jb = 0;
   while (jb + 1 < A.n_jobs && tt >= A.tile0[jb + 1]) ++jb;
   if (!A.head[jb]) return;
-  const WgradJob &J = A.job[jb];
+  const auto &J = A.job[jb];
   const int t = tt - A.tile0[jb];
   const int tiles_k = (J.K + TILE - 1) / TILE;
   const int n0 = (t / tiles_k) * TILE, k0 = (t % tiles_k) * TILE;
@@ -527,10 +530,20 @@
     if (dst) dst[n0 + tid] += v;
   }
 }
-
-__global__ __launch_bounds__(256) void skinny_reduce_kernel(const SkinnyArgs A, int n_split) {
-  __shared__ float part[8][32], bpart[256];
-  const int jb = blockIdx.x, c = blockIdx.y, k0 = blockIdx.z * 32, tid = threadIdx.x, kk = tid & 31, g = tid >> 5;
+template <int TILE> __global__ __launch_bounds__(256) void wgrad_reduce_kernel(const WgradArgs A) {
+  wgrad_reduce_body<TILE>(A, (int)blockIdx.x);
+}
+
+template <typename T, int TILE> __global__ __launch_bounds__(256)
+void skinny_wgrad_reduce_kernel(const SkinnyArgs S, int n_split, int n_skinny_blocks, const WgradReduceArgs W) {
+  __shared__ float red[4 * 512 + 4];
+  const int b = (int)blockIdx.x;
+  if (b < n_skinny_blocks) skinny_wgrad_body<T>(S, b % n_split, b / n_split, n_split, red);
+  else wgrad_reduce_body<TILE>(W, b - n_skinny_blocks);
+}
+
+__device__ __forceinline__ void skinny_reduce_body(const SkinnyArgs &A, int n_split, int jb, int c, int k0, float (*part)[32], float *bpart) {
+  const int tid = threadIdx.x, kk = tid & 31, g = tid >> 5;
   const SkinnyJob &J = A.job[jb];
   if (c >= J.nc || !J.out[c] || k0 >= J.K) return;
   for (int j2 = 0; j2 < jb; ++j2)
@@ -576,6 +589,18 @@
   if (g == 0 && k0 + kk < J.K) J.out[c][k0 + kk] += v;
   if (k0 == 0 && tid == 0 && J.bias[c]) *J.bias[c] += vb;
 }
+__global__ __launch_bounds__(256) void skinny_reduce_kernel(const SkinnyArgs A, int n_split) {
+  __shared__ float part[8][32], bpart[256];
+  skinny_reduce_body(A, n_split, (int)blockIdx.x, (int)blockIdx.y, (int)blockIdx.z * 32, part, bpart);
+}
+
+__global__ __launch_bounds__(256) void skinny_reduce_unfold_kernel(const SkinnyArgs S, int n_split, const FoldArgs F, int n_unfold_tiles) {
+  __shared__ float red[3 * 16 * 64];
+  const int b = (int)blockIdx.x;
+  if (b < n_unfold_tiles) { unfold_body(F, b, red); return; }
+  const int q = b - n_unfold_tiles;
+  skinny_reduce_body(S, n_split, q / 64, (q / 16) & 3, (q & 15) * 32, (float (*)[32])red, red + 8 * 32);
+}
 
 static void wg_chain(WgradArgs &wv) {
   for (int j = 0; j < wv.n_jobs; ++j) { wv.chain_next[j] = -1; wv.head[j] = 1; }
@@ -589,7 +614,7 @@
   }
 }
 
-int bn_launch_wgrad(WgradArgs &wv, bool bf, bool f16m, int64_t Mpad, float *part, size_t part_bytes, hipStream_t st) {
+int bn_launch_wgrad(WgradArgs &wv, bool bf, bool f16m, int64_t Mpad, float *part, size_t part_bytes, hipStream_t st, bool reduce) {
   if (wv.n_jobs == 0) { wv.tile0[0] = 0; return 0; }
   BN_REQUIRE(part, "wgrad: no slab workspace");
   wv.part = part;
@@ -617,6 +642,7 @@
       else wgrad256_kernel<bf16><<<grd, blk, lds, st>>>(wv, (int)n_split, n_blocks);
       BN_LAUNCH_CHECK("wgrad256");
     }
+    if (!reduce) return 0;
     BnProfScope prof_(BN_K_WGRAD_REDUCE, st);
     wgrad_reduce_kernel<256><<<dim3((unsigned)tiles * 64), 256, 0, st>>>(wv);
     BN_LAUNCH_CHECK("wgrad_reduce");
@@ -637,6 +663,7 @@
     wgrad_kernel<float><<<grid, 256, 0, st>>>(wv);
     BN_LAUNCH_CHECK("wgrad");
   }
+  if (!reduce) return 0;
   BnProfScope prof_(BN_K_WGRAD_REDUCE, st);
   wgrad_reduce_kernel<128><<<dim3((unsigned)tiles * 16), 256, 0, st>>>(wv);
   BN_LAUNCH_CHECK("wgrad_reduce");
@@ -664,3 +691,53 @@
   BN_LAUNCH_CHECK("skinny_reduce");
   return 0;
 }
+
+int bn_launch_skinny_merged(SkinnyArgs &sv, const WgradArgs *wv, const FoldArgs *unfold, bool bf, bool f16m, int64_t Mpad,
+                            int64_t m_per_block, float *part, size_t part_bytes, hipStream_t st) {
+  BN_REQUIRE(sv.n_jobs > 0, "skinny_wgrad (merged): no skinny job to carry the neighbours");
+  sv.part = part;
+  sv.m_per_block = (int)m_per_block;
+  const int n_split = (int)ceil_div64(Mpad, m_per_block);
+  BN_REQUIRE(n_split <= 256, "skinny_wgrad: %d splits (at most 256)", n_split);
+  BN_REQUIRE(part && (size_t)sv.n_jobs * n_split * SK_SLAB * sizeof(float) <= part_bytes, "skinny_wgrad: %d jobs x %d splits do not fit the slab workspace",
+             sv.n_jobs, n_split);
+  const int n_skinny = n_split * sv.n_jobs;
+  {
+    BnProfScope prof_(BN_K_SKINNY, st);
+    if (wv && wv->n_jobs > 0) {
+      const size_t wg_floats = (size_t)wv->tile0[wv->n_jobs] * wv->n_split * (bf ? WG_SLAB256 : WG_SLAB128);
+      BN_REQUIRE(part >= wv->part + wg_floats || part + (size_t)n_skinny * SK_SLAB <= wv->part, "skinny_wgrad (merged): the slab workspaces overlap");
+      WgradReduceArgs r;
+      for (int j = 0; j < wv->n_jobs; ++j) {
+        const WgradJob &J = wv->job[j];
+        r.job[j] = WgradReduceJob{J.C, J.bias, J.ldc, J.N, J.K, J.scale_sel};
+        r.tile0[j] = wv->tile0[j]; r.chain_next[j] = wv->chain_next[j]; r.head[j] = wv->head[j];
+      }
+      r.tile0[wv->n_jobs] = wv->tile0[wv->n_jobs];
+      r.n_jobs = wv->n_jobs; r.n_split = wv->n_split; r.amax = wv->amax; r.part = wv->part;
+      const int tiles = wv->tile0[wv->n_jobs];
+      const dim3 grid((unsigned)(n_skinny + tiles * (bf ? 64 : 16)));
+      if (f16m) skinny_wgrad_reduce_kernel<f16, 256><<<grid, 256, 0, st>>>(sv, n_split, n_skinny, r);
+      else if (bf) skinny_wgrad_reduce_kernel<bf16, 256><<<grid, 256, 0, st>>>(sv, n_split, n_skinny, r);
+      else skinny_wgrad_reduce_kernel<float, 128><<<grid, 256, 0, st>>>(sv, n_split, n_skinny, r);
+      BN_LAUNCH_CHECK("skinny_wgrad_reduce");
+    } else {
+      const dim3 grid((unsigned)n_split, (unsigned)sv.n_jobs);
+      if (f16m) skinny_wgrad_kernel<f16><<<grid, 256, 0, st>>>(sv);
+      else if (bf) skinny_wgrad_kernel<bf16><<<grid, 256, 0, st>>>(sv);
+      else skinny_wgrad_kernel<float><<<grid, 256, 0, st>>>(sv);
+      BN_LAUNCH_CHECK("skinny_wgrad");
+    }
+  }
+  if (unfold) {
+    BnProfScope prof_(BN_K_REDUCE_UNFOLD, st);
+    const int n_unfold = unfold->tiles_dw1 + unfold->tiles_dwf;
+    skinny_reduce_unfold_kernel<<<dim3((unsigned)(n_unfold + sv.n_jobs * 64)), 256, 0, st>>>(sv, n_split, *unfold, n_unfold);
+    BN_LAUNCH_CHECK("skinny_reduce_unfold");
+  } else {
+    BnProfScope prof_(BN_K_WGRAD_REDUCE, st);
+    skinny_reduce_kernel<<<dim3((unsigned)sv.n_jobs, 4, 16), 256, 0, st>>>(sv, n_split);
+    BN_LAUNCH_CHECK("skinny_reduce");
+  }
+  return 0;
+}
diff --git a/brdf_nerf_amd/csrc/head_fold.h b/brdf_nerf_amd/csrc/head_fold.h
--- /dev/null
+++ b/brdf_nerf_amd/csrc/head_fold.h
@@ -0,0 +1,110 @@
+#pragma once
+#include "common.h"
+
+struct FoldArgs {
+  bn_fold_desc d;
+  int tiles_per_head;
+  int tiles_dw1, tiles_dwf;
+};
+
+__device__ __forceinline__ f32x4 k4_load(const float *p, int64_t sk, bool vec) {
+  if (vec) return *(const f32x4 *)p;
+  return f32x4{p[0], p[sk], p[2 * sk], p[3 * sk]};
+}
+__device__ __forceinline__ void tile_mac(f32x16 &acc, const float *A, int64_t sam, int64_t sak, const float *B, int64_t sbk, int64_t sbn,
+                                         int k0, int k1, int lane) {
+  const int r = lane & 31, h = lane >> 5;
+  const bool a4 = sak == 1 && (sam & 3) == 0 && ((uintptr_t)A & 15) == 0;
+  const bool b4 = sbk == 1 && (sbn & 3) == 0 && ((uintptr_t)B & 15) == 0;
+  const float *a = A + r * sam + 4 * h * sak, *b = B + r * sbn + 4 * h * sbk;
+  int k = k0;
+  for (; k + 32 <= k1; k += 32) {
+    f32x4 av[4], bv[4];
+#pragma unroll
+    for (int u = 0; u < 4; ++u) {
+      av[u] = k4_load(a + (int64_t)(k + 8 * u) * sak, sak, a4);
+      bv[u] = k4_load(b + (int64_t)(k + 8 * u) * sbk, sbk, b4);
+    }
+#pragma unroll
+    for (int u = 0; u < 4; ++u)
+#pragma unroll
+      for (int q = 0; q < 4; ++q) acc = __builtin_amdgcn_mfma_f32_32x32x2f32(av[u][q], bv[u][q], acc, 0, 0, 0);
+  }
+  for (; k + 8 <= k1; k += 8) {
+    const f32x4 av = k4_load(a + (int64_t)k * sak, sak, a4), bv = k4_load(b + (int64_t)k * sbk, sbk, b4);
+#pragma unroll
+    for (int q = 0; q < 4; ++q) acc = __builtin_amdgcn_mfma_f32_32x32x2f32(av[q], bv[q], acc, 0, 0, 0);
+  }
+}
+__device__ __forceinline__ void tile_reduce(f32x16 &acc, float *red, int wave, int lane) {
+  if (wave > 0) {
+#pragma unroll
+    for (int i = 0; i < 16; ++i) red[((wave - 1) * 16 + i) * 64 + lane] = acc[i];
+  }
+  __syncthreads();
+  if (wave == 0) {
+#pragma unroll
+    for (int w = 0; w < 3; ++w)
+#pragma unroll
+      for (int i = 0; i < 16; ++i) acc[i] += red[(w * 16 + i) * 64 + lane];
+  }
+}
+
+__device__ __forceinline__ void unfold_body(const FoldArgs &A, int b, float *red) {
+  const bn_fold_desc &d = A.d;
+  const int tid = threadIdx.x, lane = tid & 63, wave = tid >> 6, r = lane & 31, h = lane >> 5;
+  const int F = d.F, rows = d.rows, nt = F / 32;
+  f32x16 acc;
+#pragma unroll
+  for (int i = 0; i < 16; ++i) acc[i] = 0.f;
+  if (b < A.tiles_dw1) {
+    const int head = b / A.tiles_per_head, t = b % A.tiles_per_head;
+    if (!d.m[head] || !d.d_w1[head]) return;
+    const int m0 = (t / nt) * 32, n0 = (t % nt) * 32, kq = F / 4;
+    tile_mac(acc, d.m[head] + (int64_t)m0 * F, F, 1, d.wf + (int64_t)n0 * F, 1, F, wave * kq, (wave + 1) * kq, lane);
+    tile_reduce(acc, red, wave, lane);
+    if (wave == 0) {
+      const float bfn = d.bf[n0 + r];
+#pragma unroll
+      for (int i = 0; i < 16; ++i) {
+        const int m = m0 + (i & 3) + 8 * (i >> 2) + 4 * h;
+        float *p = d.d_w1[head] + (int64_t)m * d.d_w1_ld[head] + n0 + r;
+        *p += acc[i] + d.s[head][m] * bfn;
+      }
+    }
+    if (n0 == 0 && tid < 32 && d.d_b1[head]) d.d_b1[head][m0 + tid] += d.s[head][m0 + tid];
+    return;
+  }
+  b -= A.tiles_dw1;
+  if (b < A.tiles_dwf) {
+    if (!d.d_wf) return;
+    const int m0 = (b / nt) * 32, n0 = (b % nt) * 32, kq = rows / 4;
+    for (int head = 0; head < d.n_heads; ++head)
+      if (d.m[head])
+        tile_mac(acc, d.w1[head] + m0, 1, d.w1_ld[head], d.m[head] + n0, F, 1, wave * kq, (wave + 1) * kq, lane);
+    tile_reduce(acc, red, wave, lane);
+    if (wave == 0) {
+#pragma unroll
+      for (int i = 0; i < 16; ++i) d.d_wf[(int64_t)(m0 + (i & 3) + 8 * (i >> 2) + 4 * h) * F + n0 + r] += acc[i];
+    }
+    if (n0 == 0 && d.d_bf) {
+      const int kk = tid & 31, grp = tid >> 5;
+      float sum = 0.f;
+      for (int head = 0; head < d.n_heads; ++head)
+        if (d.s[head])
+          for (int n = grp; n < rows; n += 8) sum = fmaf(d.w1[head][(int64_t)n * d.w1_ld[head] + m0 + kk], d.s[head][n], sum);
+      __syncthreads();
+      red[grp * 32 + kk] = sum;
+      __syncthreads();
+      if (tid < 32) {
+        float v = 0.f;
+#pragma unroll
+        for (int q = 0; q < 8; ++q) v += red[q * 32 + tid];
+        d.d_bf[m0 + tid] += v;
+      }
+    }
+    return;
+  }
+}
+
+int bn_unfold_args(const bn_fold_desc *d, FoldArgs *a);
diff --git a/brdf_nerf_amd/csrc/head_fold.hip b/brdf_nerf_amd/csrc/head_fold.hip
--- a/brdf_nerf_amd/csrc/head_fold.hip
+++ b/brdf_nerf_amd/csrc/head_fold.hip
@@ -1,53 +1,4 @@
-#include "common.h"
-
-struct FoldArgs {
-  bn_fold_desc d;
-  int tiles_per_head;
-  int tiles_dw1, tiles_dwf;
-};
-
-__device__ __forceinline__ f32x4 k4_load(const float *p, int64_t sk, bool vec) {
-  if (vec) return *(const f32x4 *)p;
-  return f32x4{p[0], p[sk], p[2 * sk], p[3 * sk]};
-}
-__device__ __forceinline__ void tile_mac(f32x16 &acc, const float *A, int64_t sam, int64_t sak, const float *B, int64_t sbk, int64_t sbn,
-                                         int k0, int k1, int lane) {
-  const int r = lane & 31, h = lane >> 5;
-  const bool a4 = sak == 1 && (sam & 3) == 0 && ((uintptr_t)A & 15) == 0;
-  const bool b4 = sbk == 1 && (sbn & 3) == 0 && ((uintptr_t)B & 15) == 0;
-  const float *a = A + r * sam + 4 * h * sak, *b = B + r * sbn + 4 * h * sbk;
-  int k = k0;
-  for (; k + 32 <= k1; k += 32) {
-    f32x4 av[4], bv[4];
-#pragma unroll
-    for (int u = 0; u < 4; ++u) {
-      av[u] = k4_load(a + (int64_t)(k + 8 * u) * sak, sak, a4);
-      bv[u] = k4_load(b + (int64_t)(k + 8 * u) * sbk, sbk, b4);
-    }
-#pragma unroll
-    for (int u = 0; u < 4; ++u)
-#pragma unroll
-      for (int q = 0; q < 4; ++q) acc = __builtin_amdgcn_mfma_f32_32x32x2f32(av[u][q], bv[u][q], acc, 0, 0, 0);
-  }
-  for (; k + 8 <= k1; k += 8) {
-    const f32x4 av = k4_load(a + (int64_t)k * sak, sak, a4), bv = k4_load(b + (int64_t)k * sbk, sbk, b4);
-#pragma unroll
-    for (int q = 0; q < 4; ++q) acc = __builtin_amdgcn_mfma_f32_32x32x2f32(av[q], bv[q], acc, 0, 0, 0);
-  }
-}
-__device__ __forceinline__ void tile_reduce(f32x16 &acc, float *red, int wave, int lane) {
-  if (wave > 0) {
-#pragma unroll
-    for (int i = 0; i < 16; ++i) red[((wave - 1) * 16 + i) * 64 + lane] = acc[i];
-  }
-  __syncthreads();
-  if (wave == 0) {
-#pragma unroll
-    for (int w = 0; w < 3; ++w)
-#pragma unroll
-      for (int i = 0; i < 16; ++i) acc[i] += red[(w * 16 + i) * 64 + lane];
-  }
-}
+#include "head_fold.h"
 
 __global__ __launch_bounds__(256) void fold_kernel(const FoldArgs A) {
   __shared__ float red[3 * 16 * 64];
@@ -100,61 +51,7 @@
 
 __global__ __launch_bounds__(256) void unfold_kernel(const FoldArgs A) {
   __shared__ float red[3 * 16 * 64];
-  const bn_fold_desc &d = A.d;
-  const int tid = threadIdx.x, lane = tid & 63, wave = tid >> 6, r = lane & 31, h = lane >> 5;
-  const int F = d.F, rows = d.rows, nt = F / 32;
-  int b = blockIdx.x;
-  f32x16 acc;
-#pragma unroll
-  for (int i = 0; i < 16; ++i) acc[i] = 0.f;
-  if (b < A.tiles_dw1) {
-    const int head = b / A.tiles_per_head, t = b % A.tiles_per_head;
-    if (!d.m[head] || !d.d_w1[head]) return;
-    const int m0 = (t / nt) * 32, n0 = (t % nt) * 32, kq = F / 4;
-    tile_mac(acc, d.m[head] + (int64_t)m0 * F, F, 1, d.wf + (int64_t)n0 * F, 1, F, wave * kq, (wave + 1) * kq, lane);
-    tile_reduce(acc, red, wave, lane);
-    if (wave == 0) {
-      const float bfn = d.bf[n0 + r];
-#pragma unroll
-      for (int i = 0; i < 16; ++i) {
-        const int m = m0 + (i & 3) + 8 * (i >> 2) + 4 * h;
-        float *p = d.d_w1[head] + (int64_t)m * d.d_w1_ld[head] + n0 + r;
-        *p += acc[i] + d.s[head][m] * bfn;
-      }
-    }
-    if (n0 == 0 && tid < 32 && d.d_b1[head]) d.d_b1[head][m0 + tid] += d.s[head][m0 + tid];
-    return;
-  }
-  b -= A.tiles_dw1;
-  if (b < A.tiles_dwf) {
-    if (!d.d_wf) return;
-    const int m0 = (b / nt) * 32, n0 = (b % nt) * 32, kq = rows / 4;
-    for (int head = 0; head < d.n_heads; ++head)
-      if (d.m[head])
-        tile_mac(acc, d.w1[head] + m0, 1, d.w1_ld[head], d.m[head] + n0, F, 1, wave * kq, (wave + 1) * kq, lane);
-    tile_reduce(acc, red, wave, lane);
-    if (wave == 0) {
-#pragma unroll
-      for (int i = 0; i < 16; ++i) d.d_wf[(int64_t)(m0 + (i & 3) + 8 * (i >> 2) + 4 * h) * F + n0 + r] += acc[i];
-    }
-    if (n0 == 0 && d.d_bf) {
-      const int kk = tid & 31, grp = tid >> 5;
-      float sum = 0.f;
-      for (int head = 0; head < d.n_heads; ++head)
-        if (d.s[head])
-          for (int n = grp; n < rows; n += 8) sum = fmaf(d.w1[head][(int64_t)n * d.w1_ld[head] + m0 + kk], d.s[head][n], sum);
-      __syncthreads();
-      red[grp * 32 + kk] = sum;
-      __syncthreads();
-      if (tid < 32) {
-        float v = 0.f;
-#pragma unroll
-        for (int q = 0; q < 8; ++q) v += red[q * 32 + tid];
-        d.d_bf[m0 + tid] += v;
-      }
-    }
-    return;
-  }
+  unfold_body(A, (int)blockIdx.x, red);
 }
 
 static int fold_check(const bn_fold_desc *d, const char *what) {
@@ -176,11 +73,16 @@
   return 0;
 }
 
+int bn_unfold_args(const bn_fold_desc *d, FoldArgs *a) {
+  if (int e = fold_check(d, "unfold_heads")) return e;
+  a->d = *d; a->tiles_per_head = (d->rows / 32) * (d->F / 32);
+  a->tiles_dw1 = d->n_heads * a->tiles_per_head; a->tiles_dwf = (d->F / 32) * (d->F / 32);
+  return 0;
+}
+
 extern "C" int bn_unfold_heads(const bn_fold_desc *d, void *stream) {
-  if (int e = fold_check(d, "unfold_heads")) return e;
   FoldArgs a;
-  a.d = *d; a.tiles_per_head = (d->rows / 32) * (d->F / 32);
-  a.tiles_dw1 = d->n_heads * a.tiles_per_head; a.tiles_dwf = (d->F / 32) * (d->F / 32);
+  if (int e = bn_unfold_args(d, &a)) return e;
   BnProfScope prof_(BN_K_PACK, (hipStream_t)stream);
   unfold_kernel<<<dim3((unsigned)(a.tiles_dw1 + a.tiles_dwf)), 256, 0, (hipStream_t)stream>>>(a);
   BN_LAUNCH_CHECK("unfold_heads");
diff --git a/brdf_nerf_amd/csrc/prof.h b/brdf_nerf_amd/csrc/prof.h
--- a/brdf_nerf_amd/csrc/prof.h
+++ b/brdf_nerf_amd/csrc/prof.h
@@ -1,7 +1,8 @@
 #pragma once
 #include <hip/hip_runtime.h>
 enum { BN_K_PACK = 0, BN_K_FWD_SIGMA, BN_K_FWD_FULL, BN_K_BWD_CHAIN, BN_K_WGRAD, BN_K_SKINNY, BN_K_COMPOSITE_FWD,
-       BN_K_COMPOSITE_BWD, BN_K_GUIDED, BN_K_STRATIFIED, BN_K_ADAM, BN_K_BRDF, BN_K_ADJOINT, BN_K_ADJBWD, BN_K_WGRAD_REDUCE, BN_K_COUNT };
+       BN_K_COMPOSITE_BWD, BN_K_GUIDED, BN_K_STRATIFIED, BN_K_ADAM, BN_K_BRDF, BN_K_ADJOINT, BN_K_ADJBWD, BN_K_WGRAD_REDUCE,
+       BN_K_REDUCE_UNFOLD, BN_K_COUNT };
 extern bool g_bn_prof_on;
 void bn_prof_start(int id, hipStream_t st);
 void bn_prof_stop(hipStream_t st);
diff --git a/brdf_nerf_amd/functions.py b/brdf_nerf_amd/functions.py
--- a/brdf_nerf_amd/functions.py
+++ b/brdf_nerf_amd/functions.py
@@ -367,9 +367,18 @@
 
 
 def field_backward_raw(spec, named_params, named_grads, packed, out, d_out, stash, xyz=None, rays=None, z=None, unfold=True,
-                       zero_folded=True, parts=L.BN_BWD_ALL, z2=None):
+                       zero_folded=True, parts=L.BN_BWD_ALL, z2=None, merged=False):
     pts = make_points(xyz, rays, z, z2=z2)
     ps, gs = spec.params_struct(named_params), spec.params_struct(named_grads, grads=True)
+    if merged:
+        assert not (spec.fold_feats and unfold and zero_folded), "merged launches: the caller re-folds (or clears M, s) itself"
+        d = None
+        if spec.fold_feats and unfold and spec.fold_grads:
+            d, _keep = spec._fold_desc({k: v.detach() for k, v in named_params.items()}, named_grads)
+        L.check(L.lib().bn_field_backward_merged(C.byref(spec.desc), C.byref(ps), _p(packed), C.byref(pts), _p(out), _p(d_out), _p(stash),
+                                                 C.byref(gs), int(parts), C.byref(d) if d is not None else None, _stream()),
+                "bn_field_backward_merged")
+        return
     L.check(L.lib().bn_field_backward_parts(C.byref(spec.desc), C.byref(ps), _p(packed), C.byref(pts), _p(out), _p(d_out), _p(stash),
                                             C.byref(gs), int(parts), _stream()), "bn_field_backward")
     if spec.fold_feats and unfold:
diff --git a/brdf_nerf_amd/trainer.py b/brdf_nerf_amd/trainer.py
--- a/brdf_nerf_amd/trainer.py
+++ b/brdf_nerf_amd/trainer.py
@@ -58,6 +58,7 @@
         self.max_buf_variants = 3
         self.lean = True
         self.merge_passes = True
+        self._merged_launches = True
         self.overlap_allreduce = True
         self.ray_offset = 0
         self.keep_grads = False
@@ -528,7 +529,8 @@
             def backward(parts, last):
                 for b in rows.blocks:
                     Fn.field_backward_raw(spec, named, self.grad_views, packed, b.out, rows.of(rows.d_all, b), b.stash, rays=rays, z=b.z,
-                                          z2=b.z2, unfold=last and b is rows.blocks[-1], zero_folded=False, parts=parts)
+                                          z2=b.z2, unfold=last and b is rows.blocks[-1], zero_folded=False, parts=parts,
+                                          merged=self._merged_launches and self.world == 1)
             if self.world > 1 and self.overlap_allreduce and 0 < self.n_trunk < self.flat_grad.numel():
                 import torch.distributed as dist
                 backward(L.BN_BWD_CHAIN | L.BN_BWD_WGRAD_TRUNK, False)
diff --git a/include/brdfnerf_hip.h b/include/brdfnerf_hip.h
--- a/include/brdfnerf_hip.h
+++ b/include/brdfnerf_hip.h
@@ -251,6 +251,9 @@
 } bn_fold_desc;
 int bn_fold_heads(const bn_fold_desc *d, void *stream);
 int bn_unfold_heads(const bn_fold_desc *d, void *stream);
+int bn_field_backward_merged(const bn_field_desc *desc, const bn_field_params *params, const void *packed,
+                             const bn_points *pts, const float *out, const float *d_out, void *stash,
+                             const bn_field_grads *grads, int32_t parts, const bn_fold_desc *unfold, void *stream);
 
 int bn_adam_multi(float *param, float *grad, float *exp_avg, float *exp_avg_sq, int32_t n_groups, const int64_t *lo,
                   const int64_t *hi, const int32_t *active, float beta1, float beta2, float eps, float weight_decay,
diff --git a/profiles/ab_kernels.py b/profiles/ab_kernels.py
--- a/profiles/ab_kernels.py
+++ b/profiles/ab_kernels.py
@@ -82,7 +82,7 @@
             torch.cuda.synchronize()
             if rnd:
                 step_ms[tag].append((time.perf_counter() - t0) / 30 * 1e3)
-    keys = ["pack", "field_fwd_sigma", "field_fwd_full", "field_bwd_chain", "wgrad", "skinny_wgrad", "wgrad_reduce", "field_adjoint", "field_adjoint_bwd",
+    keys = ["pack", "field_fwd_sigma", "field_fwd_full", "field_bwd_chain", "wgrad", "skinny_wgrad", "wgrad_reduce", "reduce_unfold", "field_adjoint", "field_adjoint_bwd",
             "composite_fwd", "composite_bwd", "brdf", "guided_samples", "stratified_z", "adam"]
     print(f"config {config} dtype {dtype} rays {n_rays}: launches per step x ms per launch, median (min) over {rounds} alternating rounds")
     print(f"{'kernel':>18} " + " ".join(f"{t[:26]:>26}" for t in tags))
```
